# mikostrzewa/AprilSLAM

Hardware: AMD Instinct MI355X
Metric: frames/sec at 1280x720, 20 tags/frame (detection + batched PnP) (higher is better)
Workload: dtype u8/f64

## Files before the change

aprilslam_amd/csrc/aprilslam.hip:

```cpp
#include "../../include/aprilslam.h"

#include <algorithm>
#include <chrono>
#include <cmath>
#include <cstdarg>
#include <cstdio>
#include <cstring>
#include <memory>
#include <string>
#include <type_traits>
#include <vector>

#include "asl_common.h"
#include "tag_standard41h12.inc"
#include "k_wave.inc"

#include "k_threshold.inc"
#include "k_cc.inc"
#include "k_cluster.inc"
#include "k_seg.inc"
#include "k_quad.inc"
#include "k_decode.inc"
#include "k_pnp.inc"
#include "k_dedup.inc"
#include "k_graph.inc"
#include "k_render.inc"
#include "k_gn.inc"
#include "k_localize.inc"
#include "k_posecov.inc"
#include "k_rig.inc"
#include "k_calib.inc"
#include "k_map.inc"

static thread_local std::string g_err;

#include <dlfcn.h>
static struct Markers {
    int (*push)(const char *) = nullptr;
    int (*pop)() = nullptr;
    bool tried = false;
    void load()
    {
        tried = true;
        const char *e = getenv("ASL_ROCTX");
        if (!e || !*e || *e == '0') return;
        void *h = dlopen("librocprofiler-sdk-roctx.so", RTLD_NOW | RTLD_GLOBAL);
        if (!h) h = dlopen("libroctx64.so", RTLD_NOW | RTLD_GLOBAL);
        if (!h) return;
        push = reinterpret_cast<int (*)(const char *)>(dlsym(h, "roctxRangePushA"));
        pop = reinterpret_cast<int (*)()>(dlsym(h, "roctxRangePop"));
        if (!push || !pop) { push = nullptr; pop = nullptr; }
    }
} g_markers;
static inline void range_push(const char *name) { if (!g_markers.tried) g_markers.load(); if (g_markers.push) g_markers.push(name); }
static inline void range_pop() { if (g_markers.pop) g_markers.pop(); }

static int fail(int code, const char *fmt, ...)
{
    char buf[512];
    va_list ap;
    va_start(ap, fmt);
    vsnprintf(buf, sizeof buf, fmt, ap);
    va_end(ap);
    g_err = buf;
    return code;
}

#define HIPCHK(expr)                                                                                   \
    do {                                                                                               \
        hipError_t e__ = (expr);                                                                       \
        if (e__ != hipSuccess) return fail(ASL_EDEVICE, "%s failed: %s", #expr, hipGetErrorString(e__)); \
    } while (0)

#define MAX_STAGES 24

struct asl_detector {
    int device = 0;
    int maxhamming = 1;
    int decimate = 2;
    int refine = 1;
    int pnp_both_minima = 0;
    FamilyDev fam;
    DevBuf<unsigned long long> codes;
    DevBuf<unsigned short> idx_start;
    DevBuf<unsigned long long> idx_entries;

    unsigned int hash_slots_per_frame = 1024;
    unsigned int clusters_per_frame = 2048;
    unsigned int dets_per_frame = 256;
    double points_per_pixel = 0.5;

    DevBuf<uint8_t> in, dgray, tmin, tmax, tcut;
    DevBuf<uint8_t> dbg_thresh;
    DevBuf<unsigned int> dbg_labels;
    DevBuf<unsigned int> parent, sizes;
    DevBuf<unsigned long long> hkeys, points, rootmask, wmask, bmask;
    DevBuf<unsigned int> hcounts, class_lists, stage_pos, frame_cursor, dense_tiles, dense_seg, quad_list;
    DevBuf<unsigned long long> stage_rec;
    DevBuf<uint4> seg_edges;
    unsigned int stage_cap = 0;
    DevBuf<unsigned long long> slot_cluster;
    DevBuf<ClusterRec> clusters;
    DevBuf<QuadRec> quads;
    DevBuf<double> scratch, quadH, wtab, side_mom;
    DevBuf<DetRec> dets;
    DevBuf<unsigned int> frame_ndets, frame_idx, frame_nkeep, frame_off;
    DevBuf<DetOut> out_det;
    DevBuf<PoseOut> out_pose;
    DevBuf<long long> counters;
    DevBuf<float> pnp_corners;
    DevBuf<double> pnp_out;
    DevBuf<uint8_t> pnp_ok;
    DevBuf<uint8_t> gn_ws;
    DevBuf<uint8_t> loc_obs, loc_map;
    DevBuf<uint8_t> solve_out;
    DevBuf<uint8_t> rig_cams;
    DevBuf<uint8_t> cal_ws;
    DevBuf<uint8_t> map_ws, map_lm;
    hipStream_t copy_stream = nullptr, host_stream = nullptr;
    std::vector<hipEvent_t> copy_done;
    hipStream_t aux_stream = nullptr;

    Geom last{};
    unsigned int nslots = 0, max_clusters = 0, max_points = 0, max_dets = 0;
    long long last_counters[CNT__N] = {0};
    bool pending = false;
    const uint8_t *p_frames = nullptr;
    Geom p_geom{};
    hipStream_t p_stream = nullptr;
    bool p_has_cam = false;
    CamDev p_cam{};
    size_t prefetched = 0, nd_guess = 0;
    std::chrono::steady_clock::time_point t_submit, t_enqueued;
    PinnedBuf<long long> pinned_counters;
    PinnedBuf<DetOut> host_det;
    PinnedBuf<PoseOut> host_pose;
    PinnedBuf<unsigned int> host_nkeep;

    int profiling = 0;
    hipEvent_t ev[MAX_STAGES + 1] = {nullptr};
    int nev = 0;
    const char *stage_names[MAX_STAGES] = {nullptr};
    float stage_ms[MAX_STAGES] = {0};
    int nstages = 0;
    float host_ms[4] = {0, 0, 0, 0};

    size_t host_cap() const { return std::min(host_det.n, host_pose.n); }
    ~asl_detector()
    {
        for (hipStream_t s : {aux_stream, copy_stream, host_stream})
            if (s) (void)hipStreamDestroy(s);
        for (hipEvent_t e : copy_done) (void)hipEventDestroy(e);
        for (hipEvent_t e : ev)
            if (e) (void)hipEventDestroy(e);
    }
};

static const char *kVersion = "aprilslam 0.1 gfx950 (HIP, tagStandard41h12)";

extern "C" const char *asl_last_error(void) { return g_err.c_str(); }
extern "C" const char *asl_version(void) { return kVersion; }

static int build_code_index(asl_detector *d)
{
    FamilyDev &f = d->fam;
    f.idx_nch = 0; f.idx_start = nullptr; f.idx_entries = nullptr;
    const int nch = d->maxhamming + 1;
    if (f.nbits > 48 || f.ncodes > 65535 || nch > IDX_MAX_CHUNKS) return 0;
    if (getenv("ASL_NO_CODE_INDEX")) return 0;
    std::vector<unsigned short> start((size_t)nch * (IDX_BUCKETS + 1), 0);
    std::vector<unsigned long long> entries((size_t)nch * f.ncodes);
    int lo = 0;
    for (int c = 0; c < nch; c++) {
        const int w = f.nbits / nch + (c < f.nbits % nch ? 1 : 0);
        f.idx_lo[c] = lo; f.idx_w[c] = w;
        std::vector<unsigned int> bucket(f.ncodes);
        unsigned short *st = start.data() + (size_t)c * (IDX_BUCKETS + 1);
        for (int i = 0; i < f.ncodes; i++) {
            bucket[i] = idx_bucket((kTag41h12Codes[i] >> lo) & ((1ull << w) - 1ull), w);
            st[bucket[i] + 1]++;
        }
        for (int b = 0; b < IDX_BUCKETS; b++) st[b + 1] = (unsigned short)(st[b + 1] + st[b]);
        std::vector<unsigned short> fill(st, st + IDX_BUCKETS);
        for (int i = 0; i < f.ncodes; i++)
            entries[(size_t)c * f.ncodes + fill[bucket[i]]++] = ((unsigned long long)i << 48) | kTag41h12Codes[i];
        lo += w;
    }
    for (int c = nch; c < IDX_MAX_CHUNKS; c++) { f.idx_lo[c] = 0; f.idx_w[c] = 1; }
    if (d->idx_start.ensure(start.size()) || d->idx_entries.ensure((size_t)IDX_MAX_CHUNKS * kTag41h12NCodes)) return -1;
    if (hipMemcpy(d->idx_start.p, start.data(), start.size() * sizeof(unsigned short), hipMemcpyHostToDevice) != hipSuccess) return -1;
    if (hipMemcpy(d->idx_entries.p, entries.data(), entries.size() * sizeof(unsigned long long), hipMemcpyHostToDevice) != hipSuccess) return -1;
    f.idx_start = d->idx_start.p; f.idx_entries = d->idx_entries.p; f.idx_nch = nch;
    return 0;
}

extern "C" int asl_detector_create(const char *family, int nthreads, int maxhamming, float decimate, float blur,
                                   int refine_edges, int device, asl_detector **out)
{
    (void)nthreads;
    if (!out) return fail(ASL_EINVAL, "out is NULL");
    *out = nullptr;
    if (!family || strcmp(family, "tagStandard41h12") != 0)
        return fail(ASL_EINVAL, "unknown tag family '%s' (supported: tagStandard41h12)", family ? family : "(null)");
    if (!(decimate >= 1.0f) || decimate != std::floor(decimate) || decimate > 8.0f)
        return fail(ASL_EINVAL, "decimate must be an integer value in [1, 8] (got %g)", (double)decimate);
    if (blur != 0.0f) return fail(ASL_EINVAL, "blur (quad_sigma) != 0 is not supported (the reference never sets it)");
    if (maxhamming < 0 || maxhamming > 3) return fail(ASL_EINVAL, "maxhamming must be in [0, 3]");
    int ndev = 0;
    hipError_t e = hipGetDeviceCount(&ndev);
    if (e != hipSuccess || ndev <= 0) return fail(ASL_EDEVICE, "no HIP device available (%s)", hipGetErrorString(e));
    if (device < 0 || device >= ndev) return fail(ASL_EINVAL, "device %d out of range (have %d)", device, ndev);
    HIPCHK(hipSetDevice(device));
    std::unique_ptr<asl_detector> d(new asl_detector());
    d->device = device;
    d->maxhamming = maxhamming;
    d->decimate = (int)decimate;
    d->refine = refine_edges ? 1 : 0;
    memset(&d->fam, 0, sizeof d->fam);
    d->fam.nbits = kTag41h12NBits;
    d->fam.width_at_border = kTag41h12WidthAtBorder;
    d->fam.total_width = kTag41h12TotalWidth;
    d->fam.reversed_border = 1;
    d->fam.ncodes = kTag41h12PinnedIds;
    for (int i = 0; i < kTag41h12NBits; i++) { d->fam.bit_x[i] = kTag41h12BitX[i]; d->fam.bit_y[i] = kTag41h12BitY[i]; }
    if (d->codes.ensure(kTag41h12NCodes)) return fail(ASL_ENOMEM, "hipMalloc(code book) failed");
    if (hipMemcpy(d->codes.p, kTag41h12Codes, sizeof(unsigned long long) * kTag41h12NCodes, hipMemcpyHostToDevice) != hipSuccess)
        return fail(ASL_EDEVICE, "hipMemcpy(code book) failed");
    d->fam.codes = d->codes.p;
    if (build_code_index(d.get())) return fail(ASL_ENOMEM, "code-book index allocation failed");
    if (d->wtab.ensure(WEIGHT_TABLE_N)) return fail(ASL_ENOMEM, "hipMalloc(weight table) failed");
    hipLaunchKernelGGL(k_weight_table, dim3((WEIGHT_TABLE_N + 255) / 256), dim3(256), 0, 0, d->wtab.p);
    if (hipDeviceSynchronize() != hipSuccess) return fail(ASL_EDEVICE, "weight table kernel failed");
    (void)hipFuncSetAttribute(reinterpret_cast<const void *>(&k_fit_quads<256, true, CLASS3_CAP / 256>), hipFuncAttributeMaxDynamicSharedMemorySize, QUAD_LDS_BYTES(CLASS3_CAP));
    *out = d.release();
    return ASL_OK;
}

extern "C" void asl_detector_destroy(asl_detector *d)
{
    if (!d) return;
    (void)hipSetDevice(d->device);
    if (d->pending) (void)hipStreamSynchronize(d->p_stream);
    delete d;
}

extern "C" int asl_detector_set_id_limit(asl_detector *d, int n_ids)
{
    if (!d) return fail(ASL_EINVAL, "detector is NULL");
    if (n_ids > kTag41h12NCodes) return fail(ASL_EINVAL, "the code table holds %d ids (asked for %d)", kTag41h12NCodes, n_ids);
    if (d->pending) return fail(ASL_EINVAL, "a batch is in flight on this detector");
    d->fam.ncodes = n_ids <= 0 ? kTag41h12NCodes : n_ids;
    HIPCHK(hipSetDevice(d->device));
    if (build_code_index(d)) return fail(ASL_ENOMEM, "code-book index allocation failed");
    return ASL_OK;
}

extern "C" int asl_detector_set_pnp_both_minima(asl_detector *d, int enabled)
{
    if (!d) return fail(ASL_EINVAL, "detector is NULL");
    d->pnp_both_minima = enabled ? 1 : 0;
    return ASL_OK;
}

extern "C" int asl_set_profiling(asl_detector *d, int enabled)
{
    if (!d) return fail(ASL_EINVAL, "detector is NULL");
    d->profiling = enabled ? 1 : 0;
    if (enabled)
        for (int i = 0; i <= MAX_STAGES; i++)
            if (!d->ev[i]) HIPCHK(hipEventCreate(&d->ev[i]));
    return ASL_OK;
}

extern "C" int asl_stage_times(asl_detector *d, const char **names, float *ms, int max_n, int *n)
{
    if (!d || !n) return fail(ASL_EINVAL, "NULL argument");
    int k = std::min(max_n, d->nstages);
    for (int i = 0; i < k; i++) { if (names) names[i] = d->stage_names[i]; if (ms) ms[i] = d->stage_ms[i]; }
    static const char *hn[4] = {"host_enqueue", "host_wait", "host_copy", "host_post"};
    for (int i = 0; i < 4 && k < max_n; i++, k++) { if (names) names[k] = hn[i]; if (ms) ms[k] = d->host_ms[i]; }
    *n = k;
    return ASL_OK;
}

static int pnp_tpw(size_t expected)
{
    const char *e = getenv("ASL_PNP_TPW");
    if (e) { int x = atoi(e); return x < 1 ? 1 : (x > 16 ? 16 : x); }
    int v = 1;
    while (v < 16 && (size_t)v * 2 * 1024 <= expected) v <<= 1;
    return v;
}

static unsigned int next_pow2(unsigned long long v)
{
    unsigned long long p = 1;
    while (p < v) p <<= 1;
    return (unsigned int)p;
}

static int make_geom(asl_detector *d, int n_frames, int channels, int w, int h, int stride, size_t frame_pitch, Geom *g)
{
    if (n_frames <= 0 || n_frames > 65535) return fail(ASL_EINVAL, "n_frames must be in [1, 65535] (got %d)", n_frames);
    if (channels != 1 && channels != 3) return fail(ASL_EINVAL, "channels must be 1 (gray) or 3 (BGR), got %d", channels);
    if (w < 8 || h < 8 || w > 16384 || h > 16384) return fail(ASL_EINVAL, "unsupported image size %dx%d", w, h);
    if (stride < w * channels) return fail(ASL_EINVAL, "stride %d smaller than a row (%d bytes)", stride, w * channels);
    g->w = w; g->h = h; g->stride = stride; g->channels = channels; g->f = d->decimate;
    g->sw = 1 + (w - 1) / g->f; g->sh = 1 + (h - 1) / g->f;
    g->tw = g->sw / TILESZ; g->th = g->sh / TILESZ;
    g->nframes = n_frames; g->frame_pitch = frame_pitch;
    g->npix = (size_t)g->sw * g->sh;
    if (g->npix >= (1u << 24)) return fail(ASL_EINVAL, "decimated frame has %zu pixels; the cluster key holds 2^24", g->npix);
    return ASL_OK;
}

static int seg_nwx(const Geom &g) { return (g.sw + 63) / 64; }
static int seg_point_tiles_y(const Geom &g) { return std::max(1, (g.sh - 1 + SEG_PH - 1) / SEG_PH); }
static size_t count_tiles(const Geom &g) { return (size_t)seg_nwx(g) * (size_t)seg_point_tiles_y(g); }

static int ensure_workspace(asl_detector *d, const Geom &g)
{
    size_t B = (size_t)g.nframes;
    size_t total = B * g.npix;
    d->nslots = next_pow2(std::max<unsigned long long>(16384ull, (unsigned long long)B * d->hash_slots_per_frame));
    unsigned long long mc = (unsigned long long)B * d->clusters_per_frame;
    d->max_clusters = (unsigned int)std::min<unsigned long long>(mc, 0x7FFFFFFFull);
    unsigned long long mp = (unsigned long long)((double)total * d->points_per_pixel) + 65536ull;
    d->max_points = (unsigned int)std::min<unsigned long long>(mp, 0xFFFFFFF0ull);
    d->max_dets = (unsigned int)std::min<unsigned long long>((unsigned long long)B * d->dets_per_frame, 0x7FFFFFFFull);
    int bad = 0;
    bad |= d->dgray.ensure(total);
    bad |= d->tmin.ensure(B * (size_t)std::max(1, g.tw * g.th) + 8);
    bad |= d->tmax.ensure(B * (size_t)std::max(1, g.tw * g.th) + 8);
    bad |= d->tcut.ensure(B * (size_t)std::max(1, g.tw * g.th));
    bad |= d->parent.ensure(total);
    bad |= d->sizes.ensure(total);
    bad |= d->rootmask.ensure(B * (size_t)g.sh * (size_t)seg_nwx(g));
    bad |= d->wmask.ensure(B * (size_t)g.sh * (size_t)seg_nwx(g));
    bad |= d->bmask.ensure(B * (size_t)g.sh * (size_t)seg_nwx(g));
    bad |= d->hkeys.ensure(d->nslots);
    bad |= d->hcounts.ensure(d->nslots);
    bad |= d->class_lists.ensure((size_t)NCLASSES * d->max_clusters);
    bad |= d->slot_cluster.ensure(d->nslots);
    bad |= d->clusters.ensure(d->max_clusters);
    bad |= d->quads.ensure(d->max_clusters);
    bad |= d->quad_list.ensure(d->max_clusters);
    bad |= d->quadH.ensure((size_t)10 * d->max_clusters);
    bad |= d->side_mom.ensure((size_t)24 * d->max_clusters);
    bad |= d->points.ensure(d->max_points);
    d->stage_cap = (unsigned int)((double)g.npix * d->points_per_pixel) + 1024u;
    bad |= d->stage_rec.ensure((size_t)B * d->stage_cap);
    bad |= d->stage_pos.ensure((size_t)B * d->stage_cap);
    bad |= d->frame_cursor.ensure(B);
    bad |= d->dense_tiles.ensure(B * count_tiles(g));
    bad |= d->dense_seg.ensure(B * (size_t)seg_nwx(g) * (size_t)((g.sh + SEG_TH - 1) / SEG_TH));
    bad |= d->seg_edges.ensure(B * (size_t)seg_nwx(g) * (size_t)((g.sh + SEG_TH - 1) / SEG_TH));
    bad |= d->scratch.ensure((size_t)d->max_points * 8);
    bad |= d->dets.ensure(d->max_dets);
    bad |= d->frame_ndets.ensure(B);
    bad |= d->frame_nkeep.ensure(B);
    bad |= d->frame_off.ensure(B);
    bad |= d->frame_idx.ensure(B * (size_t)d->dets_per_frame);
    bad |= d->out_det.ensure(d->max_dets);
    bad |= d->out_pose.ensure(d->max_dets);
    bad |= d->counters.ensure(CNT__N);
    if (bad) return fail(ASL_ENOMEM, "device workspace allocation failed (%zu frames of %dx%d)", B, g.sw, g.sh);
    return ASL_OK;
}

#define STAGE(name)                                                        \
    do {                                                                   \
        if (d->profiling && d->nev < MAX_STAGES) {                         \
            d->stage_names[d->nev] = name;                                 \
            HIPCHK(hipEventRecord(d->ev[d->nev], st));                     \
            d->nev++;                                                      \
        }                                                                  \
    } while (0)

static int tag_width(const asl_detector *d, const Geom &g) { return std::max(3, d->fam.width_at_border / g.f); }

template <int BLOCK, int CAP>
static void launch_fit(asl_detector *d, const Geom &g, int cls, unsigned int grid, hipStream_t st)
{
    const int want_rev = d->fam.reversed_border ? 1 : 0, want_norm = d->fam.reversed_border ? 0 : 1;
    hipLaunchKernelGGL((k_fit_quads<BLOCK, (CAP > 0), CAP / BLOCK>), dim3(grid), dim3(BLOCK), CAP > 0 ? QUAD_LDS_BYTES(CAP) : 0, st, d->clusters.p,
                       d->class_lists.p + (size_t)cls * d->max_clusters, d->counters.p, cls, d->max_clusters, CAP, d->points.p, d->dgray.p, g,
                       tag_width(d, g), want_rev, want_norm, d->scratch.p, d->quads.p, d->wtab.p, d->side_mom.p);
}

static void launch_fit_class(asl_detector *d, const Geom &g, int cls, unsigned int B, hipStream_t st)
{
    const unsigned int qgrid = std::min<unsigned int>(d->max_clusters, std::max<unsigned int>(16384u, 32u * B));
    const unsigned int q2grid = std::min<unsigned int>(d->max_clusters, 2048u);
    switch (cls) {
    case 0: return launch_fit<64, CLASS0_CAP>(d, g, 0, qgrid, st);
    case 1: return launch_fit<128, CLASS1_CAP>(d, g, 1, qgrid, st);
    case 2: return launch_fit<256, CLASS2_CAP>(d, g, 2, q2grid, st);
    case 3: return launch_fit<256, CLASS3_CAP>(d, g, 3, q2grid, st);
    default: return launch_fit<256, 0>(d, g, 4, q2grid, st);
    }
}

static void launch_quad_finish(asl_detector *d, const Geom &g, hipStream_t st)
{
    hipLaunchKernelGGL(k_quad_finish, dim3(std::min<unsigned int>((d->max_clusters + 63) / 64, 4096u)), dim3(256), 0, st, d->quads.p, d->side_mom.p, d->counters.p,
                       d->max_clusters, tag_width(d, g));
}

static int enqueue_detect(asl_detector *d, const uint8_t *d_frames, const Geom &g, hipStream_t st, const CamDev *cam)
{
    dim3 blk(64, 4, 1);
    int thx = (g.sh + TILESZ - 1) / TILESZ;
    unsigned int B = (unsigned int)g.nframes;
    d->nev = 0;
    range_push("S0-S4 gray, decimate, threshold, segmentation, clusters");
    STAGE("k_hash_clear");
    hipLaunchKernelGGL(k_hash_clear, dim3((std::max<unsigned int>(d->nslots, std::max<unsigned int>(B, CNT__N)) + 255) / 256), dim3(256), 0, st, d->hkeys.p,
                       d->hcounts.p, d->nslots, d->counters.p, d->frame_cursor.p, d->frame_ndets.p, B);

    STAGE("k_decimate_minmax");
    if (g.f == 2) {
        const unsigned int ntile = (unsigned int)(g.tw * g.th);
        const unsigned int nrest = (unsigned int)(g.sw - 4 * g.tw) * (unsigned int)g.sh + (unsigned int)(g.sh - 4 * g.th) * (unsigned int)(4 * g.tw);
        if (ntile)
            hipLaunchKernelGGL((g.channels == 1 ? k_decimate2_tiles<1> : k_decimate2_tiles<3>), dim3((ntile + 255) / 256, B), dim3(256), 0, st, d_frames, g,
                               d->dgray.p, d->tmin.p, d->tmax.p);
        if (nrest)
            hipLaunchKernelGGL((g.channels == 1 ? k_decimate_rest<1> : k_decimate_rest<3>), dim3((nrest + 255) / 256, B), dim3(256), 0, st, d_frames, g,
                               d->dgray.p);
    } else
        hipLaunchKernelGGL((g.channels == 1 ? k_decimate_minmax<1> : k_decimate_minmax<3>), dim3((g.sw + 63) / 64, (thx + 3) / 4, B), blk, 0, st, d_frames, g, d->dgray.p, d->tmin.p, d->tmax.p);

    const int nwx = seg_nwx(g), pty = seg_point_tiles_y(g);
    const size_t nwords = (size_t)B * g.sh * nwx;
    STAGE("k_tile_cut");
    if (g.tw > 0 && g.th > 0)
        hipLaunchKernelGGL(k_tile_cut, dim3((((g.tw + 3) / 4) * ((g.th + 3) / 4) + 255) / 256, B), dim3(256), 0, st, d->tmin.p, d->tmax.p, g, d->tcut.p);
    STAGE("k_seg_tile");
    {
        const int ntiles = nwx * ((g.sh + SEG_TH - 1) / SEG_TH);
        hipLaunchKernelGGL(k_seg_tile, dim3((ntiles + SEG_TILE_WAVES - 1) / SEG_TILE_WAVES, 1, B), dim3(64 * SEG_TILE_WAVES), 0, st, d->dgray.p, d->tcut.p, g, nwx, ntiles,
                           d->wmask.p, d->bmask.p, d->parent.p, d->sizes.p, d->rootmask.p, d->seg_edges.p, d->dense_seg.p, d->counters.p);
        hipLaunchKernelGGL(k_seg_tile_dense, dim3(1024), dim3(64), 0, st, g, nwx, ntiles, d->wmask.p, d->bmask.p, d->parent.p, d->sizes.p,
                           d->rootmask.p, d->dense_seg.p, d->counters.p);
    }
    STAGE("k_seg_border");
    {
        const size_t nseams = nwx > 1 ? (size_t)B * g.sh * (nwx - 1) : 0;
        const unsigned int ncol_blocks = (unsigned int)((nseams + 63) / 64);
        const int nrb = (g.sh - 1) / SEG_TH;
        const unsigned int nrow_blocks = (unsigned int)nwx * (unsigned int)nrb * (unsigned int)B;
        if (ncol_blocks + nrow_blocks > 0)
            hipLaunchKernelGGL(k_seg_border, dim3(ncol_blocks + nrow_blocks), dim3(64), 0, st, d->wmask.p, d->bmask.p, d->seg_edges.p,
                               nwx * ((g.sh + SEG_TH - 1) / SEG_TH), g, nwx, d->parent.p, d->counters.p, ncol_blocks, nrb > 0 ? nrb : 1);
    }
    STAGE("k_seg_roots");
    hipLaunchKernelGGL(k_seg_roots, dim3((unsigned int)((nwords + 255) / 256)), dim3(256), 0, st, d->rootmask.p, g, nwx, d->parent.p, d->sizes.p);

    STAGE("k_seg_points");
    hipLaunchKernelGGL((k_seg_points<SEGP_PCAP, SEGP_RUNCAP, SEGP_NW, 1>), dim3(B, (nwx + SEGP_NW - 1) / SEGP_NW, pty), dim3(64 * SEGP_NW), 0, st,
                       d->wmask.p, d->bmask.p, g, nwx, d->parent.p, d->sizes.p, d->hkeys.p, d->hcounts.p, d->nslots - 1, d->stage_rec.p,
                       d->stage_pos.p, d->frame_cursor.p, d->stage_cap, d->dense_tiles.p, pty, d->counters.p);
    hipLaunchKernelGGL((k_seg_points<SEGP_PCAP_DENSE, SEGP_RUNCAP_DENSE, 1, 2>), dim3(256), dim3(64), 0, st, d->wmask.p, d->bmask.p, g, nwx,
                       d->parent.p, d->sizes.p, d->hkeys.p, d->hcounts.p, d->nslots - 1, d->stage_rec.p, d->stage_pos.p, d->frame_cursor.p,
                       d->stage_cap, d->dense_tiles.p, pty, d->counters.p);
    STAGE("k_cluster_filter");
    hipLaunchKernelGGL(k_cluster_filter, dim3((d->nslots + 1023) / 1024), dim3(1024), 0, st, d->hkeys.p, d->hcounts.p, d->nslots, g,
                       d->clusters.p, d->slot_cluster.p, d->class_lists.p, d->max_clusters, d->max_points, d->counters.p);
    STAGE("k_point_place");
    hipLaunchKernelGGL(k_point_place, dim3(16, B), dim3(256), 0, st, d->stage_rec.p, d->stage_pos.p, d->frame_cursor.p, d->stage_cap,
                       d->slot_cluster.p, d->points.p, d->counters.p);

    range_pop();
    range_push("S5 quad fit");
    for (int cls = 0; cls < NCLASSES; cls++) {
        static const char *const kFitStage[NCLASSES] = {"k_fit_quads<0>", "k_fit_quads<1>", "k_fit_quads<2>", "k_fit_quads<3>", "k_fit_quads<4>"};
        STAGE(kFitStage[cls]);
        launch_fit_class(d, g, cls, B, st);
    }

    STAGE("k_quad_finish");
    launch_quad_finish(d, g, st);
    range_pop();
    range_push("S6-S7 edge refinement, homography, decode");
    STAGE("k_quad_compact");
    hipLaunchKernelGGL(k_quad_compact, dim3((d->max_clusters + 1023) / 1024), dim3(1024), 0, st, d->quads.p, d->counters.p, d->max_clusters,
                       d->quad_list.p);
    unsigned int dgrid = std::min<unsigned int>(d->max_clusters, std::max<unsigned int>(8192u, 64u * B));
    STAGE("k_refine");
    hipLaunchKernelGGL((g.channels == 1 ? k_refine<1> : k_refine<3>), dim3(dgrid), dim3(64), 0, st, d->quads.p, d->counters.p, d->max_clusters, d_frames, g,
                       d->fam.reversed_border ? 1 : 0, d->refine, d->quadH.p, d->quad_list.p, d->side_mom.p);
    STAGE("k_homography");
    hipLaunchKernelGGL(k_homography, dim3(std::min<unsigned int>((d->max_clusters + 31) / 32, 2048u)), dim3(256), 0, st, d->quadH.p, d->counters.p, d->max_clusters,
                       d->quad_list.p, d->side_mom.p);
    STAGE("k_decode");
    hipLaunchKernelGGL((g.channels == 1 ? k_decode<1> : k_decode<3>), dim3(dgrid), dim3(64), 0, st, d->quads.p, d->quadH.p, d->counters.p, d->max_clusters, d_frames, g, d->fam,
                       d->maxhamming, d->dets.p, d->max_dets, d->counters.p, d->quad_list.p);

    range_pop();
    range_push("S9 PnP, S8 de-duplication");
    if (cam) {
        STAGE("k_pnp_dets");
        const int tpw = pnp_tpw(d->nd_guess ? d->nd_guess : (size_t)20 * B);
        hipLaunchKernelGGL(k_pnp_dets, dim3((d->max_dets + tpw - 1) / tpw), dim3(64), 0, st, d->dets.p, d->counters.p, d->max_dets, *cam, tpw);
    }
    STAGE("k_det_dedup");
    {
        const unsigned int cap_f = d->dets_per_frame;
        hipLaunchKernelGGL(k_det_bucket, dim3((d->max_dets + 255) / 256), dim3(256), 0, st, d->dets.p, d->counters.p, d->max_dets, d->frame_ndets.p,
                           d->frame_idx.p, cap_f, d->counters.p);
        hipLaunchKernelGGL(k_det_dedup, dim3(B), dim3(256), 0, st, d->dets.p, d->counters.p, d->frame_ndets.p, d->frame_idx.p, cap_f,
                           d->frame_nkeep.p, d->counters.p);
        hipLaunchKernelGGL(k_det_offsets, dim3(1), dim3(1024), 0, st, d->frame_nkeep.p, B, d->frame_off.p, d->counters.p);
        hipLaunchKernelGGL(k_det_gather, dim3((cap_f + 255) / 256, B), dim3(256), 0, st, d->dets.p, d->frame_idx.p, cap_f, d->frame_nkeep.p,
                           d->frame_off.p, d->out_det.p, d->out_pose.p, d->max_dets, cam ? 1 : 0);
    }
    range_pop();
    if (d->profiling && d->nev <= MAX_STAGES) HIPCHK(hipEventRecord(d->ev[d->nev], st));
    HIPCHK(hipGetLastError());
    return ASL_OK;
}

static CamDev make_cam(const asl_detector *d, const double *K, const double *dist, int n_dist, double tag_size)
{
    CamDev c;
    c.both_minima = d->pnp_both_minima; c.pad = 0;
    c.fx = K[0]; c.fy = K[4]; c.cx = K[2]; c.cy = K[5];
    c.k1 = c.k2 = c.p1 = c.p2 = c.k3 = 0;
    if (dist && n_dist >= 4) { c.k1 = dist[0]; c.k2 = dist[1]; c.p1 = dist[2]; c.p2 = dist[3]; }
    if (dist && n_dist >= 5) c.k3 = dist[4];
    c.half = (double)(float)(tag_size / 2);
    return c;
}

using clk = std::chrono::steady_clock;
static float msf(clk::time_point a, clk::time_point b) { return std::chrono::duration<float, std::milli>(b - a).count(); }

static int ensure_host_out(asl_detector *d, size_t want, size_t nframes)
{
    HIPCHK(d->host_nkeep.ensure(nframes, hipHostMallocDefault));
    if (want <= d->host_cap()) return ASL_OK;
    d->host_det.release(); d->host_pose.release();
    want = std::max<size_t>(want * 2, 4096);
    HIPCHK(d->host_det.ensure(want, hipHostMallocNonCoherent));
    HIPCHK(d->host_pose.ensure(want, hipHostMallocNonCoherent));
    return ASL_OK;
}

static int submit_batch(asl_detector *d, const uint8_t *d_frames, const Geom &g, hipStream_t st, const CamDev *cam)
{
    if (d->pending) return fail(ASL_EINVAL, "a batch is already in flight on this detector: collect it first");
    int rc = ensure_workspace(d, g);
    if (rc) return rc;
    d->t_submit = clk::now();
    rc = enqueue_detect(d, d_frames, g, st, cam);
    if (rc) return rc;
    HIPCHK(d->pinned_counters.ensure(CNT__N, hipHostMallocDefault));
    HIPCHK(hipMemcpyAsync(d->pinned_counters.p, d->counters.p, sizeof(long long) * CNT__N, hipMemcpyDeviceToHost, st));
    d->prefetched = 0;
    rc = ensure_host_out(d, std::min<size_t>(d->nd_guess, d->max_dets), (size_t)g.nframes);
    if (rc) return rc;
    HIPCHK(hipMemcpyAsync(d->host_nkeep.p, d->frame_nkeep.p, sizeof(unsigned int) * (size_t)g.nframes, hipMemcpyDeviceToHost, st));
    if (d->nd_guess > 0) {
        size_t guess = std::min<size_t>(d->nd_guess, d->max_dets);
        HIPCHK(hipMemcpyAsync(d->host_det.p, d->out_det.p, guess * sizeof(DetOut), hipMemcpyDeviceToHost, st));
        if (cam) HIPCHK(hipMemcpyAsync(d->host_pose.p, d->out_pose.p, guess * sizeof(PoseOut), hipMemcpyDeviceToHost, st));
        d->prefetched = guess;
    }
    d->pending = true;
    d->p_frames = d_frames; d->p_geom = g; d->p_stream = st; d->p_has_cam = cam != nullptr;
    if (cam) d->p_cam = *cam;
    d->t_enqueued = clk::now();
    return ASL_OK;
}

static int collect_batch(asl_detector *d, asl_detection *out, asl_pose *poses, int max_out, int *n_per_frame, int *n_out)
{
    if (!d->pending) return fail(ASL_EINVAL, "no batch in flight on this detector");
    const Geom g = d->p_geom;
    hipStream_t st = d->p_stream;
    const CamDev *cam = d->p_has_cam ? &d->p_cam : nullptr;
    clk::time_point t0 = d->t_submit, t1 = d->t_enqueued, t2 = t1;
    for (int attempt = 0; attempt < 4; attempt++) {
        if (attempt > 0) {
            d->pending = false;
            d->nd_guess = 0;
            int rc = submit_batch(d, d->p_frames, g, st, cam);
            if (rc) return rc;
        }
        HIPCHK(hipStreamSynchronize(st));
        t2 = clk::now();
        memcpy(d->last_counters, d->pinned_counters.p, sizeof(long long) * CNT__N);
        d->last = g;
        long long *c = d->last_counters;
        if (c[CNT_UF_GUARD]) {
            d->pending = false;
            return fail(ASL_ECAPACITY, "a union-find loop hit its iteration guard (%lld times): labels of this batch are not trustworthy", c[CNT_UF_GUARD]);
        }
        bool again = false;
        if (c[CNT_OVERFLOW_HASH]) { d->hash_slots_per_frame *= 4; again = true; }
        if (c[CNT_OVERFLOW_CLUSTERS] || c[CNT_NCLUSTERS] > (long long)d->max_clusters) { d->clusters_per_frame *= 4; again = true; }
        if (c[CNT_OVERFLOW_POINTS]) { d->points_per_pixel *= 2; again = true; }
        if (c[CNT_OVERFLOW_DETS]) { d->dets_per_frame *= 4; again = true; }
        if (again) {
            if (attempt == 3) {
                d->pending = false;
                return fail(ASL_ECAPACITY, "work buffers still overflow after growing (hash %lld clusters %lld points %lld dets %lld)",
                            c[CNT_OVERFLOW_HASH], c[CNT_OVERFLOW_CLUSTERS], c[CNT_OVERFLOW_POINTS], c[CNT_OVERFLOW_DETS]);
            }
            continue;
        }
        break;
    }
    d->pending = false;
    if (d->profiling) {
        d->nstages = d->nev;
        for (int i = 0; i < d->nev; i++) HIPCHK(hipEventElapsedTime(&d->stage_ms[i], d->ev[i], d->ev[i + 1]));
    }
    if (d->last_counters[CNT_DEDUP_LIMIT])
        return fail(ASL_ECAPACITY, "%lld frame(s) hold more than %d detections: the de-duplication does not sort that many", d->last_counters[CNT_DEDUP_LIMIT], DEDUP_MAX);
    size_t nd = (size_t)d->last_counters[CNT_NKEEP];
    if (nd > d->max_dets) nd = d->max_dets;
    if (nd > d->prefetched) {
        size_t have = d->prefetched;
        if (nd > d->host_cap()) have = 0;
        int rc = ensure_host_out(d, nd, (size_t)g.nframes);
        if (rc) return rc;
        HIPCHK(hipMemcpy(d->host_det.p + have, d->out_det.p + have, (nd - have) * sizeof(DetOut), hipMemcpyDeviceToHost));
        if (cam) HIPCHK(hipMemcpy(d->host_pose.p + have, d->out_pose.p + have, (nd - have) * sizeof(PoseOut), hipMemcpyDeviceToHost));
    }
    d->nd_guess = nd + nd / 4 + 256;
    clk::time_point t3 = clk::now();
    static_assert(sizeof(DetOut) == sizeof(asl_detection) && sizeof(PoseOut) == sizeof(asl_pose), "device results are copied verbatim");
    int total = (int)nd;
    int nw = std::min(total, max_out);
    if (out && nw > 0) memcpy(out, d->host_det.p, (size_t)nw * sizeof(asl_detection));
    if (poses && cam && nw > 0) memcpy(poses, d->host_pose.p, (size_t)nw * sizeof(asl_pose));
    if (n_per_frame) for (int f = 0; f < g.nframes; f++) n_per_frame[f] = (int)d->host_nkeep.p[f];
    if (n_out) *n_out = total;
    d->host_ms[0] = msf(t0, t1); d->host_ms[1] = msf(t1, t2); d->host_ms[2] = msf(t2, t3); d->host_ms[3] = msf(t3, clk::now());
    return ASL_OK;
}

static int check_n_dist(int n_dist)
{
    if (n_dist != 0 && n_dist != 4 && n_dist != 5) return fail(ASL_EINVAL, "n_dist must be 0, 4 or 5");
    return ASL_OK;
}

static int check_device_args(asl_detector *d, const void *d_frames, int n_frames, int channels, int w, int h, int stride, size_t frame_pitch,
                             int n_dist, Geom *g)
{
    if (!d || !d_frames) return fail(ASL_EINVAL, "NULL detector or frames");
    if (int rc = check_n_dist(n_dist)) return rc;
    HIPCHK(hipSetDevice(d->device));
    int rc = make_geom(d, n_frames, channels, w, h, stride, frame_pitch, g);
    if (rc) return rc;
    if (frame_pitch < (size_t)stride * (size_t)h) return fail(ASL_EINVAL, "frame_pitch smaller than one frame");
    return ASL_OK;
}

extern "C" int asl_submit_batch_device(asl_detector *d, const void *d_frames, int n_frames, int channels, int w, int h, int stride,
                                       size_t frame_pitch, void *stream, const double *K, const double *dist, int n_dist, double tag_size)
{
    Geom g;
    int rc = check_device_args(d, d_frames, n_frames, channels, w, h, stride, frame_pitch, n_dist, &g);
    if (rc) return rc;
    CamDev cam;
    if (K) cam = make_cam(d, K, dist, n_dist, tag_size);
    return submit_batch(d, (const uint8_t *)d_frames, g, (hipStream_t)stream, K ? &cam : nullptr);
}

extern "C" int asl_collect_batch(asl_detector *d, asl_detection *out, asl_pose *poses, int max_out, int *n_per_frame, int *n_out)
{
    if (!d) return fail(ASL_EINVAL, "NULL detector");
    if (max_out < 0 || (max_out > 0 && !out)) return fail(ASL_EINVAL, "out is NULL");
    HIPCHK(hipSetDevice(d->device));
    return collect_batch(d, out, poses, max_out, n_per_frame, n_out);
}

extern "C" int asl_collect_batch_view(asl_detector *d, const asl_detection **out, const asl_pose **poses, const uint32_t **n_per_frame, int *n_out)
{
    if (!d || !out || !n_per_frame || !n_out) return fail(ASL_EINVAL, "NULL argument");
    HIPCHK(hipSetDevice(d->device));
    const bool with_poses = d->p_has_cam;
    int rc = collect_batch(d, nullptr, nullptr, 0, nullptr, n_out);
    if (rc) return rc;
    *out = reinterpret_cast<const asl_detection *>(d->host_det.p);
    if (poses) *poses = with_poses ? reinterpret_cast<const asl_pose *>(d->host_pose.p) : nullptr;
    *n_per_frame = d->host_nkeep.p;
    return ASL_OK;
}

extern "C" int asl_detect_batch_device(asl_detector *d, const void *d_frames, int n_frames, int channels, int w, int h, int stride,
                                       size_t frame_pitch, void *stream, const double *K, const double *dist, int n_dist,
                                       double tag_size, asl_detection *out, asl_pose *poses, int max_out, int *n_per_frame, int *n_out)
{
    if (max_out < 0 || (max_out > 0 && !out)) return fail(ASL_EINVAL, "out is NULL");
    int rc = asl_submit_batch_device(d, d_frames, n_frames, channels, w, h, stride, frame_pitch, stream, K, dist, n_dist, tag_size);
    if (rc) return rc;
    return collect_batch(d, out, poses, max_out, n_per_frame, n_out);
}

#define HOST_CHUNK_FRAMES 64
static hipError_t copy_frames(asl_detector *d, const uint8_t *const *frames, int f0, int f1, size_t pitch, hipStream_t st)
{
    int i = f0;
    while (i < f1) {
        int j = i + 1;
        while (j < f1 && frames[j] == frames[j - 1] + pitch) j++;
        hipError_t e = hipMemcpyAsync(d->in.p + (size_t)i * pitch, frames[i], pitch * (size_t)(j - i), hipMemcpyHostToDevice, st);
        if (e != hipSuccess) return e;
        i = j;
    }
    return hipSuccess;
}

static int detect_host_frames(asl_detector *d, const uint8_t *const *frames, int n_frames, int channels, int w, int h, int stride,
                              const CamDev *cam, asl_detection *out, asl_pose *poses, int max_out, int *n_per_frame, int *n_out)
{
    Geom g;
    const size_t pitch = (size_t)stride * (size_t)h;
    int rc = make_geom(d, n_frames, channels, w, h, stride, pitch, &g);
    if (rc) return rc;
    if (d->in.ensure(pitch * (size_t)n_frames)) return fail(ASL_ENOMEM, "input staging allocation failed");
    for (int i = 0; i < n_frames; i++)
        if (!frames[i]) return fail(ASL_EINVAL, "frames[%d] is NULL", i);
    int chunk = HOST_CHUNK_FRAMES;
    { const char *e = getenv("ASL_HOST_CHUNK"); if (e && atoi(e) > 0) chunk = atoi(e); }
    const int nchunks = n_frames >= 2 * chunk ? (n_frames + chunk - 1) / chunk : 1;
    if (nchunks == 1) {
        HIPCHK(copy_frames(d, frames, 0, n_frames, pitch, nullptr));
        int rcs = submit_batch(d, d->in.p, g, nullptr, cam);
        if (rcs) return rcs;
        return collect_batch(d, out, poses, max_out, n_per_frame, n_out);
    }
    if (!d->copy_stream) {
        HIPCHK(hipStreamCreateWithFlags(&d->copy_stream, hipStreamNonBlocking));
        HIPCHK(hipStreamCreateWithFlags(&d->host_stream, hipStreamNonBlocking));
    }
    while ((int)d->copy_done.size() < nchunks) {
        hipEvent_t e;
        HIPCHK(hipEventCreateWithFlags(&e, hipEventDisableTiming));
        d->copy_done.push_back(e);
    }
    HIPCHK(hipStreamSynchronize(nullptr));
    for (int c = 0; c < nchunks; c++) {
        const int f0 = c * chunk, f1 = std::min(n_frames, f0 + chunk);
        HIPCHK(copy_frames(d, frames, f0, f1, pitch, d->copy_stream));
        HIPCHK(hipEventRecord(d->copy_done[c], d->copy_stream));
    }
    int total = 0;
    for (int c = 0; c < nchunks; c++) {
        const int f0 = c * chunk, f1 = std::min(n_frames, f0 + chunk);
        Geom gc = g;
        gc.nframes = f1 - f0;
        HIPCHK(hipStreamWaitEvent(d->host_stream, d->copy_done[c], 0));
        int rcs = submit_batch(d, d->in.p + (size_t)f0 * pitch, gc, d->host_stream, cam);
        if (rcs) { (void)hipStreamSynchronize(d->copy_stream); return rcs; }
        int nc = 0;
        const int room = std::max(0, max_out - total);
        rcs = collect_batch(d, out ? out + std::min(total, max_out) : nullptr, (poses && cam) ? poses + std::min(total, max_out) : nullptr, room,
                            n_per_frame ? n_per_frame + f0 : nullptr, &nc);
        if (rcs) { (void)hipStreamSynchronize(d->copy_stream); return rcs; }
        for (int k = total; k < std::min(total + nc, max_out); k++) out[k].frame += f0;
        total += nc;
    }
    if (n_out) *n_out = total;
    return ASL_OK;
}

extern "C" int asl_detect_batch_u8(asl_detector *d, const uint8_t *const *frames, int n_frames, int channels, int w, int h, int stride,
                                   asl_detection *out, int max_out, int *n_per_frame, int *n_out)
{
    if (!d || !frames) return fail(ASL_EINVAL, "NULL detector or frames");
    if (max_out < 0 || (max_out > 0 && !out)) return fail(ASL_EINVAL, "out is NULL");
    HIPCHK(hipSetDevice(d->device));
    return detect_host_frames(d, frames, n_frames, channels, w, h, stride, nullptr, out, nullptr, max_out, n_per_frame, n_out);
}

extern "C" int asl_detect_batch_pose_u8(asl_detector *d, const uint8_t *const *frames, int n_frames, int channels, int w, int h, int stride,
                                        const double *K, const double *dist, int n_dist, double tag_size, asl_detection *out, asl_pose *poses,
                                        int max_out, int *n_per_frame, int *n_out)
{
    if (!d || !frames || !K || !poses) return fail(ASL_EINVAL, "NULL detector, frames, K or poses");
    if (max_out < 0 || (max_out > 0 && !out)) return fail(ASL_EINVAL, "out is NULL");
    if (int rc = check_n_dist(n_dist)) return rc;
    if (n_dist && !dist) return fail(ASL_EINVAL, "dist is NULL but n_dist = %d", n_dist);
    HIPCHK(hipSetDevice(d->device));
    CamDev cam = make_cam(d, K, dist, n_dist, tag_size);
    return detect_host_frames(d, frames, n_frames, channels, w, h, stride, &cam, out, poses, max_out, n_per_frame, n_out);
}

extern "C" int asl_detect_gray_u8(asl_detector *d, const uint8_t *gray, int w, int h, int stride, asl_detection *out, int max_out, int *n_out)
{
    const uint8_t *fr[1] = {gray};
    return asl_detect_batch_u8(d, fr, 1, 1, w, h, stride, out, max_out, nullptr, n_out);
}

extern "C" int asl_detect_bgr_u8(asl_detector *d, const uint8_t *bgr, int w, int h, int stride, asl_detection *out, int max_out, int *n_out)
{
    const uint8_t *fr[1] = {bgr};
    return asl_detect_batch_u8(d, fr, 1, 3, w, h, stride, out, max_out, nullptr, n_out);
}

extern "C" int asl_render_frames_device(asl_detector *d, void *d_frames, int n_frames, int w, int h, int stride, size_t frame_pitch,
                                        const void *d_planes, int max_planes, const void *d_textures, int tw, int th, double half,
                                        const double *K, const double *dist, int n_dist, void *stream)
{
    if (!d || !d_frames || !d_planes || !d_textures) return fail(ASL_EINVAL, "NULL argument");
    if (n_frames <= 0 || w <= 0 || h <= 0 || max_planes <= 0 || tw <= 0 || th <= 0) return fail(ASL_EINVAL, "sizes must be positive");
    if (stride < 3 * w || frame_pitch < (size_t)stride * (size_t)h) return fail(ASL_EINVAL, "stride / frame_pitch smaller than a BGR row / frame");
    if (dist && n_dist != 4 && n_dist != 5) return fail(ASL_EINVAL, "n_dist must be 4 or 5");
    if (dist && !K) return fail(ASL_EINVAL, "lens coefficients need the camera matrix");
    static_assert(sizeof(RenderPlane) == sizeof(asl_render_plane) && sizeof(asl_render_plane) == 96, "asl_render_plane layout");
    HIPCHK(hipSetDevice(d->device));
    RenderCam cam;
    memset(&cam, 0, sizeof cam);
    cam.iters = 8;
    if (K && dist) {
        cam.fx = K[0]; cam.fy = K[4]; cam.cx = K[2]; cam.cy = K[5];
        cam.k1 = dist[0]; cam.k2 = dist[1]; cam.p1 = dist[2]; cam.p2 = dist[3]; cam.k3 = n_dist >= 5 ? dist[4] : 0.0;
        cam.distort = 1;
    }
    hipLaunchKernelGGL(k_render, dim3((w + RENDER_TW - 1) / RENDER_TW, (h + 4 * RENDER_TH - 1) / (4 * RENDER_TH), (unsigned int)n_frames), dim3(64, 4), 0, (hipStream_t)stream, (uint8_t *)d_frames, w, h,
                       stride, frame_pitch, (const RenderPlane *)d_planes, max_planes, (const uint8_t *)d_textures, tw, th, half, cam);
    HIPCHK(hipGetLastError());
    return ASL_OK;
}

extern "C" int asl_pack_observations_device(asl_detector *d, void *d_obs, int max_tags, void *stream)
{
    if (!d || !d_obs) return fail(ASL_EINVAL, "NULL detector or output");
    if (max_tags <= 0) return fail(ASL_EINVAL, "max_tags must be positive");
    if (!d->pending) return fail(ASL_EINVAL, "no batch in flight on this detector: pack between submit and the next submit");
    static_assert(sizeof(ObsRec) == sizeof(asl_obs) && sizeof(asl_obs) == 136, "asl_obs layout");
    HIPCHK(hipSetDevice(d->device));
    const int nf = d->p_geom.nframes;
    const unsigned int total = (unsigned int)nf * (unsigned int)max_tags;
    hipLaunchKernelGGL(k_obs_pack, dim3((total + 255) / 256), dim3(256), 0, (hipStream_t)stream, d->dets.p, d->frame_idx.p, d->dets_per_frame,
                       d->frame_nkeep.p, d->counters.p, (ObsRec *)d_obs, nf, max_tags);
    HIPCHK(hipGetLastError());
    return ASL_OK;
}

extern "C" int asl_graph_frames_device(asl_detector *d, const void *d_obs, int world, int n_frames, int max_tags, int coordinate_id,
                                       double *d_pose, uint8_t *d_status, uint32_t *d_last, int n_ids, void *d_picks, void *stream)
{
    if (!d || !d_obs || !d_pose || !d_status || !d_last) return fail(ASL_EINVAL, "NULL argument");
    if (world <= 0 || n_frames <= 0 || max_tags <= 0 || n_ids <= 0) return fail(ASL_EINVAL, "sizes must be positive");
    HIPCHK(hipSetDevice(d->device));
    const unsigned int total = (unsigned int)world * (unsigned int)n_frames;
    const int lds_ids = (size_t)n_ids * sizeof(unsigned int) <= 48 * 1024 ? n_ids : 0;
    hipLaunchKernelGGL(k_graph_frames, dim3((total + 255) / 256), dim3(256), sizeof(unsigned int) * (size_t)lds_ids, (hipStream_t)stream, (const ObsRec *)d_obs,
                       world, n_frames, max_tags, coordinate_id, d_pose, d_status, (unsigned int *)d_last, n_ids, lds_ids);
    if (d_picks)
        hipLaunchKernelGGL(k_graph_pick, dim3((n_ids + 255) / 256), dim3(256), 0, (hipStream_t)stream, (const ObsRec *)d_obs, world, n_frames, max_tags,
                           (const unsigned int *)d_last, n_ids, (ObsRec *)d_picks);
    HIPCHK(hipGetLastError());
    return ASL_OK;
}

extern "C" int asl_graph_picks_device(asl_detector *d, const void *d_obs, int world, int n_frames, int max_tags, const uint8_t *d_status,
                                      unsigned int order_lo, unsigned int order_hi, uint32_t *d_last, int n_ids, void *d_picks, void *stream)
{
    if (!d || !d_obs || !d_status || !d_last || !d_picks) return fail(ASL_EINVAL, "NULL argument");
    if (world <= 0 || n_frames <= 0 || max_tags <= 0 || n_ids <= 0) return fail(ASL_EINVAL, "sizes must be positive");
    if (order_lo > order_hi) return fail(ASL_EINVAL, "empty or reversed range");
    HIPCHK(hipSetDevice(d->device));
    HIPCHK(hipMemsetAsync(d_last, 0, sizeof(uint32_t) * (size_t)n_ids, (hipStream_t)stream));
    const unsigned int total = (unsigned int)world * (unsigned int)n_frames;
    const int lds_ids = (size_t)n_ids * sizeof(unsigned int) <= 48 * 1024 ? n_ids : 0;
    hipLaunchKernelGGL(k_graph_last_range, dim3((total + 255) / 256), dim3(256), sizeof(unsigned int) * (size_t)lds_ids, (hipStream_t)stream, (const ObsRec *)d_obs,
                       world, n_frames, max_tags, d_status, order_lo, order_hi, (unsigned int *)d_last, n_ids, lds_ids);
    hipLaunchKernelGGL(k_graph_pick, dim3((n_ids + 255) / 256), dim3(256), 0, (hipStream_t)stream, (const ObsRec *)d_obs, world, n_frames, max_tags,
                       (const unsigned int *)d_last, n_ids, (ObsRec *)d_picks);
    HIPCHK(hipGetLastError());
    return ASL_OK;
}

extern "C" int asl_solve_pnp_batch(asl_detector *d, const float *corners, const double *K, const double *dist, int n_dist,
                                   double tag_size, double *rvec, double *tvec, double *T, uint8_t *ok, int N)
{
    if (!d || !corners || !K || !rvec || !tvec || !T || !ok) return fail(ASL_EINVAL, "NULL argument");
    if (N < 0) return fail(ASL_EINVAL, "N < 0");
    if (int rc = check_n_dist(n_dist)) return rc;
    if (N == 0) return ASL_OK;
    HIPCHK(hipSetDevice(d->device));
    if (d->pnp_corners.ensure((size_t)N * 8) || d->pnp_out.ensure((size_t)N * 22) || d->pnp_ok.ensure((size_t)N))
        return fail(ASL_ENOMEM, "PnP workspace allocation failed");
    CamDev cam = make_cam(d, K, dist, n_dist, tag_size);
    HIPCHK(hipMemcpy(d->pnp_corners.p, corners, sizeof(float) * 8 * (size_t)N, hipMemcpyHostToDevice));
    double *dr = d->pnp_out.p, *dt = dr + 3 * (size_t)N, *dT = dt + 3 * (size_t)N;
    hipLaunchKernelGGL(k_pnp_batch, dim3((N + pnp_tpw((size_t)N) - 1) / pnp_tpw((size_t)N)), dim3(64), 0, nullptr, d->pnp_corners.p, N, cam, dr, dt, dT, d->pnp_ok.p, pnp_tpw((size_t)N));
    HIPCHK(hipGetLastError());
    HIPCHK(hipMemcpy(rvec, dr, sizeof(double) * 3 * (size_t)N, hipMemcpyDeviceToHost));
    HIPCHK(hipMemcpy(tvec, dt, sizeof(double) * 3 * (size_t)N, hipMemcpyDeviceToHost));
    HIPCHK(hipMemcpy(T, dT, sizeof(double) * 16 * (size_t)N, hipMemcpyDeviceToHost));
    HIPCHK(hipMemcpy(ok, d->pnp_ok.p, (size_t)N, hipMemcpyDeviceToHost));
    return ASL_OK;
}

#include "gn_host.inc"


static int check_obs_args(int max_tags, int n_ids, int n_dist, bool no_dist, double tag_size)
{
    if (max_tags < 1 || max_tags > 256) return fail(ASL_EINVAL, "max_tags must be in [1, 256] (got %d)", max_tags);
    if (n_ids < 1) return fail(ASL_EINVAL, "n_ids must be >= 1 (got %d)", n_ids);
    if (int rc = check_n_dist(n_dist)) return rc;
    if (n_dist && no_dist) return fail(ASL_EINVAL, "dist is NULL with n_dist = %d", n_dist);
    if (!(tag_size > 0) || !std::isfinite(tag_size)) return fail(ASL_EINVAL, "tag_size must be positive (got %g)", tag_size);
    return ASL_OK;
}

static int upload_obs(asl_detector *d, const char *what, const asl_obs *obs, int n_frames, int max_tags, const asl_map_tag *map, int n_ids)
{
    const size_t obs_bytes = sizeof(asl_obs) * (size_t)n_frames * (size_t)max_tags, map_bytes = sizeof(asl_map_tag) * (size_t)n_ids;
    if (d->loc_obs.ensure(obs_bytes) || (map && d->loc_map.ensure(map_bytes))) return fail(ASL_ENOMEM, "%s workspace allocation failed", what);
    HIPCHK(hipMemcpy(d->loc_obs.p, obs, obs_bytes, hipMemcpyHostToDevice));
    if (map) HIPCHK(hipMemcpy(d->loc_map.p, map, map_bytes, hipMemcpyHostToDevice));
    return ASL_OK;
}

static int check_localize_args(const void *obs, int n_frames, int max_tags, const void *map, int n_ids, const double *K, const double *dist,
                               int n_dist, double tag_size, double max_tag_rms_px, const void *out)
{
    if (!obs || !map || !K || !out) return fail(ASL_EINVAL, "NULL argument");
    if (n_frames < 0) return fail(ASL_EINVAL, "n_frames < 0");
    if (int rc = check_obs_args(max_tags, n_ids, n_dist, !dist, tag_size)) return rc;
    if (!(max_tag_rms_px >= 0) || !std::isfinite(max_tag_rms_px)) return fail(ASL_EINVAL, "max_tag_rms_px must be >= 0 (got %g)", max_tag_rms_px);
    return ASL_OK;
}

static void launch_localize(asl_detector *d, const void *d_obs, int n_frames, int max_tags, const void *d_map, int n_ids, const double *K,
                            const double *dist, int n_dist, double tag_size, double max_tag_rms_px, void *d_out, void *d_cov, double sigma_px,
                            hipStream_t st)
{
    CamDev cam = make_cam(d, K, dist, n_dist, tag_size);
    if (d_cov)
        hipLaunchKernelGGL(k_localize<true>, dim3((unsigned int)n_frames), dim3(ASL_WAVE), loc_lds_bytes(max_tags), st, (const ObsRec *)d_obs, max_tags,
                           (const MapTagRec *)d_map, n_ids, cam, max_tag_rms_px, (CamPoseRec *)d_out, (PoseCovRec *)d_cov, sigma_px);
    else
        hipLaunchKernelGGL(k_localize<false>, dim3((unsigned int)n_frames), dim3(ASL_WAVE), loc_lds_bytes(max_tags), st, (const ObsRec *)d_obs, max_tags,
                           (const MapTagRec *)d_map, n_ids, cam, max_tag_rms_px, (CamPoseRec *)d_out, (PoseCovRec *)nullptr, 0.0);
}

static int check_sigma_px(double sigma_px)
{
    if (!(sigma_px >= 0) || !std::isfinite(sigma_px)) return fail(ASL_EINVAL, "sigma_px must be >= 0 and finite (got %g)", sigma_px);
    return ASL_OK;
}

static int localize_frames_device(asl_detector *d, const void *d_obs, int n_frames, int max_tags, const void *d_map, int n_ids, const double *K,
                                  const double *dist, int n_dist, double tag_size, double max_tag_rms_px, double sigma_px, void *d_out,
                                  void *d_cov, void *stream)
{
    static_assert(sizeof(MapTagRec) == sizeof(asl_map_tag) && sizeof(asl_map_tag) == 104, "asl_map_tag layout");
    static_assert(sizeof(CamPoseRec) == sizeof(asl_cam_pose) && sizeof(asl_cam_pose) == 160, "asl_cam_pose layout");
    static_assert(sizeof(PoseCovRec) == sizeof(asl_pose_cov) && sizeof(asl_pose_cov) == 304, "asl_pose_cov layout");
    if (!d) return fail(ASL_EINVAL, "NULL detector");
    int rc = check_localize_args(d_obs, n_frames, max_tags, d_map, n_ids, K, dist, n_dist, tag_size, max_tag_rms_px, d_out);
    if (rc) return rc;
    if ((rc = check_sigma_px(sigma_px))) return rc;
    if (n_frames == 0) return ASL_OK;
    HIPCHK(hipSetDevice(d->device));
    launch_localize(d, d_obs, n_frames, max_tags, d_map, n_ids, K, dist, n_dist, tag_size, max_tag_rms_px, d_out, d_cov, sigma_px, (hipStream_t)stream);
    HIPCHK(hipGetLastError());
    return ASL_OK;
}

extern "C" int asl_localize_frames_device(asl_detector *d, const void *d_obs, int n_frames, int max_tags, const void *d_map, int n_ids,
                                          const double *K, const double *dist, int n_dist, double tag_size, double max_tag_rms_px,
                                          void *d_out, void *stream)
{
    return localize_frames_device(d, d_obs, n_frames, max_tags, d_map, n_ids, K, dist, n_dist, tag_size, max_tag_rms_px, 0.0, d_out, nullptr, stream);
}

extern "C" int asl_localize_cov_frames_device(asl_detector *d, const void *d_obs, int n_frames, int max_tags, const void *d_map, int n_ids,
                                              const double *K, const double *dist, int n_dist, double tag_size, double max_tag_rms_px,
                                              double sigma_px, void *d_out, void *d_cov, void *stream)
{
    if (!d_cov) return fail(ASL_EINVAL, "NULL argument");
    return localize_frames_device(d, d_obs, n_frames, max_tags, d_map, n_ids, K, dist, n_dist, tag_size, max_tag_rms_px, sigma_px, d_out, d_cov, stream);
}

static int localize_batch(asl_detector *d, const asl_obs *obs, int n_frames, int max_tags, const asl_map_tag *map, int n_ids, const double *K,
                          const double *dist, int n_dist, double tag_size, double max_tag_rms_px, double sigma_px, asl_cam_pose *out,
                          asl_pose_cov *cov)
{
    if (!d) return fail(ASL_EINVAL, "NULL detector");
    int rc = check_localize_args(obs, n_frames, max_tags, map, n_ids, K, dist, n_dist, tag_size, max_tag_rms_px, out);
    if (rc) return rc;
    if ((rc = check_sigma_px(sigma_px))) return rc;
    if (n_frames == 0) return ASL_OK;
    HIPCHK(hipSetDevice(d->device));
    asl_cam_pose *d_out = nullptr;
    asl_pose_cov *d_cov = nullptr;
    if (carve_ws(d->solve_out, [&](WsCarve &c) { d_out = c.take<asl_cam_pose>(n_frames); d_cov = c.take<asl_pose_cov>(cov ? n_frames : 0); }))
        return fail(ASL_ENOMEM, "localisation workspace allocation failed");
    if ((rc = upload_obs(d, "localisation", obs, n_frames, max_tags, map, n_ids))) return rc;
    launch_localize(d, d->loc_obs.p, n_frames, max_tags, d->loc_map.p, n_ids, K, dist, n_dist, tag_size, max_tag_rms_px, d_out, cov ? d_cov : nullptr,
                    sigma_px, nullptr);
    HIPCHK(hipGetLastError());
    HIPCHK(hipMemcpy(out, d_out, sizeof(asl_cam_pose) * (size_t)n_frames, hipMemcpyDeviceToHost));
    if (cov) HIPCHK(hipMemcpy(cov, d_cov, sizeof(asl_pose_cov) * (size_t)n_frames, hipMemcpyDeviceToHost));
    return ASL_OK;
}

extern "C" int asl_localize_batch(asl_detector *d, const asl_obs *obs, int n_frames, int max_tags, const asl_map_tag *map, int n_ids,
                                  const double *K, const double *dist, int n_dist, double tag_size, double max_tag_rms_px, asl_cam_pose *out)
{
    return localize_batch(d, obs, n_frames, max_tags, map, n_ids, K, dist, n_dist, tag_size, max_tag_rms_px, 0.0, out, nullptr);
}

extern "C" int asl_localize_cov_batch(asl_detector *d, const asl_obs *obs, int n_frames, int max_tags, const asl_map_tag *map, int n_ids,
                                      const double *K, const double *dist, int n_dist, double tag_size, double max_tag_rms_px, double sigma_px,
                                      asl_cam_pose *out, asl_pose_cov *cov)
{
    if (!cov) return fail(ASL_EINVAL, "NULL argument");
    return localize_batch(d, obs, n_frames, max_tags, map, n_ids, K, dist, n_dist, tag_size, max_tag_rms_px, sigma_px, out, cov);
}


static int check_rig_table(const asl_rig_camera *rig, int n_cams)
{
    for (int c = 0; c < n_cams; c++) {
        const asl_rig_camera &r = rig[c];
        if (check_n_dist(r.n_dist)) return fail(ASL_EINVAL, "camera %d: n_dist must be 0, 4 or 5 (got %d)", c, r.n_dist);
        for (int k = 0; k < 9; k++)
            if (!std::isfinite(r.K[k])) return fail(ASL_EINVAL, "camera %d: K is not finite", c);
        for (int k = 0; k < r.n_dist; k++)
            if (!std::isfinite(r.dist[k])) return fail(ASL_EINVAL, "camera %d: dist is not finite", c);
        for (int k = 0; k < 12; k++)
            if (!std::isfinite(r.E[k])) return fail(ASL_EINVAL, "camera %d: E is not finite", c);
        const double *E = r.E;
        double dev = 0;
        for (int i = 0; i < 3; i++)
            for (int j = 0; j < 3; j++)
                dev = std::max(dev, std::fabs(E[4 * i] * E[4 * j] + E[4 * i + 1] * E[4 * j + 1] + E[4 * i + 2] * E[4 * j + 2] - (i == j ? 1.0 : 0.0)));
        const double det = E[0] * (E[5] * E[10] - E[6] * E[9]) - E[1] * (E[4] * E[10] - E[6] * E[8]) + E[2] * (E[4] * E[9] - E[5] * E[8]);
        if (!(dev <= 1e-6) || !(det > 0))
            return fail(ASL_EINVAL, "camera %d: the rotation part of E is not a rotation (|R R^T - I| = %g, det %g)", c, dev, det);
    }
    return ASL_OK;
}

static int check_rig_args(const void *obs, int n_cams, int n_frames, int max_tags, const void *map, int n_ids, const void *rig, double tag_size,
                          double max_tag_rms_px, double sigma_px, const void *out)
{
    if (!obs || !map || !rig || !out) return fail(ASL_EINVAL, "NULL argument");
    if (n_frames < 0) return fail(ASL_EINVAL, "n_frames < 0");
    if (n_cams < 1 || n_cams > RIG_MAX_CAMS) return fail(ASL_EINVAL, "n_cams must be in [1, %d] (got %d)", RIG_MAX_CAMS, n_cams);
    if (int rc = check_obs_args(max_tags, n_ids, 0, false, tag_size)) return rc;
    if (n_cams * max_tags > RIG_MAX_SLOTS) return fail(ASL_EINVAL, "n_cams * max_tags must be <= %d (got %d x %d)", RIG_MAX_SLOTS, n_cams, max_tags);
    if (!(max_tag_rms_px >= 0) || !std::isfinite(max_tag_rms_px)) return fail(ASL_EINVAL, "max_tag_rms_px must be >= 0 (got %g)", max_tag_rms_px);
    return check_sigma_px(sigma_px);
}

static void launch_localize_rig(const void *d_obs, int n_cams, int n_frames, int max_tags, const void *d_map, int n_ids, const void *d_rig,
                                double tag_size, double max_tag_rms_px, void *d_out, void *d_cov, double sigma_px, hipStream_t st)
{
    const double half = (double)(float)(tag_size / 2);
    if (d_cov)
        hipLaunchKernelGGL(k_localize_rig<true>, dim3((unsigned int)n_frames), dim3(ASL_WAVE), rig_lds_bytes(n_cams, max_tags), st, (const ObsRec *)d_obs,
                           n_cams, max_tags, (const MapTagRec *)d_map, n_ids, (const RigCamRec *)d_rig, half, max_tag_rms_px, (CamPoseRec *)d_out,
                           (PoseCovRec *)d_cov, sigma_px);
    else
        hipLaunchKernelGGL(k_localize_rig<false>, dim3((unsigned int)n_frames), dim3(ASL_WAVE), rig_lds_bytes(n_cams, max_tags), st, (const ObsRec *)d_obs,
                           n_cams, max_tags, (const MapTagRec *)d_map, n_ids, (const RigCamRec *)d_rig, half, max_tag_rms_px, (CamPoseRec *)d_out,
                           (PoseCovRec *)nullptr, 0.0);
}

static int localize_rig_frames_device(asl_detector *d, const void *d_obs, int n_cams, int n_frames, int max_tags, const void *d_map, int n_ids,
                                      const void *d_rig, double tag_size, double max_tag_rms_px, double sigma_px, void *d_out, void *d_cov,
                                      void *stream)
{
    static_assert(sizeof(RigCamRec) == sizeof(asl_rig_camera) && sizeof(asl_rig_camera) == 216, "asl_rig_camera layout");
    if (!d) return fail(ASL_EINVAL, "NULL detector");
    if (int rc = check_rig_args(d_obs, n_cams, n_frames, max_tags, d_map, n_ids, d_rig, tag_size, max_tag_rms_px, sigma_px, d_out)) return rc;
    HIPCHK(hipSetDevice(d->device));
    asl_rig_camera tab[RIG_MAX_CAMS];
    HIPCHK(hipMemcpy(tab, d_rig, sizeof(asl_rig_camera) * (size_t)n_cams, hipMemcpyDeviceToHost));
    if (int rc = check_rig_table(tab, n_cams)) return rc;
    if (n_frames == 0) return ASL_OK;
    launch_localize_rig(d_obs, n_cams, n_frames, max_tags, d_map, n_ids, d_rig, tag_size, max_tag_rms_px, d_out, d_cov, sigma_px, (hipStream_t)stream);
    HIPCHK(hipGetLastError());
    return ASL_OK;
}

extern "C" int asl_localize_rig_frames_device(asl_detector *d, const void *d_obs, int n_cams, int n_frames, int max_tags, const void *d_map,
                                              int n_ids, const void *d_rig, double tag_size, double max_tag_rms_px, void *d_out, void *stream)
{
    return localize_rig_frames_device(d, d_obs, n_cams, n_frames, max_tags, d_map, n_ids, d_rig, tag_size, max_tag_rms_px, 0.0, d_out, nullptr, stream);
}

extern "C" int asl_localize_rig_cov_frames_device(asl_detector *d, const void *d_obs, int n_cams, int n_frames, int max_tags, const void *d_map,
                                                  int n_ids, const void *d_rig, double tag_size, double max_tag_rms_px, double sigma_px,
                                                  void *d_out, void *d_cov, void *stream)
{
    if (!d_cov) return fail(ASL_EINVAL, "NULL argument");
    return localize_rig_frames_device(d, d_obs, n_cams, n_frames, max_tags, d_map, n_ids, d_rig, tag_size, max_tag_rms_px, sigma_px, d_out, d_cov, stream);
}

static int localize_rig_batch(asl_detector *d, const asl_obs *obs, int n_cams, int n_frames, int max_tags, const asl_map_tag *map, int n_ids,
                              const asl_rig_camera *rig, double tag_size, double max_tag_rms_px, double sigma_px, asl_cam_pose *out,
                              asl_pose_cov *cov)
{
    if (!d) return fail(ASL_EINVAL, "NULL detector");
    int rc = check_rig_args(obs, n_cams, n_frames, max_tags, map, n_ids, rig, tag_size, max_tag_rms_px, sigma_px, out);
    if (rc) return rc;
    if ((rc = check_rig_table(rig, n_cams))) return rc;
    if (n_frames == 0) return ASL_OK;
    HIPCHK(hipSetDevice(d->device));
    asl_cam_pose *d_out = nullptr;
    asl_pose_cov *d_cov = nullptr;
    if (carve_ws(d->solve_out, [&](WsCarve &c) { d_out = c.take<asl_cam_pose>(n_frames); d_cov = c.take<asl_pose_cov>(cov ? n_frames : 0); }) ||
        d->rig_cams.ensure(sizeof(asl_rig_camera) * (size_t)n_cams))
        return fail(ASL_ENOMEM, "rig localisation workspace allocation failed");
    if ((rc = upload_obs(d, "rig localisation", obs, n_cams * n_frames, max_tags, map, n_ids))) return rc;
    HIPCHK(hipMemcpy(d->rig_cams.p, rig, sizeof(asl_rig_camera) * (size_t)n_cams, hipMemcpyHostToDevice));
    launch_localize_rig(d->loc_obs.p, n_cams, n_frames, max_tags, d->loc_map.p, n_ids, d->rig_cams.p, tag_size, max_tag_rms_px, d_out,
                        cov ? d_cov : nullptr, sigma_px, nullptr);
    HIPCHK(hipGetLastError());
    HIPCHK(hipMemcpy(out, d_out, sizeof(asl_cam_pose) * (size_t)n_frames, hipMemcpyDeviceToHost));
    if (cov) HIPCHK(hipMemcpy(cov, d_cov, sizeof(asl_pose_cov) * (size_t)n_frames, hipMemcpyDeviceToHost));
    return ASL_OK;
}

extern "C" int asl_localize_rig_batch(asl_detector *d, const asl_obs *obs, int n_cams, int n_frames, int max_tags, const asl_map_tag *map, int n_ids,
                                      const asl_rig_camera *rig, double tag_size, double max_tag_rms_px, asl_cam_pose *out)
{
    return localize_rig_batch(d, obs, n_cams, n_frames, max_tags, map, n_ids, rig, tag_size, max_tag_rms_px, 0.0, out, nullptr);
}

extern "C" int asl_localize_rig_cov_batch(asl_detector *d, const asl_obs *obs, int n_cams, int n_frames, int max_tags, const asl_map_tag *map,
                                          int n_ids, const asl_rig_camera *rig, double tag_size, double max_tag_rms_px, double sigma_px,
                                          asl_cam_pose *out, asl_pose_cov *cov)
{
    if (!cov) return fail(ASL_EINVAL, "NULL argument");
    return localize_rig_batch(d, obs, n_cams, n_frames, max_tags, map, n_ids, rig, tag_size, max_tag_rms_px, sigma_px, out, cov);
}


static int check_pose_cov_args(const void *in, int n, const double *K, const double *dist, int n_dist, double tag_size, double sigma_px, const void *cov)
{
    if (!in || !K || !cov) return fail(ASL_EINVAL, "NULL argument");
    if (n < 0) return fail(ASL_EINVAL, "record count < 0");
    if (int rc = check_n_dist(n_dist)) return rc;
    if (n_dist && !dist) return fail(ASL_EINVAL, "dist is NULL with n_dist = %d", n_dist);
    if (!(tag_size > 0) || !std::isfinite(tag_size)) return fail(ASL_EINVAL, "tag_size must be positive (got %g)", tag_size);
    return check_sigma_px(sigma_px);
}

static void launch_pose_cov(asl_detector *d, const void *d_obs, int n, const double *K, const double *dist, int n_dist, double tag_size,
                            double sigma_px, void *d_cov, hipStream_t st)
{
    CamDev cam = make_cam(d, K, dist, n_dist, tag_size);
    hipLaunchKernelGGL(k_pnp_cov, dim3((unsigned int)((n + PNP_TAGS_PER_WAVE - 1) / PNP_TAGS_PER_WAVE)), dim3(ASL_WAVE), 0, st, (const ObsRec *)d_obs, n, cam,
                       sigma_px, (PoseCovRec *)d_cov);
}

extern "C" int asl_pose_cov_device(asl_detector *d, const void *d_obs, int n_records, const double *K, const double *dist, int n_dist,
                                   double tag_size, double sigma_px, void *d_cov, void *stream)
{
    if (!d) return fail(ASL_EINVAL, "NULL detector");
    if (int rc = check_pose_cov_args(d_obs, n_records, K, dist, n_dist, tag_size, sigma_px, d_cov)) return rc;
    if (n_records == 0) return ASL_OK;
    HIPCHK(hipSetDevice(d->device));
    launch_pose_cov(d, d_obs, n_records, K, dist, n_dist, tag_size, sigma_px, d_cov, (hipStream_t)stream);
    HIPCHK(hipGetLastError());
    return ASL_OK;
}

extern "C" int asl_solve_pnp_cov_batch(asl_detector *d, const float *corners, const double *T, const double *K, const double *dist, int n_dist,
                                       double tag_size, double sigma_px, asl_pose_cov *cov, int N)
{
    if (!d) return fail(ASL_EINVAL, "NULL detector");
    if (!T) return fail(ASL_EINVAL, "NULL argument");
    if (int rc = check_pose_cov_args(corners, N, K, dist, n_dist, tag_size, sigma_px, cov)) return rc;
    if (N == 0) return ASL_OK;
    HIPCHK(hipSetDevice(d->device));
    std::vector<asl_obs> rec((size_t)N);
    for (int i = 0; i < N; i++) {
        bool finite = true;
        for (int k = 0; k < 12; k++) finite = finite && std::isfinite(T[16 * (size_t)i + k]);
        rec[i].id = 0;
        rec[i].flags = finite ? 3 : 1;
        memcpy(rec[i].corners, corners + 8 * (size_t)i, sizeof rec[i].corners);
        memcpy(rec[i].T, T + 16 * (size_t)i, sizeof rec[i].T);
    }
    const size_t cov_bytes = sizeof(asl_pose_cov) * (size_t)N;
    if (d->solve_out.ensure(cov_bytes)) return fail(ASL_ENOMEM, "pose covariance workspace allocation failed");
    if (int rc = upload_obs(d, "pose covariance", rec.data(), 1, N, nullptr, 0)) return rc;
    launch_pose_cov(d, d->loc_obs.p, N, K, dist, n_dist, tag_size, sigma_px, d->solve_out.p, nullptr);
    HIPCHK(hipGetLastError());
    HIPCHK(hipMemcpy(cov, d->solve_out.p, cov_bytes, hipMemcpyDeviceToHost));
    return ASL_OK;
}

static int check_calib_args(const void *obs, int n_frames, int max_tags, const void *map, int n_ids, double tag_size, int width, int height,
                            const double *K_init, int n_dist, int flags, int max_iters, const void *result, const void *poses)
{
    if (!obs || !map || !result || !poses) return fail(ASL_EINVAL, "NULL argument");
    if (n_frames < 1) return fail(ASL_EINVAL, "n_frames must be >= 1 (got %d)", n_frames);
    if (int rc = check_obs_args(max_tags, n_ids, n_dist, false, tag_size)) return rc;
    if (width < 1 || height < 1) return fail(ASL_EINVAL, "width and height must be positive (got %d x %d)", width, height);
    if (max_iters < 1) return fail(ASL_EINVAL, "max_iters must be >= 1 (got %d)", max_iters);
    if (flags & ~(ASL_CALIB_FIX_PRINCIPAL_POINT | ASL_CALIB_FIX_ASPECT_RATIO | ASL_CALIB_ZERO_TANGENT_DIST))
        return fail(ASL_EINVAL, "unknown calibration flags 0x%x", flags);
    if (K_init && !(K_init[0] > 0 && K_init[4] > 0 && std::isfinite(K_init[0]) && std::isfinite(K_init[4]) && std::isfinite(K_init[2]) &&
                    std::isfinite(K_init[5])))
        return fail(ASL_EINVAL, "K_init must have finite, positive focal lengths");
    return ASL_OK;
}

static int launch_calibrate(asl_detector *d, const void *d_obs, int n_frames, int max_tags, const void *d_map, int n_ids, double tag_size,
                            int width, int height, const double *K_init, int n_dist, int flags, int max_iters, void *d_result, void *d_poses,
                            hipStream_t st)
{
    static_assert(sizeof(CalibResultRec) == sizeof(asl_calib_result) && sizeof(asl_calib_result) == 216, "asl_calib_result layout");
    const size_t nf = (size_t)n_frames;
    CalibArgs a{};
    if (carve_ws(d->cal_ws, [&](WsCarve &c) {
            a.st = c.take<CalibState>(1); a.list = c.take<int>(nf); a.fr = c.take<int>(CAL_FR * nf);
            a.zh = c.take<double>(CAL_ZH * nf); a.seedc = c.take<double>(nf); a.pose = c.take<double>(2 * 12 * nf);
            a.H = c.take<double>(2 * CAL_HS * nf); a.SB = c.take<double>(CAL_SB * nf); a.back = c.take<double>(CAL_BK * nf);
        }))
        return fail(ASL_ENOMEM, "calibration workspace allocation failed");
    a.obs = (const ObsRec *)d_obs; a.map = (const MapTagRec *)d_map;
    a.res = (CalibResultRec *)d_result; a.out = (CamPoseRec *)d_poses;
    a.half = (double)(float)(tag_size / 2);
    a.width = width; a.height = height;
    a.has_init = K_init != nullptr;
    if (K_init) { a.Kinit[0] = K_init[0]; a.Kinit[1] = K_init[4]; a.Kinit[2] = K_init[2]; a.Kinit[3] = K_init[5]; }
    a.n_frames = n_frames; a.max_tags = max_tags; a.n_ids = n_ids; a.n_dist = n_dist; a.flags = flags; a.max_iters = max_iters;
    int np = 0;
    if (!(flags & ASL_CALIB_FIX_ASPECT_RATIO)) a.sel[np++] = 0;
    a.sel[np++] = 1;
    if (!(flags & ASL_CALIB_FIX_PRINCIPAL_POINT)) { a.sel[np++] = 2; a.sel[np++] = 3; }
    if (n_dist >= 4) {
        a.sel[np++] = 4; a.sel[np++] = 5;
        if (!(flags & ASL_CALIB_ZERO_TANGENT_DIST)) { a.sel[np++] = 6; a.sel[np++] = 7; }
    }
    if (n_dist == 5) a.sel[np++] = 8;
    a.np = np;
    const dim3 frames((unsigned int)n_frames), wave(ASL_WAVE), wg(CAL_WG);
    const size_t lds = loc_lds_bytes(max_tags);
    auto seed = n_dist == 5 ? k_calib_seed<5> : n_dist == 4 ? k_calib_seed<4> : k_calib_seed<0>;
    auto step = n_dist == 5 ? k_calib_step<5> : n_dist == 4 ? k_calib_step<4> : k_calib_step<0>;
    hipLaunchKernelGGL(k_calib_init, frames, wave, 0, st, a);
    hipLaunchKernelGGL(k_calib_k0, dim3(1), wg, 0, st, a);
    hipLaunchKernelGGL(seed, frames, wave, lds, st, a);
    hipLaunchKernelGGL(k_calib_start, dim3(1), wg, 0, st, a);
    for (int it = 0; it < max_iters; it++) {
        hipLaunchKernelGGL(k_calib_schur, frames, wave, 0, st, a, 0);
        hipLaunchKernelGGL(k_calib_solve, dim3(1), wg, 0, st, a);
        hipLaunchKernelGGL(step, frames, wave, lds, st, a);
        hipLaunchKernelGGL(k_calib_decide, dim3(1), wg, 0, st, a);
    }
    hipLaunchKernelGGL(k_calib_schur, frames, wave, 0, st, a, 1);
    hipLaunchKernelGGL(k_calib_finish, dim3(1), wg, 0, st, a);
    HIPCHK(hipGetLastError());
    return ASL_OK;
}

extern "C" int asl_calibrate_frames_device(asl_detector *d, const void *d_obs, int n_frames, int max_tags, const void *d_map, int n_ids,
                                           double tag_size, int width, int height, const double *K_init, int n_dist, int flags, int max_iters,
                                           void *d_result, void *d_poses, void *stream)
{
    if (!d) return fail(ASL_EINVAL, "NULL detector");
    int rc = check_calib_args(d_obs, n_frames, max_tags, d_map, n_ids, tag_size, width, height, K_init, n_dist, flags, max_iters, d_result, d_poses);
    if (rc) return rc;
    HIPCHK(hipSetDevice(d->device));
    return launch_calibrate(d, d_obs, n_frames, max_tags, d_map, n_ids, tag_size, width, height, K_init, n_dist, flags, max_iters, d_result,
                            d_poses, (hipStream_t)stream);
}

extern "C" int asl_calibrate_batch(asl_detector *d, const asl_obs *obs, int n_frames, int max_tags, const asl_map_tag *map, int n_ids,
                                   double tag_size, int width, int height, const double *K_init, int n_dist, int flags, int max_iters,
                                   asl_calib_result *result, asl_cam_pose *poses)
{
    if (!d) return fail(ASL_EINVAL, "NULL detector");
    int rc = check_calib_args(obs, n_frames, max_tags, map, n_ids, tag_size, width, height, K_init, n_dist, flags, max_iters, result, poses);
    if (rc) return rc;
    HIPCHK(hipSetDevice(d->device));
    asl_calib_result *d_result;
    asl_cam_pose *d_poses;
    if (carve_ws(d->solve_out, [&](WsCarve &c) { d_result = c.take<asl_calib_result>(1); d_poses = c.take<asl_cam_pose>(n_frames); }))
        return fail(ASL_ENOMEM, "calibration workspace allocation failed");
    if ((rc = upload_obs(d, "calibration", obs, n_frames, max_tags, map, n_ids))) return rc;
    rc = launch_calibrate(d, d->loc_obs.p, n_frames, max_tags, d->loc_map.p, n_ids, tag_size, width, height, K_init, n_dist, flags, max_iters,
                          d_result, d_poses, nullptr);
    if (rc) return rc;
    HIPCHK(hipMemcpy(result, d_result, sizeof(asl_calib_result), hipMemcpyDeviceToHost));
    HIPCHK(hipMemcpy(poses, d_poses, sizeof(asl_cam_pose) * (size_t)n_frames, hipMemcpyDeviceToHost));
    return ASL_OK;
}

static int check_map_args(const void *obs, int n_frames, int max_tags, int n_ids, const double *K, const double *dist, int n_dist,
                          double tag_size, int world_id, int max_iters, const void *map, const void *poses, const void *result)
{
    if (!obs || !K || !map || !poses || !result) return fail(ASL_EINVAL, "NULL argument");
    if (n_frames < 1) return fail(ASL_EINVAL, "n_frames must be >= 1 (got %d)", n_frames);
    if (int rc = check_obs_args(max_tags, n_ids, n_dist, !dist, tag_size)) return rc;
    if (world_id < -1 || world_id >= n_ids) return fail(ASL_EINVAL, "world_id must be -1 or in [0, n_ids) (got %d)", world_id);
    if (max_iters < 1 || max_iters > MAP_MAX_ITERS) return fail(ASL_EINVAL, "max_iters must be in [1, %d] (got %d)", MAP_MAX_ITERS, max_iters);
    return ASL_OK;
}

static int launch_map(asl_detector *d, const void *d_obs, int n_frames, int max_tags, int n_ids, const double *K, const double *dist, int n_dist,
                      double tag_size, int world_id, int max_iters, void *d_map, void *d_std, void *d_poses, void *d_result, hipStream_t st)
{
    static_assert(sizeof(MapResultRec) == sizeof(asl_map_result) && sizeof(asl_map_result) == 64, "asl_map_result layout");
    const size_t nf = (size_t)n_frames, ni = (size_t)n_ids, nsl = nf * (size_t)max_tags;
    MapArgs a{};
    int *per_id, *per_frame, *per_cam, *per_obs, *csr;
    if (carve_ws(d->map_ws, [&](WsCarve &c) {
            a.head = c.take<MapHead>(1); per_id = c.take<int>(4 * (ni + 1)); per_frame = c.take<int>(3 * (nf + 1));
            per_cam = c.take<int>(4 * (nf + 1)); a.tag_state = c.take<int>(ni + 1); a.slot_obs = c.take<int>(nsl); per_obs = c.take<int>(4 * nsl);
            csr = c.take<int>(2 * nsl + nf + ni + 2); a.W = c.take<double>(12 * nf); a.G = c.take<double>(12 * ni);
        }))
        return fail(ASL_ENOMEM, "map workspace allocation failed");
    a.obs = (const ObsRec *)d_obs; a.n_frames = n_frames; a.max_tags = max_tags; a.n_ids = n_ids; a.world_req = world_id;
    a.seen = per_id; a.id_tag = per_id + (ni + 1); a.tag_id = per_id + 2 * (ni + 1); a.tmp = per_id + 3 * (ni + 1);
    a.fr_npart = per_frame; a.fr_cam = per_frame + (nf + 1); a.fr_obs0 = per_frame + 2 * (nf + 1);
    a.cam_frame = per_cam; a.cam_ptr0 = per_cam + (nf + 1); a.cam_state = per_cam + 2 * (nf + 1); a.cam_seed = per_cam + 3 * (nf + 1);
    a.obs_slot = per_obs; a.obs_cam = per_obs + nsl; a.obs_tag = per_obs + 2 * nsl; a.obs_act = per_obs + 3 * nsl;
    a.cam_obs = csr; a.tag_obs = csr + nsl; a.cam_ptr = csr + 2 * nsl; a.tag_ptr = csr + 2 * nsl + nf + 1;
    const CamDev cam = make_cam(d, K, dist, n_dist, tag_size);

    hipLaunchKernelGGL(k_map_gather, dim3(1), dim3(MAP_WG), 0, st, a);
    MapHead h;
    HIPCHK(hipMemcpyAsync(&h, a.head, sizeof h, hipMemcpyDeviceToHost, st));
    HIPCHK(hipStreamSynchronize(st));
    const int NC = h.n_cams, NT = h.n_tags, NM = h.n_obs, WT = h.world_tag;
    auto finish_nothing = [&]() {
        hipLaunchKernelGGL(k_map_finish, dim3(1), dim3(MAP_WG), 0, st, a, NC, NT, NM, WT, 1, (const double *)nullptr, (const double *)nullptr,
                           (const double *)nullptr, (const double *)nullptr, (const int *)nullptr, (MapTagRec *)d_map, (double *)d_std, (CamPoseRec *)d_poses,
                           (MapResultRec *)d_result);
        HIPCHK(hipGetLastError());
        return ASL_OK;
    };
    if (NT > MAP_MAX_TAGS) return fail(ASL_EINVAL, "the frames see %d tags; the map's dense reduced system takes at most %d", NT, MAP_MAX_TAGS);
    if (WT < 0) {
        int rc = finish_nothing();
        if (rc) return rc;
        if (world_id >= 0) return fail(ASL_EINVAL, "world tag %d is not seen by any frame with 2 or more taking-part slots", world_id);
        return ASL_OK;
    }

    const int n = 6 * NT;
    const size_t nc = (size_t)NC, nt = (size_t)NT, nm = (size_t)NM;
    GnSystem sys = {nullptr, nullptr, a.cam_obs, nullptr, a.tag_obs, a.obs_cam, a.obs_tag, nullptr, NC, NT, WT};
    GnLmBufs b;
    double *seed_obs, *var;
    if (carve_ws(d->map_lm, [&](WsCarve &c) {
            b = gn_lm_carve(c, sys, NM, 2 * MAP_LM__N);
            seed_obs = c.take<double>(nm); var = c.take<double>(n); sys.cam_ptr = c.take<int>(nc + 1); sys.tag_ptr = c.take<int>(nt + 1);
        }))
        return fail(ASL_ENOMEM, "map workspace allocation failed");
    a.obs_of = sys.obs_of;
    double *lm = b.lm, *lm0 = lm + MAP_LM__N;
    const dim3 wg(MAP_WG);

    range_push("map: seed");
    HIPCHK(hipMemsetAsync(a.obs_of, 0xff, 4 * nc * nt, st));
    hipLaunchKernelGGL(k_map_table, dim3((NM + 255) / 256), dim3(256), 0, st, a, NM, NT);
    hipLaunchKernelGGL(k_map_csr, dim3(1), wg, 0, st, a, NC, NT);
    hipLaunchKernelGGL(k_map_chain, dim3(1), wg, 0, st, a, NC, NT, NM, WT);
    hipLaunchKernelGGL(k_map_csr, dim3(1), wg, 0, st, a, NC, NT);
    for (int sw = 0; sw < 2; sw++) {
        hipLaunchKernelGGL(k_map_sweep_cam, dim3(NC), dim3(ASL_WAVE), loc_lds_bytes(max_tags), st, a, cam);
        hipLaunchKernelGGL(k_map_sweep_tag, dim3(NT), dim3(ASL_WAVE), 0, st, a, cam);
    }
    hipLaunchKernelGGL(k_map_gauge, dim3(1), wg, 0, st, a, NC, NT, WT);
    hipLaunchKernelGGL(k_map_flip, dim3(NT), dim3(ASL_WAVE), 0, st, a, cam, WT);
    hipLaunchKernelGGL(k_map_behind, dim3((NC + 63) / 64), dim3(64), 0, st, a, NC, cam.half);
    hipLaunchKernelGGL(k_map_csr, dim3(1), wg, 0, st, a, NC, NT);
    hipLaunchKernelGGL(k_map_lm_init, dim3(1), dim3(1), 0, st, (const MapHead *)a.head, lm, lm0);
    HIPCHK(hipMemsetAsync(b.flag, 0, 8, st));
    range_pop();

    range_push("map: LM");
    auto lin = [&](const double *W, const double *G, double *D, int force) {
        hipLaunchKernelGGL(k_map_linearize, dim3((NM + 3) / 4), dim3(256), 0, st, a, W, G, NM, cam, D, b.cost_obs, lm, force);
    };
    auto decide = [&]() { hipLaunchKernelGGL(k_map_decide, dim3(1), dim3(1), 0, st, lm, b.flag); };
    auto park = [&]() {
        hipLaunchKernelGGL(k_map_park, dim3((NC + NT + 2 + 255) / 256), dim3(256), 0, st, lm, sys.cam_ptr, NC, sys.tag_ptr, NT);
    };
    HIPCHK(hipMemcpyAsync(sys.cam_ptr, a.cam_ptr, 4 * (nc + 1), hipMemcpyDeviceToDevice, st));
    HIPCHK(hipMemcpyAsync(sys.tag_ptr, a.tag_ptr, 4 * (nt + 1), hipMemcpyDeviceToDevice, st));
    int rc = gn_lm_run(sys, b, a.W, a.G, NM, max_iters, seed_obs, lin, decide, park, st);
    if (rc) return rc;
    lin(a.W, a.G, sys.D, 1);
    range_pop();
    if (d_std) {
        GnSystem full = sys;
        full.cam_ptr = a.cam_ptr;
        full.tag_ptr = a.tag_ptr;
        rc = gn_factor_step(full, lm0, b.flag + 1, st);
        if (rc) return rc;
        hipLaunchKernelGGL(k_map_std, dim3(n), dim3(256), (size_t)n * sizeof(double), st, sys.S, sys.Linv, n, var);
    }
    hipLaunchKernelGGL(k_map_finish, dim3(1), wg, 0, st, a, NC, NT, NM, WT, 0, lm, b.cost_obs, seed_obs, d_std ? var : nullptr, b.flag + 1,
                       (MapTagRec *)d_map, (double *)d_std, (CamPoseRec *)d_poses, (MapResultRec *)d_result);
    HIPCHK(hipGetLastError());
    return ASL_OK;
}

extern "C" int asl_map_frames_device(asl_detector *d, const void *d_obs, int n_frames, int max_tags, int n_ids, const double *K, const double *dist,
                                     int n_dist, double tag_size, int world_id, int max_iters, void *d_map, void *d_tag_std, void *d_poses,
                                     void *d_result, void *stream)
{
    if (!d) return fail(ASL_EINVAL, "NULL detector");
    int rc = check_map_args(d_obs, n_frames, max_tags, n_ids, K, dist, n_dist, tag_size, world_id, max_iters, d_map, d_poses, d_result);
    if (rc) return rc;
    HIPCHK(hipSetDevice(d->device));
    return launch_map(d, d_obs, n_frames, max_tags, n_ids, K, dist, n_dist, tag_size, world_id, max_iters, d_map, d_tag_std, d_poses, d_result,
                      (hipStream_t)stream);
}

extern "C" int asl_map_batch(asl_detector *d, const asl_obs *obs, int n_frames, int max_tags, int n_ids, const double *K, const double *dist,
                             int n_dist, double tag_size, int world_id, int max_iters, asl_map_tag *map, double *tag_std, asl_cam_pose *poses,
                             asl_map_result *result)
{
    if (!d) return fail(ASL_EINVAL, "NULL detector");
    int rc = check_map_args(obs, n_frames, max_tags, n_ids, K, dist, n_dist, tag_size, world_id, max_iters, map, poses, result);
    if (rc) return rc;
    HIPCHK(hipSetDevice(d->device));
    asl_map_result *d_result;
    asl_map_tag *d_map;
    double *d_std;
    asl_cam_pose *d_poses;
    if (carve_ws(d->solve_out, [&](WsCarve &c) {
            d_result = c.take<asl_map_result>(1); d_map = c.take<asl_map_tag>(n_ids); d_std = c.take<double>(6 * (size_t)n_ids);
            d_poses = c.take<asl_cam_pose>(n_frames);
        }))
        return fail(ASL_ENOMEM, "map workspace allocation failed");
    if ((rc = upload_obs(d, "map", obs, n_frames, max_tags, nullptr, n_ids))) return rc;
    rc = launch_map(d, d->loc_obs.p, n_frames, max_tags, n_ids, K, dist, n_dist, tag_size, world_id, max_iters, d_map, tag_std ? d_std : nullptr,
                    d_poses, d_result, nullptr);
    if (rc) return rc;
    HIPCHK(hipMemcpy(result, d_result, sizeof(asl_map_result), hipMemcpyDeviceToHost));
    HIPCHK(hipMemcpy(map, d_map, sizeof(asl_map_tag) * (size_t)n_ids, hipMemcpyDeviceToHost));
    if (tag_std) HIPCHK(hipMemcpy(tag_std, d_std, sizeof(double) * 6 * (size_t)n_ids, hipMemcpyDeviceToHost));
    HIPCHK(hipMemcpy(poses, d_poses, sizeof(asl_cam_pose) * (size_t)n_frames, hipMemcpyDeviceToHost));
    return ASL_OK;
}

#include "debug_host.inc"
```

aprilslam_amd/csrc/asl_common.h:

```cpp
#pragma once
#include <hip/hip_runtime.h>
#include <stdint.h>

#define ASL_WAVE 64
#define TILESZ 4
#define MIN_WHITE_BLACK_DIFF 5
#define MIN_COMPONENT 25u
#define MAX_NMAXIMA 10
#define MAX_LINE_FIT_MSE 10.0
#define COS_CRITICAL_RAD 0.984807753012208
#define HASH_EMPTY 0xFFFFFFFFFFFFFFFFull
#define HASH_MAX_PROBE 512
#define NCLASSES 5
#define CLASS0_CAP 128
#define CLASS1_CAP 256
#define CLASS2_CAP 512
#define CLASS3_CAP 1024

template <typename T>
struct DevBuf {
    T *p = nullptr;
    size_t n = 0;
    DevBuf() = default;
    DevBuf(const DevBuf &) = delete;
    DevBuf &operator=(const DevBuf &) = delete;
    ~DevBuf() { release(); }
    int ensure(size_t want)
    {
        if (want <= n) return 0;
        release();
        hipError_t e = hipMalloc((void **)&p, want * sizeof(T));
        if (e != hipSuccess) { p = nullptr; return -1; }
        n = want;
        return 0;
    }
    void release() { if (p) (void)hipFree(p); p = nullptr; n = 0; }
};

template <typename T>
struct PinnedBuf {
    T *p = nullptr;
    size_t n = 0;
    PinnedBuf() = default;
    PinnedBuf(const PinnedBuf &) = delete;
    PinnedBuf &operator=(const PinnedBuf &) = delete;
    ~PinnedBuf() { release(); }
    hipError_t ensure(size_t want, unsigned int flags)
    {
        if (want <= n) return hipSuccess;
        release();
        hipError_t e = hipHostMalloc((void **)&p, want * sizeof(T), flags);
        if (e != hipSuccess) { p = nullptr; return e; }
        n = want;
        return hipSuccess;
    }
    void release() { if (p) (void)hipHostFree(p); p = nullptr; n = 0; }
};

struct WsCarve {
    uintptr_t base = 0;
    size_t off = 0;
    size_t take(size_t bytes) { const size_t o = off; off += (bytes + 255) & ~(size_t)255; return o; }
    template <typename T>
    T *take(size_t n) { return (T *)(base + take(sizeof(T) * n)); }
};

template <class Carve>
static int carve_ws(DevBuf<uint8_t> &buf, Carve carve)
{
    WsCarve c;
    carve(c);
    if (buf.ensure(c.off)) return -1;
    c = WsCarve{(uintptr_t)buf.p};
    carve(c);
    return 0;
}

struct Geom {
    int w, h;
    int stride;
    int channels;
    int f;
    int sw, sh;
    int tw, th;
    int nframes;
    size_t frame_pitch;
    size_t npix;
};

struct ClusterRec {
    uint64_t key;
    unsigned int offset;
    unsigned int count;
    unsigned int fill;
    unsigned int pad;
};

struct QuadRec {
    double p[4][2];
    uint64_t key;
    int valid;
    int reversed_border;
};

struct DetRec {
    int32_t id, hamming;
    float margin;
    int32_t frame;
    double center[2];
    double corners[4][2];
    uint64_t key;
    double rvec[3], tvec[3], T[16];
    int32_t pose_ok, pad;
};

#define IDX_BUCKET_BITS 12
#define IDX_BUCKETS (1 << IDX_BUCKET_BITS)
#define IDX_MAX_CHUNKS 4
struct FamilyDev {
    int nbits, width_at_border, total_width, reversed_border, ncodes;
    int bit_x[64], bit_y[64];
    const unsigned long long *codes;
    int idx_nch;
    int idx_lo[IDX_MAX_CHUNKS], idx_w[IDX_MAX_CHUNKS];
    const unsigned short *idx_start;
    const unsigned long long *idx_entries;
};
__host__ __device__ __forceinline__ unsigned int idx_bucket(unsigned long long chunk_value, int width)
{
    return width <= IDX_BUCKET_BITS ? (unsigned int)chunk_value : (unsigned int)((chunk_value * 0x9E3779B97F4A7C15ull) >> (64 - IDX_BUCKET_BITS));
}

struct CamDev {
    double fx, fy, cx, cy, k1, k2, p1, p2, k3;
    double half;
    int both_minima;
    int pad;
};

enum {
    CNT_NCLUSTERS = 0,
    CNT_OVERFLOW_HASH = 1,
    CNT_OVERFLOW_POINTS = 2,
    CNT_OVERFLOW_CLUSTERS = 3,
    CNT_OVERFLOW_DETS = 4,
    CNT_UF_GUARD = 5,
    CNT_DEDUP_LIMIT = 6,
    CNT_NPOINTS = 16,
    CNT_CLASS0 = 32,
    CNT_NDETS = 112,
    CNT_NQUADS = 128,
    CNT_NKEEP = 144,
    CNT_DENSE_TILES = 160,
    CNT_DENSE_SEG = 161,
    CNT__N = 176
};
#define CNT_CLASS(c) (CNT_CLASS0 + 16 * (c))

struct Recip {
    double d, r;
};
__device__ __forceinline__ Recip recip_of(double d)
{
    double r = __builtin_amdgcn_rcp(d);
    double e = __builtin_fma(-d, r, 1.0);
    r = __builtin_fma(r, e, r);
    e = __builtin_fma(-d, r, 1.0);
    r = __builtin_fma(r, e, r);
    return Recip{d, r};
}
__device__ __forceinline__ double div_by(double a, const Recip &k)
{
    const double q = a * k.r;
    const double rem = __builtin_fma(-k.d, q, a);
    return __builtin_fma(rem, k.r, q);
}

__device__ __forceinline__ bool batch_poisoned(const long long *counters)
{
    return (counters[CNT_OVERFLOW_HASH] | counters[CNT_OVERFLOW_POINTS] | counters[CNT_OVERFLOW_CLUSTERS] | counters[CNT_OVERFLOW_DETS]) != 0;
}

#define PHASE_SPREAD 512
__device__ unsigned long long g_phase_cycles[64 * PHASE_SPREAD];
#ifdef ASL_PHASE_TIMING
#define PHASE_DECL()                                                                  \
    __shared__ unsigned long long ph_s__[16];                                         \
    long long ph_t__ = 0;                                                             \
    if (threadIdx.x == 0 && threadIdx.y == 0)                                         \
        for (int ph_i__ = 0; ph_i__ < 16; ph_i__++) ph_s__[ph_i__] = 0
#define PHASE_INIT() ph_t__ = clock64()
#define PHASE(k)                                                                      \
    do {                                                                              \
        if (threadIdx.x == 0 && threadIdx.y == 0) {                                   \
            long long now__ = clock64();                                              \
            ph_s__[(k) & 15] += (unsigned long long)(now__ - ph_t__);                 \
            ph_t__ = now__;                                                           \
        }                                                                             \
    } while (0)
#define PHASE_COUNT(k, v) do { if (threadIdx.x == 0 && threadIdx.y == 0) ph_s__[(k) & 15] += (unsigned long long)(v); } while (0)
#define PHASE_FLUSH(base)                                                             \
    do {                                                                              \
        if (threadIdx.x == 0 && threadIdx.y == 0)                                     \
            for (int ph_i__ = 0; ph_i__ < 16; ph_i__++)                               \
                if (ph_s__[ph_i__]) atomicAdd(&g_phase_cycles[((base) + ph_i__) * PHASE_SPREAD + ((blockIdx.x + 7u * blockIdx.y + 13u * blockIdx.z) & (PHASE_SPREAD - 1))], ph_s__[ph_i__]); \
    } while (0)
#else
#define PHASE_DECL() do {} while (0)
#define PHASE_INIT() do {} while (0)
#define PHASE(k) do {} while (0)
#define PHASE_COUNT(k, v) do {} while (0)
#define PHASE_FLUSH(base) do {} while (0)
#endif

template <int CH>
__device__ __forceinline__ unsigned int pixel_fetch(const uint8_t *frame, const Geom &g, int x, int y, unsigned int *shift)
{
    if (CH == 1) { *shift = 0; return frame[(unsigned int)y * (unsigned int)g.stride + (unsigned int)x]; }
    const unsigned int sh = (x + 1 < g.w) ? 0u : 1u;
    unsigned int u;
    __builtin_memcpy(&u, frame + ((unsigned int)y * (unsigned int)g.stride + 3u * (unsigned int)x - sh), 4);
    *shift = 8u * sh;
    return u;
}

__device__ __forceinline__ int bgr_gray(unsigned int u)
{
    const unsigned int hi = __builtin_amdgcn_udot4(u, 0x00264B0Eu, 0u, false), lo = __builtin_amdgcn_udot4(u, 0x00462397u, 16384u, false);
    return (int)(((hi << 8) + lo) >> 15);
}

template <int CH>
__device__ __forceinline__ int pixel_gray(unsigned int u, unsigned int shift)
{
    if (CH == 1) return (int)u;
    return bgr_gray(u >> shift);
}

template <int CH>
__device__ __forceinline__ int gray_at(const uint8_t *frame, const Geom &g, int x, int y)
{
    unsigned int sh;
    unsigned int u = pixel_fetch<CH>(frame, g, x, y, &sh);
    return pixel_gray<CH>(u, sh);
}
```

aprilslam_amd/csrc/debug_host.inc:

```

__global__ void __launch_bounds__(256) k_div_check(unsigned long long seed, int per_thread, int lim, unsigned long long *bad)
{
    unsigned long long s = seed + 0x9E3779B97F4A7C15ull * (blockIdx.x * (unsigned long long)blockDim.x + threadIdx.x + 1);
    auto rng = [&]() { s ^= s << 13; s ^= s >> 7; s ^= s << 17; return s; };
    for (int i = 0; i < 8; i++) rng();
    unsigned long long nbad = 0;
    for (int i = 0; i < per_thread; i++) {
        const unsigned long long u = rng(), v = rng(), w = rng();
        const int ea = (int)(u % (unsigned)(2 * lim + 1)) - lim, ed = (int)((u >> 20) % (unsigned)(2 * lim + 1)) - lim;
        double a = ldexp(1.0 + (double)(v & 0xFFFFFFFFFFFFFull) * 0x1p-52, ea);
        double dd = ldexp(1.0 + (double)(w & 0xFFFFFFFFFFFFFull) * 0x1p-52, ed);
        if (u & (1ull << 60)) a = -a;
        if (u & (1ull << 61)) dd = -dd;
        if ((u >> 40) % 257 == 0) a = 0.0;
        const double want = a / dd, got = div_by(a, recip_of(dd));
        if (__double_as_longlong(want) != __double_as_longlong(got)) nbad++;
    }
    if (nbad) atomicAdd(bad, nbad);
}

static int expand_thresh(asl_detector *d, const Geom &g, size_t total)
{
    if (d->dbg_thresh.ensure(total)) return fail(ASL_ENOMEM, "debug buffer allocation failed");
    hipLaunchKernelGGL(k_seg_debug_thresh, dim3((g.sw + 63) / 64, (g.sh + 3) / 4, (unsigned int)g.nframes), dim3(64, 4), 0, nullptr,
                       d->wmask.p, d->bmask.p, g, seg_nwx(g), d->dbg_thresh.p);
    HIPCHK(hipGetLastError());
    return ASL_OK;
}

extern "C" int asl_debug_fetch(asl_detector *d, int what, void *dst, size_t bytes, size_t *n_items)
{
    if (!d || !dst || !n_items) return fail(ASL_EINVAL, "NULL argument");
    HIPCHK(hipSetDevice(d->device));
    const Geom &g = d->last;
    size_t total = (size_t)g.nframes * g.npix;
    if (what >= 0 && what <= 3 && total == 0) return fail(ASL_EINVAL, "no batch has run yet");
    switch (what) {
    case 0: {
        if (bytes < total) return fail(ASL_EINVAL, "dst too small: need %zu bytes", total);
        HIPCHK(hipMemcpy(dst, d->dgray.p, total, hipMemcpyDeviceToHost));
        *n_items = total;
        return ASL_OK;
    }
    case 1: {
        if (bytes < total) return fail(ASL_EINVAL, "dst too small: need %zu bytes", total);
        if (int rc = expand_thresh(d, g, total)) return rc;
        HIPCHK(hipMemcpy(dst, d->dbg_thresh.p, total, hipMemcpyDeviceToHost));
        *n_items = total;
        return ASL_OK;
    }
    case 2: {
        if (bytes < total * 4) return fail(ASL_EINVAL, "dst too small: need %zu bytes", total * 4);
        if (d->dbg_labels.ensure(total)) return fail(ASL_ENOMEM, "debug buffer allocation failed");
        hipLaunchKernelGGL(k_seg_debug_labels, dim3((g.sw + 63) / 64, (g.sh + 3) / 4, (unsigned int)g.nframes), dim3(64, 4), 0, nullptr,
                           d->wmask.p, d->bmask.p, g, seg_nwx(g), d->parent.p, d->dbg_labels.p);
        HIPCHK(hipGetLastError());
        HIPCHK(hipMemcpy(dst, d->dbg_labels.p, total * 4, hipMemcpyDeviceToHost));
        *n_items = total;
        return ASL_OK;
    }
    case 3: {
        if (bytes < total * 4) return fail(ASL_EINVAL, "dst too small: need %zu bytes", total * 4);
        if (int rc = expand_thresh(d, g, total)) return rc;
        std::vector<uint8_t> th(total);
        HIPCHK(hipMemcpy(th.data(), d->dbg_thresh.p, total, hipMemcpyDeviceToHost));
        HIPCHK(hipMemcpy(dst, d->sizes.p, total * 4, hipMemcpyDeviceToHost));
        unsigned int *o = (unsigned int *)dst;
        for (size_t i = 0; i < total; i++)
            if (th[i] == 127) o[i] = 1u;
        *n_items = total;
        return ASL_OK;
    }
    case 4: {
        size_t ncl = (size_t)std::min<long long>(d->last_counters[CNT_NCLUSTERS], (long long)d->max_clusters);
        std::vector<QuadRec> q(ncl);
        if (ncl) HIPCHK(hipMemcpy(q.data(), d->quads.p, ncl * sizeof(QuadRec), hipMemcpyDeviceToHost));
        const size_t nvalid = (size_t)std::count_if(q.begin(), q.end(), [](const QuadRec &r) { return r.valid != 0; });
        if (bytes < nvalid * sizeof(asl_debug_quad))
            return fail(ASL_EINVAL, "dst too small: need %zu bytes for %zu quads", nvalid * sizeof(asl_debug_quad), nvalid);
        std::sort(q.begin(), q.end(), [](const QuadRec &a, const QuadRec &b) { return a.key < b.key; });
        asl_debug_quad *o = (asl_debug_quad *)dst;
        size_t k = 0;
        for (size_t i = 0; i < ncl; i++) {
            if (!q[i].valid) continue;
            for (int a = 0; a < 4; a++) { o[k].p[a][0] = q[i].p[a][0]; o[k].p[a][1] = q[i].p[a][1]; }
            unsigned long long key = q[i].key;
            o[k].frame = (int)(key >> 48);
            o[k].cluster = (((key >> 24) & 0xFFFFFFull) << 32) + (key & 0xFFFFFFull);
            o[k].reversed_border = q[i].reversed_border;
            k++;
        }
        *n_items = k;
        return ASL_OK;
    }
    case 5: {
        if (bytes < sizeof(long long) * 18) return fail(ASL_EINVAL, "dst too small: need %zu bytes", sizeof(long long) * 18);
        long long *o = (long long *)dst;
        o[0] = g.nframes; o[1] = g.sw; o[2] = g.sh;
        o[3] = d->last_counters[CNT_NCLUSTERS]; o[4] = d->last_counters[CNT_NPOINTS]; o[5] = d->last_counters[CNT_NQUADS];
        o[6] = d->last_counters[CNT_NDETS]; o[7] = d->nslots; o[8] = d->max_clusters; o[9] = d->max_points; o[10] = d->max_dets;
        o[11] = d->last_counters[CNT_OVERFLOW_HASH]; o[12] = d->last_counters[CNT_OVERFLOW_CLUSTERS];
        o[13] = d->last_counters[CNT_OVERFLOW_POINTS]; o[14] = d->last_counters[CNT_OVERFLOW_DETS]; o[15] = d->last_counters[CNT_CLASS0];
        o[16] = d->last_counters[CNT_DENSE_TILES]; o[17] = d->last_counters[CNT_DENSE_SEG];
        *n_items = 18;
        return ASL_OK;
    }
    case 6: {
        size_t ncl = (size_t)std::min<long long>(d->last_counters[CNT_NCLUSTERS], (long long)d->max_clusters);
        size_t npts = (size_t)std::min<long long>(d->last_counters[CNT_NPOINTS], (long long)d->max_points);
        if (bytes < ncl * 24) return fail(ASL_EINVAL, "dst too small: need %zu bytes", ncl * 24);
        std::vector<ClusterRec> cl(ncl);
        std::vector<unsigned long long> pts(npts);
        if (ncl) HIPCHK(hipMemcpy(cl.data(), d->clusters.p, ncl * sizeof(ClusterRec), hipMemcpyDeviceToHost));
        if (npts) HIPCHK(hipMemcpy(pts.data(), d->points.p, npts * sizeof(unsigned long long), hipMemcpyDeviceToHost));
        std::sort(cl.begin(), cl.end(), [](const ClusterRec &a, const ClusterRec &b) { return a.key < b.key; });
        unsigned long long *o = (unsigned long long *)dst;
        for (size_t i = 0; i < ncl; i++) {
            unsigned long long h = 0xcbf29ce484222325ull;
            if ((size_t)cl[i].offset + cl[i].count <= npts) {
                std::sort(pts.begin() + cl[i].offset, pts.begin() + cl[i].offset + cl[i].count);
                for (unsigned int k = 0; k < cl[i].count; k++) { h ^= pts[(size_t)cl[i].offset + k]; h *= 0x100000001b3ull; }
            }
            o[3 * i] = cl[i].key; o[3 * i + 1] = cl[i].count; o[3 * i + 2] = h;
        }
        *n_items = ncl;
        return ASL_OK;
    }
    default:
        return fail(ASL_EINVAL, "unknown debug item %d", what);
    }
}

extern "C" int asl_debug_refit(asl_detector *d, int reps, int64_t *out, size_t n_out)
{
    if (!d || !out) return fail(ASL_EINVAL, "NULL argument");
    if (reps < 1) return fail(ASL_EINVAL, "reps must be >= 1 (got %d)", reps);
    if (n_out < 2 + NCLASSES) return fail(ASL_EINVAL, "out too small: need %d values (got %zu)", 2 + NCLASSES, n_out);
    if (d->pending) return fail(ASL_EINVAL, "a batch is in flight on this detector");
    size_t ncl = (size_t)std::min<long long>(d->last_counters[CNT_NCLUSTERS], (long long)d->max_clusters);
    if (!ncl) return fail(ASL_EINVAL, "no clusters in the last batch");
    HIPCHK(hipSetDevice(d->device));
    const Geom &g = d->last;
    std::vector<QuadRec> ref(ncl), cur(ncl);
    std::vector<ClusterRec> cl(ncl);
    HIPCHK(hipMemcpy(cl.data(), d->clusters.p, ncl * sizeof(ClusterRec), hipMemcpyDeviceToHost));
    for (int k = 0; k < 2 + NCLASSES; k++) out[k] = 0;
    for (int r = 0; r < reps; r++) {
        for (int cls = 0; cls < NCLASSES - 1; cls++) launch_fit_class(d, g, cls, (unsigned int)g.nframes, nullptr);
        launch_quad_finish(d, g, nullptr);
        HIPCHK(hipGetLastError());
        HIPCHK(hipMemcpy((r ? cur : ref).data(), d->quads.p, ncl * sizeof(QuadRec), hipMemcpyDeviceToHost));
        if (!r) continue;
        for (size_t i = 0; i < ncl; i++) {
            const bool same = cur[i].valid == ref[i].valid && (!ref[i].valid || memcmp(cur[i].p, ref[i].p, sizeof ref[i].p) == 0);
            if (same) continue;
            const unsigned int cnt = cl[i].count;
            if (cnt > CLASS3_CAP) continue;
            out[1]++;
            out[2 + (cnt <= CLASS0_CAP ? 0 : (cnt <= CLASS1_CAP ? 1 : (cnt <= CLASS2_CAP ? 2 : (cnt <= CLASS3_CAP ? 3 : 4))))]++;
        }
    }
    out[0] = reps;
    return ASL_OK;
}

extern "C" int asl_debug_division_check(asl_detector *d, int exponent_limit, int64_t *out, size_t n_out)
{
    if (!d || !out) return fail(ASL_EINVAL, "NULL argument");
    if (exponent_limit < 1 || exponent_limit > 900) return fail(ASL_EINVAL, "exponent_limit must be in [1, 900] (got %d)", exponent_limit);
    if (n_out < 2) return fail(ASL_EINVAL, "out too small: need 2 values (got %zu)", n_out);
    HIPCHK(hipSetDevice(d->device));
    const int blocks = 2048, per = 1024;
    DevBuf<unsigned long long> d_bad;
    if (d_bad.ensure(1)) return fail(ASL_ENOMEM, "debug buffer allocation failed");
    HIPCHK(hipMemset(d_bad.p, 0, sizeof(unsigned long long)));
    hipLaunchKernelGGL(k_div_check, dim3(blocks), dim3(256), 0, nullptr, 20260301ull, per, exponent_limit, d_bad.p);
    HIPCHK(hipGetLastError());
    unsigned long long h_bad = 0;
    HIPCHK(hipMemcpy(&h_bad, d_bad.p, sizeof h_bad, hipMemcpyDeviceToHost));
    out[0] = (int64_t)blocks * 256 * per;
    out[1] = (int64_t)h_bad;
    return ASL_OK;
}

extern "C" int asl_debug_phase_cycles(asl_detector *d, unsigned long long *out, size_t n_out, int reset)
{
    if (!d || !out) return fail(ASL_EINVAL, "NULL argument");
    if (n_out < 64) return fail(ASL_EINVAL, "out too small: need 64 values (got %zu)", n_out);
    HIPCHK(hipSetDevice(d->device));
    std::vector<unsigned long long> all((size_t)64 * PHASE_SPREAD);
    HIPCHK(hipMemcpyFromSymbol(all.data(), HIP_SYMBOL(g_phase_cycles), sizeof(unsigned long long) * all.size()));
    for (int i = 0; i < 64; i++) {
        out[i] = 0;
        for (int k = 0; k < PHASE_SPREAD; k++) out[i] += all[(size_t)i * PHASE_SPREAD + k];
    }
    if (reset) {
        std::fill(all.begin(), all.end(), 0ull);
        HIPCHK(hipMemcpyToSymbol(HIP_SYMBOL(g_phase_cycles), all.data(), sizeof(unsigned long long) * all.size()));
    }
    return ASL_OK;
}
```

aprilslam_amd/csrc/k_seg.inc:

```

#define SEG_TH 32
#define SEG_PH 63

__device__ __forceinline__ unsigned long long seg_join_mask(int x0, int sw)
{
    unsigned long long m = ~0ull;
    if (x0 == 0) m &= ~1ull;
    const int last = sw - 2 - x0;
    if (last < 0) return 0ull;
    if (last < 63) m &= (2ull << last) - 1ull;
    return m;
}

__device__ __forceinline__ unsigned long long seg_exist_mask(int x0, int sw)
{
    const int n = sw - x0;
    return n >= 64 ? ~0ull : ((1ull << n) - 1ull);
}

__device__ __forceinline__ unsigned long long seg_starts(unsigned long long M, unsigned long long J) { return M & ~((M << 1) & J); }

__device__ __forceinline__ int seg_start_of(unsigned long long S, int x)
{
    return 63 - __clzll((long long)(S & (~0ull >> (63 - x))));
}

__device__ __forceinline__ int seg_run_len(unsigned long long M, unsigned long long J, int sx)
{
    const unsigned long long cont = (M >> 1) & (J >> 1);
    return 1 + __ffsll((long long)~(cont >> sx)) - 1;
}

__device__ __forceinline__ unsigned int seg_writelane(unsigned int old, unsigned int val, int lane)
{
#if __HIP_DEVICE_COMPILE__
    asm("v_writelane_b32 %0, %1, %2" : "+v"(old) : "s"(val), "i"(lane));
    return old;
#else
    (void)val; (void)lane;
    return old;
#endif
}

__device__ __forceinline__ void seg_wave_sync()
{
    __builtin_amdgcn_fence(__ATOMIC_SEQ_CST, "wavefront");
    __builtin_amdgcn_wave_barrier();
}

#define SEG_LW 65
#define SEG_LN (SEG_TH * SEG_LW)
__device__ __forceinline__ unsigned int seg_lrow(unsigned int i) { return (i * 2017u) >> 17; }

__device__ __forceinline__ unsigned int seg_lds_load(const unsigned int *L, unsigned int a)
{
    return __hip_atomic_load(&L[a], __ATOMIC_RELAXED, __HIP_MEMORY_SCOPE_WORKGROUP) & 0xFFFFu;
}

__device__ __forceinline__ void seg_lds_find2(const unsigned int *L, unsigned int &a, unsigned int &b)
{
    unsigned int pa = seg_lds_load(L, a), pb = seg_lds_load(L, b);
    int guard = 0;
    while ((pa != a || pb != b) && guard++ < 4096) {
        a = pa; b = pb;
        pa = seg_lds_load(L, a); pb = seg_lds_load(L, b);
    }
}

__device__ __forceinline__ bool seg_lds_union(unsigned int *L, unsigned int a, unsigned int b)
{
    for (int guard = 0; guard < 4096; guard++) {
        seg_lds_find2(L, a, b);
        if (a == b) return true;
        if (a < b) { unsigned int t = a; a = b; b = t; }
        unsigned int old = atomicMin(&L[a], b);
        if (old == a) return true;
        a = old;
    }
    return false;
}

__global__ void __launch_bounds__(256) k_tile_cut(const uint8_t *__restrict__ tmin, const uint8_t *__restrict__ tmax, Geom g,
                                                  uint8_t *__restrict__ tcut)
{
    const int tw = g.tw, th = g.th, gx = (tw + 3) >> 2, gy = (th + 3) >> 2;
    const int i = blockIdx.x * 256 + threadIdx.x, fr = blockIdx.y;
    if (i >= gx * gy) return;
    const int by = i / gx, t0 = (i - by * gx) * 4, y0 = by * 4;
    const uint8_t *pmin = tmin + (size_t)fr * tw * th, *pmax = tmax + (size_t)fr * tw * th;
    uint8_t *out = tcut + (size_t)fr * tw * th + t0;
    if (t0 + 4 <= tw) {
        const bool first = t0 == 0, last = t0 + 4 >= tw;
        unsigned int hmn[6], hmx[6];
#pragma unroll
        for (int r = 0; r < 6; r++) {
            const unsigned int row = (unsigned int)min(max(y0 - 1 + r, 0), th - 1) * (unsigned int)tw;
            unsigned long long a, b;
            __builtin_memcpy(&a, pmin + row + t0 - (first ? 0 : 1), 8);
            __builtin_memcpy(&b, pmax + row + t0 - (first ? 0 : 1), 8);
            if (first) { a = (a << 8) | (a & 255ull); b = (b << 8) | (b & 255ull); }
            if (last) { a = (a & ~(255ull << 40)) | (((a >> 32) & 255ull) << 40); b = (b & ~(255ull << 40)) | (((b >> 32) & 255ull) << 40); }
            unsigned int pn = 0, px = 0;
#pragma unroll
            for (int k = 0; k < 4; k++) {
                const unsigned int n0 = (unsigned int)(a >> (8 * k)) & 255u, n1 = (unsigned int)(a >> (8 * k + 8)) & 255u, n2 = (unsigned int)(a >> (8 * k + 16)) & 255u;
                const unsigned int x0 = (unsigned int)(b >> (8 * k)) & 255u, x1 = (unsigned int)(b >> (8 * k + 8)) & 255u, x2 = (unsigned int)(b >> (8 * k + 16)) & 255u;
                pn |= min(min(n0, n1), n2) << (8 * k);
                px |= max(max(x0, x1), x2) << (8 * k);
            }
            hmn[r] = pn; hmx[r] = px;
        }
#pragma unroll
        for (int r = 0; r < 4; r++) {
            if (y0 + r >= th) break;
            unsigned int packed = 0;
#pragma unroll
            for (int k = 0; k < 4; k++) {
                const unsigned int mn = min(min((hmn[r] >> (8 * k)) & 255u, (hmn[r + 1] >> (8 * k)) & 255u), (hmn[r + 2] >> (8 * k)) & 255u);
                const unsigned int mx = max(max((hmx[r] >> (8 * k)) & 255u, (hmx[r + 1] >> (8 * k)) & 255u), (hmx[r + 2] >> (8 * k)) & 255u);
                packed |= (mx - mn < (unsigned int)MIN_WHITE_BLACK_DIFF ? 255u : mn + (mx - mn) / 2u) << (8 * k);
            }
            __builtin_memcpy(out + (size_t)(y0 + r) * tw, &packed, 4);
        }
        return;
    }
    for (int ty = y0; ty < min(y0 + 4, th); ty++)
        for (int tx = t0; tx < tw; tx++) {
            int mn = 255, mx = 0;
            for (int dy = -1; dy <= 1; dy++) {
                const int yy = min(max(ty + dy, 0), th - 1);
                for (int dx = -1; dx <= 1; dx++) {
                    const int xx = min(max(tx + dx, 0), tw - 1);
                    mn = min(mn, (int)pmin[yy * tw + xx]);
                    mx = max(mx, (int)pmax[yy * tw + xx]);
                }
            }
            out[(size_t)ty * tw + tx - t0] = (uint8_t)(mx - mn < MIN_WHITE_BLACK_DIFF ? 255 : mn + (mx - mn) / 2);
        }
}

#ifndef SEG_TILE_WAVES
#define SEG_TILE_WAVES 4
#endif
#define SEG_CAP 512

__device__ __forceinline__ unsigned long long seg_upto(int x) { return ~0ull >> (63 - x); }

__device__ __forceinline__ unsigned long long seg_threshold_tile(const uint8_t *__restrict__ dg, const uint8_t *__restrict__ tc, const Geom &g, int x0, int y0, int lane)
{
    const int sw = g.sw, sh = g.sh;
    const int seg = lane & 3, rq = lane >> 2;
    const int xs = x0 + 16 * seg;
    const bool whole = xs + 16 <= sw;
    uint4 px[2];
    unsigned int cut[2][4];
#pragma unroll
    for (int hf = 0; hf < 2; hf++) {
        const unsigned int yy = (unsigned int)min(y0 + 16 * hf + rq, sh - 1);
        const unsigned int trow = (unsigned int)min((int)yy / TILESZ, g.th - 1) * (unsigned int)g.tw;
#pragma unroll
        for (int q = 0; q < 4; q++) cut[hf][q] = tc[trow + (unsigned int)min((xs >> 2) + q, g.tw - 1)];
    }
#pragma unroll
    for (int hf = 0; hf < 2; hf++) {
        const unsigned int yy = (unsigned int)min(y0 + 16 * hf + rq, sh - 1);
        const uint8_t *row = dg + (size_t)yy * (unsigned int)sw;
        if (whole) {
            px[hf] = *reinterpret_cast<const uint4 *>(row + xs);
        } else {
            unsigned int d[4] = {0, 0, 0, 0};
            for (int k = 0; k < 16; k++) d[k >> 2] |= (unsigned int)row[min(xs + k, sw - 1)] << (8 * (k & 3));
            px[hf] = make_uint4(d[0], d[1], d[2], d[3]);
        }
    }
    const unsigned int cmin = min(min(min(cut[0][0], cut[0][1]), min(cut[0][2], cut[0][3])), min(min(cut[1][0], cut[1][1]), min(cut[1][2], cut[1][3])));
    if (__ballot(cmin != 255u) == 0ull) return 0ull;
    unsigned int xlo[2], xhi[2];
#pragma unroll
    for (int hf = 0; hf < 2; hf++) {
        const unsigned int d[4] = {px[hf].x, px[hf].y, px[hf].z, px[hf].w};
        unsigned int wbits = 0, cbits = 0;
#pragma unroll
        for (int q = 0; q < 4; q++) {
            const unsigned int c = cut[hf][q];
            if (c != 255u) cbits |= 0xFu << (4 * q);
#pragma unroll
            for (int k = 0; k < 4; k++) wbits |= (((d[q] >> (8 * k)) & 255u) > c ? 1u : 0u) << (4 * q + k);
        }
        const int left = sw - xs;
        cbits &= left >= 16 ? 0xFFFFu : (left <= 0 ? 0u : (1u << left) - 1u);
        wbits &= cbits;
        const unsigned int pk = wbits | ((cbits & ~wbits) << 16);
        const unsigned int q0 = quad_bcast<0>(pk), q1 = quad_bcast<1>(pk), q2 = quad_bcast<2>(pk), q3 = quad_bcast<3>(pk);
        const bool blk = (seg & 1) != 0;
        xlo[hf] = blk ? ((q0 >> 16) | (q1 & 0xFFFF0000u)) : ((q0 & 0xFFFFu) | (q1 << 16));
        xhi[hf] = blk ? ((q2 >> 16) | (q3 & 0xFFFF0000u)) : ((q2 & 0xFFFFu) | (q3 << 16));
    }
    const int src = 4 * (lane & 15) + (lane >> 5);
    const bool second = (lane & 16) != 0;
    const unsigned int lo0 = (unsigned int)__shfl((int)xlo[0], src), hi0 = (unsigned int)__shfl((int)xhi[0], src);
    const unsigned int lo1 = (unsigned int)__shfl((int)xlo[1], src), hi1 = (unsigned int)__shfl((int)xhi[1], src);
    return ((unsigned long long)(second ? hi1 : hi0) << 32) | (second ? lo1 : lo0);
}

__global__ void __launch_bounds__(64 * SEG_TILE_WAVES) k_seg_tile(const uint8_t *__restrict__ dgray, const uint8_t *__restrict__ tcut, Geom g, int nwx, int ntiles,
                                                 unsigned long long *__restrict__ wmask, unsigned long long *__restrict__ bmask,
                                                 unsigned int *__restrict__ parent, unsigned int *__restrict__ sizes,
                                                 unsigned long long *__restrict__ rootmask, uint4 *__restrict__ edges, unsigned int *__restrict__ dense_list,
                                                 long long *counters)
{
    __shared__ unsigned int Ls[SEG_TILE_WAVES][SEG_CAP];
    __shared__ unsigned int WLs[SEG_TILE_WAVES][SEG_CAP];
    __shared__ unsigned long long RMKs[SEG_TILE_WAVES][SEG_TH];
    const int lane = threadIdx.x & 63, wave = threadIdx.x >> 6;
    unsigned int *const L = Ls[wave], *const WL = WLs[wave];
    unsigned long long *const RMK = RMKs[wave];
    const int tile = blockIdx.x * SEG_TILE_WAVES + wave, fr = blockIdx.z;
    if (tile >= ntiles) return;
    const int wx = tile % nwx, x0 = wx * 64, y0 = (tile / nwx) * SEG_TH;
    const int sw = g.sw, sh = g.sh;
    PHASE_DECL();
    PHASE_INIT();
    unsigned long long M = 0;
    if (g.tw > 0 && g.th > 0)
        M = seg_threshold_tile(dgray + (size_t)fr * g.npix, tcut + (size_t)fr * g.tw * g.th, g, x0, y0, lane);
    PHASE(2);
    const int r = lane & 31;
    const bool isw = lane < 32;
    const int y = y0 + r;
    if (y >= sh) M = 0;
    const size_t mi = ((size_t)fr * nwx + wx) * sh + y;
    if (y < sh) { if (isw) wmask[mi] = M; else bmask[mi] = M; }
    {
        const unsigned long long el = __ballot((M & 1ull) != 0ull), er = __ballot((M >> 63) != 0ull);
        if (lane == 0) edges[(size_t)fr * ntiles + tile] = make_uint4((unsigned int)el, (unsigned int)(el >> 32), (unsigned int)er, (unsigned int)(er >> 32));
    }
    PHASE(8);
    if (__ballot(M != 0) == 0ull) {
        if (isw && y < sh) rootmask[mi] = 0ull;
        PHASE_FLUSH(48);
        return;
    }
    const unsigned long long J = seg_join_mask(x0, sw);
    const unsigned long long S = seg_starts(M, J);
    unsigned long long Mp = __shfl_up(M, 1), Sp = __shfl_up(S, 1);
    if (r == 0) { Mp = 0; Sp = 0; }
    const unsigned long long U = M & Mp & J;
    unsigned long long link[3];
    link[0] = U & ~(U << 1);
    link[1] = isw ? (M & J & (Mp << 1) & ~Mp) : 0ull;
    link[2] = isw ? (M & J & (Mp >> 1) & ~(Mp & (J >> 1))) : 0ull;
    const unsigned int nlinks_lane = (unsigned int)(__popcll(link[0]) + __popcll(link[1]) + __popcll(link[2])), nruns_lane = (unsigned int)__popcll(S);
    const unsigned int incl = wave_scan<false>(nlinks_lane | (nruns_lane << 16), 0u, [](unsigned int a, unsigned int b) { return a + b; });
    const unsigned int tot = readlane(incl, 63);
    const int nlinks = (int)(tot & 0xFFFFu), nruns = (int)(tot >> 16);
    PHASE_COUNT(12, nlinks); PHASE_COUNT(13, nruns); PHASE_COUNT(14, 1);
    if (nlinks > SEG_CAP || nruns > SEG_CAP) {
        if (lane == 0) dense_list[atomicAdd((unsigned long long *)&counters[CNT_DENSE_SEG], 1ull)] = (unsigned int)fr * (unsigned int)ntiles + (unsigned int)tile;
        PHASE_FLUSH(48);
        return;
    }
    const unsigned int rb = (incl >> 16) - nruns_lane;
    const unsigned int rbp = (unsigned int)__shfl_up((int)rb, 1);
    for (int i = lane; i < nruns; i += 64) L[i] = (unsigned int)i;
    if (lane < SEG_TH) RMK[lane] = 0ull;
    {
        unsigned int j = (incl & 0xFFFFu) - nlinks_lane;
#pragma unroll
        for (int t = 0; t < 3; t++) {
            unsigned long long m = link[t];
            const int dx = t == 0 ? 0 : (t == 1 ? -1 : 1);
            while (m) {
                const int bx = __ffsll((long long)m) - 1;
                m &= m - 1;
                const unsigned int a = rb + (unsigned int)__popcll(S & seg_upto(bx)) - 1u;
                const unsigned int b = rbp + (unsigned int)__popcll(Sp & seg_upto(bx + dx)) - 1u;
                WL[j++] = a | (b << 16);
            }
        }
    }
    seg_wave_sync();
    PHASE(3);
    {
        bool bad = false;
        for (int i = lane; i < nlinks; i += 64) {
            const unsigned int e = WL[i];
            bad |= !seg_lds_union(L, e & 0xFFFFu, e >> 16);
        }
        if (bad) atomicAdd((unsigned long long *)&counters[CNT_UF_GUARD], 1ull);
    }
    seg_wave_sync();
    PHASE(9);
    {
        unsigned int j = rb;
        unsigned long long m = S;
        while (m) {
            const int sx = __ffsll((long long)m) - 1;
            m &= m - 1;
            WL[j++] = (unsigned int)r | ((unsigned int)sx << 5) | ((unsigned int)(seg_run_len(M, J, sx) - 1) << 11);
        }
    }
    seg_wave_sync();
    unsigned int *P = parent + (size_t)fr * g.npix;
    for (int i = lane; i < nruns; i += 128) {
        const bool two = i + 64 < nruns;
        const unsigned int i0 = (unsigned int)i, i1 = two ? i0 + 64u : i0;
        const unsigned int e0 = WL[i0], e1 = WL[i1];
        unsigned int r0 = i0, r1 = i1;
        seg_lds_find2(L, r0, r1);
        const unsigned int f0 = WL[r0], f1 = WL[r1];
        atomicAdd(&L[r0], ((e0 >> 11) + 1u) << 16);
        if (two) atomicAdd(&L[r1], ((e1 >> 11) + 1u) << 16);
        if (r0 != i0) L[i0] = r0; else atomicOr(&RMK[e0 & 31u], 1ull << ((e0 >> 5) & 63u));
        if (two) { if (r1 != i1) L[i1] = r1; else atomicOr(&RMK[e1 & 31u], 1ull << ((e1 >> 5) & 63u)); }
        P[(size_t)(y0 + (int)(e0 & 31u)) * sw + x0 + (int)((e0 >> 5) & 63u)] = (unsigned int)((y0 + (int)(f0 & 31u)) * sw + x0 + (int)((f0 >> 5) & 63u));
        if (two) P[(size_t)(y0 + (int)(e1 & 31u)) * sw + x0 + (int)((e1 >> 5) & 63u)] = (unsigned int)((y0 + (int)(f1 & 31u)) * sw + x0 + (int)((f1 >> 5) & 63u));
    }
    seg_wave_sync();
    PHASE(10);
    const unsigned long long rm = RMK[r];
    {
        unsigned int *SZ = sizes + (size_t)fr * g.npix;
        unsigned long long m = rm & S;
        while (m) {
            const int sx = __ffsll((long long)m) - 1;
            m &= m - 1;
            SZ[(size_t)y * sw + x0 + sx] = L[rb + (unsigned int)__popcll(S & seg_upto(sx)) - 1u] >> 16;
        }
    }
    if (isw && y < sh) rootmask[mi] = rm;
    PHASE(11);
    PHASE_FLUSH(48);
}

__global__ void __launch_bounds__(64) k_seg_tile_dense(Geom g, int nwx, int ntiles, const unsigned long long *__restrict__ wmask,
                                                       const unsigned long long *__restrict__ bmask, unsigned int *__restrict__ parent,
                                                       unsigned int *__restrict__ sizes, unsigned long long *__restrict__ rootmask,
                                                       const unsigned int *__restrict__ dense_list, long long *counters)
{
    __shared__ __attribute__((aligned(16))) unsigned int L[SEG_LN];
    const int lane = threadIdx.x & 63, r = lane & 31;
    const bool isw = lane < 32;
    const int sw = g.sw, sh = g.sh;
    const long long n = counters[CNT_DENSE_SEG];
    for (long long w = blockIdx.x; w < n; w += gridDim.x) {
        const unsigned int id = dense_list[w];
        const int fr = (int)(id / (unsigned int)ntiles), tile = (int)(id % (unsigned int)ntiles);
        const int wx = tile % nwx, x0 = wx * 64, y0 = (tile / nwx) * SEG_TH;
        const int y = y0 + r;
        const size_t mi = ((size_t)fr * nwx + wx) * sh + y;
        const unsigned long long M = y < sh ? (isw ? wmask[mi] : bmask[mi]) : 0ull;
        const unsigned long long J = seg_join_mask(x0, sw);
        const unsigned long long S = seg_starts(M, J);
        unsigned long long Mp = __shfl_up(M, 1), Sp = __shfl_up(S, 1);
        if (r == 0) { Mp = 0; Sp = 0; }
        seg_wave_sync();
#pragma unroll
        for (int k = 0; k < (SEG_LN + 255) / 256; k++) {
            const unsigned int i = (unsigned int)(k * 256 + 4 * lane);
            if (i < (unsigned int)SEG_LN) *reinterpret_cast<uint4 *>(&L[i]) = make_uint4(i, i + 1, i + 2, i + 3);
        }
        seg_wave_sync();
        const unsigned int rbase = (unsigned int)(r * SEG_LW);
        {
            const unsigned long long U = M & Mp & J;
            unsigned long long link[3];
            link[0] = U & ~(U << 1);
            link[1] = isw ? (M & J & (Mp << 1) & ~Mp) : 0ull;
            link[2] = isw ? (M & J & (Mp >> 1) & ~(Mp & (J >> 1))) : 0ull;
            bool bad = false;
#pragma unroll
            for (int t = 0; t < 3; t++) {
                unsigned long long m = link[t];
                const int dx = t == 0 ? 0 : (t == 1 ? -1 : 1);
                while (m) {
                    const int bx = __ffsll((long long)m) - 1;
                    m &= m - 1;
                    bad |= !seg_lds_union(L, rbase + (unsigned int)seg_start_of(S, bx), rbase - (unsigned int)SEG_LW + (unsigned int)seg_start_of(Sp, bx + dx));
                }
            }
            if (bad) atomicAdd((unsigned long long *)&counters[CNT_UF_GUARD], 1ull);
        }
        seg_wave_sync();
        unsigned int *P = parent + (size_t)fr * g.npix;
        unsigned long long rm = 0;
        {
            unsigned long long m = S;
            while (m) {
                const int sx0 = __ffsll((long long)m) - 1;
                m &= m - 1;
                const bool two = m != 0ull;
                const int sx1 = two ? __ffsll((long long)m) - 1 : sx0;
                if (two) m &= m - 1;
                const unsigned int i0 = rbase + (unsigned int)sx0, i1 = rbase + (unsigned int)sx1;
                unsigned int r0 = i0, r1 = i1;
                seg_lds_find2(L, r0, r1);
                atomicAdd(&L[r0], (unsigned int)seg_run_len(M, J, sx0) << 16);
                if (two) atomicAdd(&L[r1], (unsigned int)seg_run_len(M, J, sx1) << 16);
                if (r0 != i0) L[i0] = r0; else rm |= 1ull << sx0;
                if (two) { if (r1 != i1) L[i1] = r1; else rm |= 1ull << sx1; }
                const unsigned int q0 = seg_lrow(r0), q1 = seg_lrow(r1);
                P[(size_t)y * sw + x0 + sx0] = (unsigned int)((y0 + (int)q0) * sw + x0 + (int)(r0 - q0 * SEG_LW));
                if (two) P[(size_t)y * sw + x0 + sx1] = (unsigned int)((y0 + (int)q1) * sw + x0 + (int)(r1 - q1 * SEG_LW));
            }
        }
        seg_wave_sync();
        {
            unsigned int *SZ = sizes + (size_t)fr * g.npix;
            unsigned long long m = rm;
            while (m) {
                const int sx = __ffsll((long long)m) - 1;
                m &= m - 1;
                SZ[(size_t)y * sw + x0 + sx] = L[rbase + (unsigned int)sx] >> 16;
            }
        }
        rm |= __shfl_down(rm, 32);
        if (isw && y < sh) rootmask[mi] = rm;
    }
}

__device__ __forceinline__ bool seg_global_join(unsigned int *P, unsigned int a, unsigned int b)
{
    for (int guard = 0; guard < (1 << 16); guard++) {
        unsigned int pa = __hip_atomic_load(&P[a], __ATOMIC_RELAXED, __HIP_MEMORY_SCOPE_AGENT);
        unsigned int pb = __hip_atomic_load(&P[b], __ATOMIC_RELAXED, __HIP_MEMORY_SCOPE_AGENT);
        int hops = 0;
        while ((pa != a || pb != b) && hops++ < (1 << 22)) {
            a = pa; b = pb;
            pa = __hip_atomic_load(&P[a], __ATOMIC_RELAXED, __HIP_MEMORY_SCOPE_AGENT);
            pb = __hip_atomic_load(&P[b], __ATOMIC_RELAXED, __HIP_MEMORY_SCOPE_AGENT);
        }
        if (a == b) return true;
        if (a < b) { unsigned int t = a; a = b; b = t; }
        unsigned int old = atomicMin(&P[a], b);
        if (old == a) return true;
        a = old;
    }
    return false;
}

__device__ __forceinline__ void seg_border_cols_body(const unsigned long long *__restrict__ wmask, const unsigned long long *__restrict__ bmask,
                                                     const uint4 *__restrict__ edges, int ntiles, const Geom &g, int nwx,
                                                     unsigned int *__restrict__ parent, long long *counters, unsigned int blk)
{
    const int sw = g.sw, sh = g.sh;
    const size_t per_frame = (size_t)nwx * sh, seams = (size_t)(nwx - 1) * sh;
    const size_t i0 = (size_t)blk * 64 + threadIdx.x;
    const bool inrange = i0 < seams * g.nframes;
    const size_t i = inrange ? i0 : 0;
    const int fr = (int)(i / seams);
    const int rem = (int)(i - (size_t)fr * seams);
    const int wx = 1 + rem / sh, y = rem % sh, x0 = wx * 64;
    const unsigned long long *wm = wmask + (size_t)fr * per_frame, *bm = bmask + (size_t)fr * per_frame;
    const size_t m0 = (size_t)wx * sh + y;
    const size_t et = (size_t)fr * ntiles + (size_t)(y / SEG_TH) * nwx + wx;
    const uint4 ec = edges[et], el = edges[et - 1];
    const bool seam = inrange && ((((ec.x | ec.y) | (el.z | el.w)) >> (y % SEG_TH)) & 1u) != 0u;
    if (__ballot(seam) == 0ull) return;
    const bool diag = seam && y > 0 && (y % SEG_TH) != 0;
    const unsigned long long W = seam ? wm[m0] : 0ull, B = seam ? bm[m0] : 0ull, Wl = seam ? wm[m0 - sh] : 0ull, Bl = seam ? bm[m0 - sh] : 0ull;
    const unsigned long long Wp = diag ? wm[m0 - 1] : 0ull, Wlp = diag ? wm[m0 - sh - 1] : 0ull;
    unsigned int *P = parent + (size_t)fr * g.npix;
    const unsigned long long J = seam ? seg_join_mask(x0, sw) : 0ull, Jl = seam ? seg_join_mask(x0 - 64, sw) : 0ull;
    auto gidx = [&](int word, int yy, int bit) { return (unsigned int)(yy * sw + word * 64 + bit); };
    unsigned int ja[4], jb[4];
    bool jv[4] = {false, false, false, false};
    if (J & 1ull) {
        if ((W & 1ull) && (Wl >> 63)) { jv[0] = true; ja[0] = gidx(wx, y, 0); jb[0] = gidx(wx - 1, y, seg_start_of(seg_starts(Wl, Jl), 63)); }
        if ((B & 1ull) && (Bl >> 63)) { jv[1] = true; ja[1] = gidx(wx, y, 0); jb[1] = gidx(wx - 1, y, seg_start_of(seg_starts(Bl, Jl), 63)); }
        if ((W & 1ull) && (Wlp >> 63)) { jv[2] = true; ja[2] = gidx(wx, y, 0); jb[2] = gidx(wx - 1, y - 1, seg_start_of(seg_starts(Wlp, Jl), 63)); }
    }
    if ((Jl >> 63) && (Wl >> 63) && (Wp & 1ull)) { jv[3] = true; ja[3] = gidx(wx - 1, y, seg_start_of(seg_starts(Wl, Jl), 63)); jb[3] = gidx(wx, y - 1, 0); }
    bool ok = true;
#pragma unroll
    for (int t = 0; t < 4; t++) {
        if (jv[t]) {
            ja[t] = __hip_atomic_load(&P[ja[t]], __ATOMIC_RELAXED, __HIP_MEMORY_SCOPE_AGENT);
            jb[t] = __hip_atomic_load(&P[jb[t]], __ATOMIC_RELAXED, __HIP_MEMORY_SCOPE_AGENT);
        }
    }
#pragma unroll
    for (int t = 0; t < 4; t++) {
        const unsigned long long key = jv[t] ? (((unsigned long long)ja[t] << 32) | jb[t]) : ~0ull;
        const unsigned long long up = __shfl_up(key, 1);
        const bool dup = jv[t] && threadIdx.x > 0 && y > 0 && up == key;
        if (jv[t] && !dup) ok &= seg_global_join(P, ja[t], jb[t]);
    }
    if (!ok) atomicAdd((unsigned long long *)&counters[CNT_UF_GUARD], 1ull);
}

__device__ __forceinline__ void seg_border_rows_body(const unsigned long long *__restrict__ wmask, const unsigned long long *__restrict__ bmask,
                                                     const Geom &g, int nwx, unsigned int *__restrict__ parent, long long *counters, int wx, int rb, int fr)
{
    const int sw = g.sw, sh = g.sh;
    const int y = (rb + 1) * SEG_TH, x0 = wx * 64;
    const int bx = threadIdx.x;
    const size_t per_frame = (size_t)nwx * sh;
    const unsigned long long *wm = wmask + (size_t)fr * per_frame, *bm = bmask + (size_t)fr * per_frame;
    const size_t m0 = (size_t)wx * sh + y;
    const unsigned long long W = wm[m0], B = bm[m0], Wp = wm[m0 - 1], Bp = bm[m0 - 1];
    if ((W | B) == 0ull || (Wp | Bp) == 0ull) return;
    unsigned int *P = parent + (size_t)fr * g.npix;
    const unsigned long long J = seg_join_mask(x0, sw);
    const unsigned long long bit = 1ull << bx;
    auto gidx = [&](int word, int yy, int b) { return (unsigned int)(yy * sw + word * 64 + b); };
    bool ok = true;
    {
        const unsigned long long UW = W & Wp & J, UB = B & Bp & J;
        if (UW & ~(UW << 1) & bit) ok &= seg_global_join(P, gidx(wx, y, seg_start_of(seg_starts(W, J), bx)), gidx(wx, y - 1, seg_start_of(seg_starts(Wp, J), bx)));
        if (UB & ~(UB << 1) & bit) ok &= seg_global_join(P, gidx(wx, y, seg_start_of(seg_starts(B, J), bx)), gidx(wx, y - 1, seg_start_of(seg_starts(Bp, J), bx)));
    }
    if (W & J & bit) {
        const unsigned int me = gidx(wx, y, seg_start_of(seg_starts(W, J), bx));
        if (!((Wp >> bx) & 1ull)) {
            if (bx > 0) {
                if ((Wp >> (bx - 1)) & 1ull) ok &= seg_global_join(P, me, gidx(wx, y - 1, seg_start_of(seg_starts(Wp, J), bx - 1)));
            } else if (wx > 0) {
                const unsigned long long Wlp = wm[m0 - sh - 1];
                if (Wlp >> 63) ok &= seg_global_join(P, me, gidx(wx - 1, y - 1, seg_start_of(seg_starts(Wlp, seg_join_mask(x0 - 64, sw)), 63)));
            }
        }
        if (bx < 63) {
            if (((Wp >> (bx + 1)) & 1ull) && !(((Wp >> bx) & 1ull) && ((J >> (bx + 1)) & 1ull)))
                ok &= seg_global_join(P, me, gidx(wx, y - 1, seg_start_of(seg_starts(Wp, J), bx + 1)));
        } else if (wx + 1 < nwx) {
            const unsigned long long Wrp = wm[m0 + sh - 1];
            if ((Wrp & 1ull) && !((Wp >> 63) && (seg_join_mask(x0 + 64, sw) & 1ull))) ok &= seg_global_join(P, me, gidx(wx + 1, y - 1, 0));
        }
    }
    if (!ok) atomicAdd((unsigned long long *)&counters[CNT_UF_GUARD], 1ull);
}

__global__ void __launch_bounds__(64) k_seg_border(const unsigned long long *__restrict__ wmask, const unsigned long long *__restrict__ bmask,
                                                   const uint4 *__restrict__ edges, int ntiles, Geom g, int nwx, unsigned int *__restrict__ parent,
                                                   long long *counters, unsigned int ncol_blocks, int nrb)
{
    if (blockIdx.x < ncol_blocks) {
        seg_border_cols_body(wmask, bmask, edges, ntiles, g, nwx, parent, counters, blockIdx.x);
    } else {
        const unsigned int r = blockIdx.x - ncol_blocks;
        const unsigned int t = r / (unsigned int)nwx;
        seg_border_rows_body(wmask, bmask, g, nwx, parent, counters, (int)(r - t * (unsigned int)nwx), (int)(t % (unsigned int)nrb), (int)(t / (unsigned int)nrb));
    }
}

__global__ void __launch_bounds__(256) k_seg_roots(const unsigned long long *__restrict__ rootmask, Geom g, int nwx,
                                                   unsigned int *__restrict__ parent, unsigned int *__restrict__ sizes)
{
    const size_t per_frame = (size_t)nwx * g.sh;
    const size_t i = (size_t)blockIdx.x * blockDim.x + threadIdx.x;
    if (i >= per_frame * g.nframes) return;
    unsigned long long w = rootmask[i];
    if (!w) return;
    const int fr = (int)(i / per_frame);
    const int rem = (int)(i - (size_t)fr * per_frame);
    const int wx = rem / g.sh, y = rem - wx * g.sh;
    unsigned int *P = parent + (size_t)fr * g.npix;
    unsigned int *S = sizes + (size_t)fr * g.npix;
    while (w) {
        const int b = __ffsll((long long)w) - 1;
        w &= w - 1;
        const unsigned int p = (unsigned int)(y * g.sw + wx * 64 + b);
        const unsigned int sp = S[p];
        const unsigned int root = uf_find(P, p);
        if (root != p) {
            atomicAdd(&S[root], sp);
            P[p] = root;
        }
    }
}

#define SEGP_NSLOT 256
#define SEGP_NW 4
#define SEGP_RUNCAP 2048
#define SEGP_RUNCAP_DENSE 4352
#define SEGP_PCAP 4096
#define SEGP_PCAP_DENSE 8192

template <int PCAP, int RUNCAP, int NW, int NHALF>
__global__ void __launch_bounds__(64 * NW) k_seg_points(const unsigned long long *__restrict__ wmask, const unsigned long long *__restrict__ bmask,
                                                        Geom g, int nwx, const unsigned int *__restrict__ labels, const unsigned int *__restrict__ sizes,
                                                        unsigned long long *keys, unsigned int *counts, unsigned int hmask,
                                                        unsigned long long *stage_rec, unsigned int *stage_pos, unsigned int *frame_cursor,
                                                        unsigned int stage_cap, unsigned int *dense_tiles, int tiles_y, long long *counters)
{
    constexpr bool DENSE = NHALF > 1;
    constexpr int NSLOT = SEGP_NSLOT, NT = 64 * NW;
    __shared__ unsigned int RT[RUNCAP];
    __shared__ unsigned long long ROWS[NT];
    __shared__ unsigned int ROWB[NT];
    __shared__ unsigned long long BK[NSLOT];
    __shared__ unsigned int BC[NSLOT];
    __shared__ __attribute__((aligned(8))) unsigned int PT[PCAP];
    static_assert(PCAP >= 3 * NT, "the small-run masks borrow the parking space");
    unsigned long long *const SML = reinterpret_cast<unsigned long long *>(PT);
    unsigned int *const EFL = PT + 2 * NT;
    __shared__ unsigned int s_npts, s_base, s_wtot[NW];
    const int tid = threadIdx.x, lane = tid & 63, wid = tid >> 6;
    const int sw = g.sw, sh = g.sh;
    const size_t per_frame = (size_t)nwx * sh;
    PHASE_DECL();
    const long long ndense = DENSE ? counters[CNT_DENSE_TILES] : 1;
  for (long long work = DENSE ? blockIdx.x : 0; work < ndense; work += DENSE ? gridDim.x : 1) {
    int wx, ty, fr;
    if (DENSE) {
        __syncthreads();
        const unsigned int tile_id = dense_tiles[work];
        wx = (int)(tile_id % (unsigned int)nwx);
        ty = (int)((tile_id / (unsigned int)nwx) % (unsigned int)tiles_y);
        fr = (int)(tile_id / (unsigned int)(nwx * tiles_y));
    } else {
        fr = blockIdx.x; ty = blockIdx.z; wx = (int)blockIdx.y * NW + wid;
    }
    const unsigned int my_tile_id = (unsigned int)((fr * tiles_y + ty) * nwx + wx);
    const int x0 = wx * 64, y0 = ty * SEG_PH;
    const int y = y0 + lane;
    const bool rowok = y < sh && wx < nwx;
    const unsigned long long *wm = wmask + (size_t)fr * per_frame, *bm = bmask + (size_t)fr * per_frame;
    const unsigned int *lab = labels + (size_t)fr * g.npix, *siz = sizes + (size_t)fr * g.npix;
    PHASE_INIT();
    const size_t m0 = (size_t)wx * sh + y;
    unsigned long long W = 0, B = 0;
    bool wl = false, bl = false, wr = false, br = false;
    unsigned long long SL = 0;
    if (rowok) {
        W = wm[m0]; B = bm[m0];
        if (wx > 0) {
            const unsigned long long Wl = wm[m0 - sh], Bl = bm[m0 - sh];
            wl = Wl >> 63; bl = Bl >> 63;
            if (wl || bl) SL = seg_starts(wl ? Wl : Bl, seg_join_mask(x0 - 64, sw));
        }
        if (wx + 1 < nwx) { wr = wm[m0 + sh] & 1ull; br = bm[m0 + sh] & 1ull; }
    }
    const bool tile_live = __ballot((W | B) != 0ull) != 0ull;
    if (!DENSE) {
        if (!__syncthreads_or(tile_live ? 1 : 0)) return;
    }
    const unsigned long long J = seg_join_mask(x0, sw);
    const unsigned long long Sall = seg_starts(W, J) | seg_starts(B, J);
    const bool havel = wl || bl, haver = wr || br;
    const int nown = __popcll(Sall);
    const int cnt = tile_live ? nown + (havel ? 1 : 0) + (haver ? 1 : 0) : 0;
    int incl = cnt;
#pragma unroll
    for (int off = 1; off < 64; off <<= 1) {
        int o = __shfl_up(incl, off);
        if (lane >= off) incl += o;
    }
    if (lane == 63) s_wtot[wid] = (unsigned int)incl;
    __syncthreads();
    int base = incl - cnt, total = 0;
#pragma unroll
    for (int w = 0; w < NW; w++) {
        if (w < wid) base += (int)s_wtot[w];
        total += (int)s_wtot[w];
    }
    SML[tid] = 0ull;
    EFL[tid] = 0u;
    ROWS[tid] = Sall;
    ROWB[tid] = (unsigned int)base | ((unsigned int)nown << 13) | (havel ? 1u << 20 : 0u);
    if (total > RUNCAP) {
        if (lane == 0 && tile_live) dense_tiles[atomicAdd((unsigned long long *)&counters[CNT_DENSE_TILES], 1ull)] = my_tile_id;
        return;
    }
    if (tile_live) {
        unsigned long long m = Sall;
        int j = base;
        const unsigned int tag = (unsigned int)(lane << 6) | ((unsigned int)wid << 14);
        while (m) {
            const int sx = __ffsll((long long)m) - 1;
            m &= m - 1;
            RT[j++] = tag | (unsigned int)sx;
        }
        if (havel) RT[j++] = tag | (unsigned int)seg_start_of(SL, 63) | (1u << 12);
        if (haver) RT[j++] = tag | (2u << 12);
    }
    __syncthreads();
    PHASE(32);
    for (int i0 = 0; i0 < total; i0 += 4 * NT) {
        unsigned int e[4], l[4], s[4];
#pragma unroll
        for (int u = 0; u < 4; u++) {
            const int i = i0 + u * NT + tid;
            e[u] = i < total ? RT[i] : 0xFFFFFFFFu;
            const int kind = (int)((e[u] >> 12) & 3u), ew = DENSE ? 0 : (int)((e[u] >> 14) & 3u);
            const int ex0 = DENSE ? x0 : ((int)blockIdx.y * NW + ew) * 64;
            const unsigned int p = (unsigned int)((y0 + (int)((e[u] >> 6) & 63u)) * sw + ex0 + (kind == 1 ? -64 : (kind == 2 ? 64 : 0)) + (int)(e[u] & 63u));
            l[u] = e[u] != 0xFFFFFFFFu ? lab[p] : 0u;
        }
#pragma unroll
        for (int u = 0; u < 4; u++) l[u] = e[u] != 0xFFFFFFFFu ? lab[l[u]] : 0u;
#pragma unroll
        for (int u = 0; u < 4; u++) s[u] = e[u] != 0xFFFFFFFFu ? siz[l[u]] : MIN_COMPONENT;
#pragma unroll
        for (int u = 0; u < 4; u++) {
            const int i = i0 + u * NT + tid;
            if (e[u] == 0xFFFFFFFFu) continue;
            const bool small = s[u] < MIN_COMPONENT;
            RT[i] = l[u] | (small ? 0x80000000u : 0u);
            if (small) {
                const int row = (int)((e[u] >> 6) & 63u) + 64 * (int)((e[u] >> 14) & 3u), kind = (int)((e[u] >> 12) & 3u);
                if (kind == 0) {
                    const int sx = (int)(e[u] & 63u);
                    atomicOr(reinterpret_cast<unsigned int *>(&SML[row]) + (sx >> 5), 1u << (sx & 31));
                } else
                    atomicOr(&EFL[row], (unsigned int)kind);
            }
        }
    }
    __syncthreads();
    PHASE(33);
    {
        unsigned long long m = SML[tid];
        while (m) {
            const int sx = __ffsll((long long)m) - 1;
            m &= m - 1;
            const bool white = (W >> sx) & 1ull;
            const int len = seg_run_len(white ? W : B, J, sx);
            const unsigned long long bits = (len >= 64 ? ~0ull : ((1ull << len) - 1ull)) << sx;
            if (white) W &= ~bits; else B &= ~bits;
        }
        const unsigned int ef = EFL[tid];
        if (ef & 1u) { wl = false; bl = false; }
        if (ef & 2u) { wr = false; br = false; }
    }
    const unsigned long long Wn = __shfl_down(W, 1), Bn = __shfl_down(B, 1);
    const int fl = (wl ? 1 : 0) | (bl ? 2 : 0) | (wr ? 4 : 0) | (br ? 8 : 0);
    const int fln = __shfl_down(fl, 1);
    const bool wln = fln & 1, bln = fln & 2, wrn = fln & 4, brn = fln & 8;
    auto label_at = [&](int trow, int xx) -> unsigned int {
        const unsigned int rb = ROWB[trow];
        const int b = (int)(rb & 0x1FFFu), no = (int)((rb >> 13) & 0x7Fu);
        int j;
        if (xx < 0) j = b + no;
        else if (xx > 63) j = b + no + (int)((rb >> 20) & 1u);
        else j = b + __popcll(ROWS[trow] & (~0ull >> (63 - xx))) - 1;
        return RT[j] & 0x7FFFFFFFu;
    };
    const unsigned long long Wsr = (W >> 1) | ((unsigned long long)wr << 63), Bsr = (B >> 1) | ((unsigned long long)br << 63);
    const unsigned long long Wnsr = (Wn >> 1) | ((unsigned long long)wrn << 63), Bnsr = (Bn >> 1) | ((unsigned long long)brn << 63);
    const unsigned long long Wnsl = (Wn << 1) | (unsigned long long)wln, Bnsl = (Bn << 1) | (unsigned long long)bln;
#pragma unroll 1
  for (int half = 0; half < NHALF; half++) {
    const int rlo = NHALF == 1 ? 0 : half * 32, rhi = NHALF == 1 ? SEG_PH - 1 : min(half * 32 + 31, SEG_PH - 1);
    if (half > 0) __syncthreads();
    if (tid == 0) s_npts = 0;
    for (int i = tid; i < NSLOT; i += NT) { BK[i] = HASH_EMPTY; BC[i] = 0; }
    __syncthreads();
    const unsigned long long V = (lane >= rlo && lane <= rhi && y >= 1 && y <= sh - 2) ? J : 0ull;
    const unsigned long long E0 = ((W & Bsr) | (B & Wsr)) & V;
    const unsigned long long E1 = ((W & Bn) | (B & Wn)) & V;
    const unsigned long long E3 = ((W & Bnsr) | (B & Wnsr)) & V;
    unsigned long long E2 = ((W & Bnsl) | (B & Wnsl)) & V;
    {
        unsigned long long cl = E3 << 1;
        if (x0 >= 64 && ((wl && (Bn & 1ull)) || (bl && (Wn & 1ull)))) cl |= 1ull;
        E2 &= ~cl;
    }
    unsigned long long any = E0 | E1 | E2 | E3;
    const unsigned int npts_lane = (unsigned int)(__popcll(E0) + __popcll(E1) + __popcll(E2) + __popcll(E3));
    {
        const unsigned int nitems_lane = (unsigned int)__popcll(any);
        unsigned int ib = 0, pi = 0;
        if (nitems_lane) {
            const unsigned int old = atomicAdd(&s_npts, nitems_lane | (npts_lane << 16));
            ib = old & 0xFFFFu; pi = old >> 16;
        }
        const unsigned int rowtag = ((unsigned int)lane << 6) | ((unsigned int)wid << 12);
#pragma unroll
        for (int hf = 0; hf < 2; hf++) {
            unsigned int a = (unsigned int)(any >> (32 * hf));
            const unsigned int e0 = (unsigned int)(E0 >> (32 * hf)), e1 = (unsigned int)(E1 >> (32 * hf)), e2 = (unsigned int)(E2 >> (32 * hf)),
                               e3 = (unsigned int)(E3 >> (32 * hf)), bb = (unsigned int)(B >> (32 * hf));
            while (a) {
                const int b = __ffs((int)a) - 1;
                a &= a - 1;
                const unsigned int m = ((e0 >> b) & 1u) | (((e1 >> b) & 1u) << 1) | (((e2 >> b) & 1u) << 2) | (((e3 >> b) & 1u) << 3);
                if (pi < (unsigned int)PCAP) PT[ib] = (unsigned int)(b + 32 * hf) | rowtag | (m << 14) | (((bb >> b) & 1u) << 18) | (pi << 19);
                ib++;
                pi += (unsigned int)__popc(m);
            }
        }
    }
    __syncthreads();
    PHASE(37);
    const unsigned int packed = s_npts;
    const unsigned int nitems = packed & 0xFFFFu, npts = packed >> 16;
    if (npts <= (unsigned int)PCAP && nitems > 0) {
#pragma unroll 1
        for (int rd = (int)((nitems - 1u) / (unsigned int)NT); rd >= 0; rd--) {
            const unsigned int i = (unsigned int)rd * (unsigned int)NT + (unsigned int)tid;
            const bool have = i < nitems;
            const unsigned int e = have ? PT[i] : 0u;
            __syncthreads();
            if (!have) continue;
            const int lx = (int)(e & 63u), trow = (int)((e >> 6) & 255u);
            unsigned int m = (e >> 14) & 15u, pidx = e >> 19;
            const unsigned int rb0 = ROWB[trow], rb1 = ROWB[trow + 1];
            const unsigned long long S0 = ROWS[trow], S1 = ROWS[trow + 1];
            const int b0 = (int)(rb0 & 0x1FFFu), n0 = (int)((rb0 >> 13) & 0x7Fu), b1 = (int)(rb1 & 0x1FFFu), n1 = (int)((rb1 >> 13) & 0x7Fu);
            const unsigned long long upto = ~0ull >> (63 - lx);
            const int j0 = b0 + __popcll(S0 & upto) - 1;
            const int j00 = lx == 63 ? b0 + n0 + (int)((rb0 >> 20) & 1u) : b0 + __popcll(S0 & ((upto << 1) | 1ull)) - 1;
            const int j10 = b1 + __popcll(S1 & upto) - 1;
            const int j11 = lx == 0 ? b1 + n1 : b1 + __popcll(S1 & (upto >> 1)) - 1;
            const int j12 = lx == 63 ? b1 + n1 + (int)((rb1 >> 20) & 1u) : b1 + __popcll(S1 & ((upto << 1) | 1ull)) - 1;
            const unsigned int rep0 = RT[j0] & 0x7FFFFFFFu;
            unsigned int rep1[4];
            rep1[0] = RT[(m & 1u) ? j00 : j0] & 0x7FFFFFFFu;
            rep1[1] = RT[(m & 2u) ? j10 : j0] & 0x7FFFFFFFu;
            rep1[2] = RT[(m & 4u) ? j11 : j0] & 0x7FFFFFFFu;
            rep1[3] = RT[(m & 8u) ? j12 : j0] & 0x7FFFFFFFu;
            const unsigned int where = (e & 0xFFFu) | (((e >> 18) & 1u) << 14) | (((e >> 12) & 3u) << 15);
            while (m) {
                const unsigned int rr = (m & 1u) ? rep1[0] : ((m & 2u) ? rep1[1] : ((m & 4u) ? rep1[2] : rep1[3]));
                const unsigned int grp = m & ((rep1[0] == rr ? 1u : 0u) | (rep1[1] == rr ? 2u : 0u) | (rep1[2] == rr ? 4u : 0u) | (rep1[3] == rr ? 8u : 0u));
                m &= ~grp;
                const unsigned int hi = rep0 > rr ? rep0 : rr, lo = rep0 > rr ? rr : rep0;
                const unsigned long long key = ((unsigned long long)fr << 48) | ((unsigned long long)hi << 24) | lo;
                unsigned int h = hi ^ ((lo << 11) | (lo >> 21));
                h ^= h >> 15;
                h ^= h >> 7;
                h &= (unsigned int)(NSLOT - 1);
                if (h == (unsigned int)(NSLOT - 1)) h = (unsigned int)(NSLOT / 2 - 1);
                unsigned int slot = NSLOT - 1;
#pragma unroll 1
                for (int probe = 0; probe < NSLOT - 1; probe++) {
                    unsigned long long cur = __hip_atomic_load(&BK[h], __ATOMIC_RELAXED, __HIP_MEMORY_SCOPE_WORKGROUP);
                    if (cur == key) { slot = h; break; }
                    if (cur == HASH_EMPTY) {
                        unsigned long long old = atomicCAS(&BK[h], HASH_EMPTY, key);
                        if (old == HASH_EMPTY || old == key) { slot = h; break; }
                    }
                    h = h + 1 == (unsigned int)(NSLOT - 1) ? 0u : h + 1;
                }
                if (slot != (unsigned int)(NSLOT - 1)) atomicAdd(&BC[slot], (unsigned int)__popc(grp));
                const unsigned int word = where | (slot << 17);
#pragma unroll
                for (int k = 0; k < 4; k++)
                    if (grp & (1u << k)) PT[pidx++] = word | ((unsigned int)k << 12);
            }
        }
    }
    __syncthreads();
    PHASE(34);
    if (npts > (unsigned int)PCAP) {
        if (!DENSE) {
            if (lane == 0 && tile_live) dense_tiles[atomicAdd((unsigned long long *)&counters[CNT_DENSE_TILES], 1ull)] = my_tile_id;
            return;
        }
        if (tid == 0) atomicAdd((unsigned long long *)&counters[CNT_OVERFLOW_POINTS], 1ull);
        continue;
    }
    if (npts == 0) continue;
    for (int i = tid; i < NSLOT - 1; i += NT) {
        const unsigned int c = BC[i];
        if (c) {
            int gslot = hash_insert(keys, hmask, BK[i]);
            unsigned int bg = 0xFFFFFFFFu, bb = 0u;
            if (gslot < 0) atomicAdd((unsigned long long *)&counters[CNT_OVERFLOW_HASH], 1ull);
            else { bg = (unsigned int)gslot; bb = atomicAdd(&counts[gslot], c); }
            BK[i] = (unsigned long long)bg | ((unsigned long long)bb << 32);
            BC[i] = 0u;
        }
    }
    if (tid == NT - 1) {
        unsigned int b = atomicAdd(&frame_cursor[fr], npts);
        if (b + npts > stage_cap) { atomicAdd((unsigned long long *)&counters[CNT_OVERFLOW_POINTS], 1ull); b = 0xFFFFFFFFu; }
        s_base = b;
    }
    __syncthreads();
    PHASE(35);
    const unsigned int tbase = s_base;
    if (tbase == 0xFFFFFFFFu) continue;
    uint2 *const srec = reinterpret_cast<uint2 *>(stage_rec) + ((size_t)fr * stage_cap + tbase);
    unsigned int *const spos = stage_pos + ((size_t)fr * stage_cap + tbase);
    for (unsigned int i = tid; i < npts; i += NT) {
        const unsigned int w = PT[i];
        const int lx = (int)(w & 63u), ly = (int)((w >> 6) & 63u), k = (int)((w >> 12) & 3u), pw = (int)((w >> 15) & 3u);
        const bool black = (w >> 14) & 1u;
        const unsigned int slot = w >> 17;
        const int dx = k == 0 ? 1 : (k == 1 ? 0 : (k == 2 ? -1 : 1)), dy = k == 0 ? 0 : 1;
        const int px0 = DENSE ? x0 : ((int)blockIdx.y * NW + pw) * 64;
        unsigned int gslot, pos;
        if (slot == (unsigned int)(NSLOT - 1)) {
            int gs = hash_insert(keys, hmask, cluster_key(fr, label_at(pw * 64 + ly, lx), label_at(pw * 64 + ly + dy, lx + dx)));
            gslot = gs < 0 ? 0xFFFFFFFFu : (unsigned int)gs;
            pos = gs < 0 ? 0u : atomicAdd(&counts[gs], 1u);
            if (gs < 0) atomicAdd((unsigned long long *)&counters[CNT_OVERFLOW_HASH], 1ull);
        } else {
            const unsigned long long gb = BK[slot];
            gslot = (unsigned int)gb;
            pos = (unsigned int)(gb >> 32) + atomicAdd(&BC[slot], 1u);
        }
        const bool good = gslot != 0xFFFFFFFFu;
        const unsigned int cpos = black ? 1u : 2u, cneg = 3u - cpos;
        const unsigned int cgx = dx == 0 ? 0u : (dx > 0 ? cpos : cneg), cgy = dy == 0 ? 0u : cpos;
        uint2 rec;
        rec.x = good ? ((unsigned int)(2 * (px0 + lx) + dx) | ((unsigned int)(2 * (y0 + ly) + dy) << 16)) : 0xFFFFFFFFu;
        rec.y = good ? (cgx | (cgy << 2) | (gslot << (POINT_BITS - 32))) : 0xFFFFFFFFu;
        srec[i] = rec;
        spos[i] = good ? pos : 0u;
    }
    PHASE(36);
  }
  }
    PHASE_FLUSH(32);
}

__global__ void __launch_bounds__(256) k_seg_debug_thresh(const unsigned long long *__restrict__ wmask, const unsigned long long *__restrict__ bmask,
                                                          Geom g, int nwx, uint8_t *__restrict__ thresh)
{
    const int x = blockIdx.x * 64 + threadIdx.x, y = blockIdx.y * 4 + threadIdx.y, fr = blockIdx.z;
    if (x >= g.sw || y >= g.sh) return;
    const size_t mi = ((size_t)fr * nwx + (x >> 6)) * g.sh + y;
    const unsigned long long W = wmask[mi], B = bmask[mi];
    thresh[(size_t)fr * g.npix + (size_t)y * g.sw + x] = ((W >> (x & 63)) & 1ull) ? 255 : (((B >> (x & 63)) & 1ull) ? 0 : 127);
}

__global__ void __launch_bounds__(256) k_seg_debug_labels(const unsigned long long *__restrict__ wmask, const unsigned long long *__restrict__ bmask,
                                                          Geom g, int nwx, const unsigned int *__restrict__ parent, unsigned int *__restrict__ out)
{
    const int x = blockIdx.x * 64 + threadIdx.x, y = blockIdx.y * 4 + threadIdx.y, fr = blockIdx.z;
    if (x >= g.sw || y >= g.sh) return;
    const int wx = x >> 6, b = x & 63;
    const size_t mi = ((size_t)fr * nwx + wx) * g.sh + y;
    const unsigned long long W = wmask[mi], B = bmask[mi];
    const unsigned int p = (unsigned int)(y * g.sw + x);
    unsigned int l = p;
    if (((W | B) >> b) & 1ull) {
        const unsigned long long J = seg_join_mask(wx * 64, g.sw);
        const unsigned long long S = seg_starts(((W >> b) & 1ull) ? W : B, J);
        l = uf_find(parent + (size_t)fr * g.npix, (unsigned int)(y * g.sw + wx * 64 + seg_start_of(S, b)));
    }
    out[(size_t)fr * g.npix + p] = l;
}
```

Baseline: 382,000.

## Compact active segmentation tiles into work lists and launch persistent loops over them

Adds a pre-pass that marks labelling tiles whose threshold cuts are not all flat and compacts them, and the point-group units touching them, into device lists with atomic counters. The seg_tile, seg_roots and seg_points kernels become grid-stride loops over these lists instead of covering the full grid, and they skip reads of inactive neighbour masks. Grid sizes come from the previous frame's active counts plus headroom. This trades two extra small kernels and list indirection for skipping uniform background tiles. The grid may be undersized if activity jumps between calls, though the loops still stride over the full count.

Result: no change. 379,700, median of 2 (-0.6%).

```diff
diff --git a/aprilslam_amd/csrc/aprilslam.hip b/aprilslam_amd/csrc/aprilslam.hip
--- a/aprilslam_amd/csrc/aprilslam.hip
+++ b/aprilslam_amd/csrc/aprilslam.hip
@@ -98,6 +98,8 @@
     DevBuf<unsigned int> hcounts, class_lists, stage_pos, frame_cursor, dense_tiles, dense_seg, quad_list;
     DevBuf<unsigned long long> stage_rec;
     DevBuf<uint4> seg_edges;
+    DevBuf<uint8_t> seg_active;
+    DevBuf<unsigned int> seg_list, pts_list;
     unsigned int stage_cap = 0;
     DevBuf<unsigned long long> slot_cluster;
     DevBuf<ClusterRec> clusters;
@@ -131,6 +133,7 @@
     bool p_has_cam = false;
     CamDev p_cam{};
     size_t prefetched = 0, nd_guess = 0;
+    size_t seg_guess = 0, pts_guess = 0;
     std::chrono::steady_clock::time_point t_submit, t_enqueued;
     PinnedBuf<long long> pinned_counters;
     PinnedBuf<DetOut> host_det;
@@ -315,6 +318,8 @@
 }
 
 static int seg_nwx(const Geom &g) { return (g.sw + 63) / 64; }
+static int seg_ntiles(const Geom &g) { return seg_nwx(g) * ((g.sh + SEG_TH - 1) / SEG_TH); }
+static int seg_point_groups_x(const Geom &g) { return (seg_nwx(g) + SEGP_NW - 1) / SEGP_NW; }
 static int seg_point_tiles_y(const Geom &g) { return std::max(1, (g.sh - 1 + SEG_PH - 1) / SEG_PH); }
 static size_t count_tiles(const Geom &g) { return (size_t)seg_nwx(g) * (size_t)seg_point_tiles_y(g); }
 
@@ -353,8 +358,11 @@
     bad |= d->stage_pos.ensure((size_t)B * d->stage_cap);
     bad |= d->frame_cursor.ensure(B);
     bad |= d->dense_tiles.ensure(B * count_tiles(g));
-    bad |= d->dense_seg.ensure(B * (size_t)seg_nwx(g) * (size_t)((g.sh + SEG_TH - 1) / SEG_TH));
-    bad |= d->seg_edges.ensure(B * (size_t)seg_nwx(g) * (size_t)((g.sh + SEG_TH - 1) / SEG_TH));
+    bad |= d->dense_seg.ensure(B * (size_t)seg_ntiles(g));
+    bad |= d->seg_edges.ensure(B * (size_t)seg_ntiles(g));
+    bad |= d->seg_active.ensure(B * (size_t)seg_ntiles(g));
+    bad |= d->seg_list.ensure(B * (size_t)seg_ntiles(g));
+    bad |= d->pts_list.ensure(B * (size_t)seg_point_groups_x(g) * (size_t)seg_point_tiles_y(g));
     bad |= d->scratch.ensure((size_t)d->max_points * 8);
     bad |= d->dets.ensure(d->max_dets);
     bad |= d->frame_ndets.ensure(B);
@@ -431,16 +439,20 @@
     } else
         hipLaunchKernelGGL((g.channels == 1 ? k_decimate_minmax<1> : k_decimate_minmax<3>), dim3((g.sw + 63) / 64, (thx + 3) / 4, B), blk, 0, st, d_frames, g, d->dgray.p, d->tmin.p, d->tmax.p);
 
-    const int nwx = seg_nwx(g), pty = seg_point_tiles_y(g);
-    const size_t nwords = (size_t)B * g.sh * nwx;
+    const int nwx = seg_nwx(g), pty = seg_point_tiles_y(g), ngx = seg_point_groups_x(g), ntiles = seg_ntiles(g);
+    const size_t all_seg = (size_t)B * ntiles, all_pts = (size_t)B * ngx * pty;
+    const size_t nseg = d->seg_guess ? std::min(d->seg_guess, all_seg) : all_seg, npts = d->pts_guess ? std::min(d->pts_guess, all_pts) : all_pts;
     STAGE("k_tile_cut");
     if (g.tw > 0 && g.th > 0)
         hipLaunchKernelGGL(k_tile_cut, dim3((((g.tw + 3) / 4) * ((g.th + 3) / 4) + 255) / 256, B), dim3(256), 0, st, d->tmin.p, d->tmax.p, g, d->tcut.p);
+    hipLaunchKernelGGL(k_seg_active, dim3((unsigned int)((all_seg + 255) / 256)), dim3(256), 0, st, d->tcut.p, g, nwx, ntiles, d->seg_active.p, d->seg_list.p,
+                       d->counters.p);
+    hipLaunchKernelGGL(k_seg_active_points, dim3((unsigned int)((all_pts + 255) / 256)), dim3(256), 0, st, d->seg_active.p, g, nwx, ntiles, pty, ngx,
+                       d->pts_list.p, d->counters.p);
     STAGE("k_seg_tile");
     {
-        const int ntiles = nwx * ((g.sh + SEG_TH - 1) / SEG_TH);
-        hipLaunchKernelGGL(k_seg_tile, dim3((ntiles + SEG_TILE_WAVES - 1) / SEG_TILE_WAVES, 1, B), dim3(64 * SEG_TILE_WAVES), 0, st, d->dgray.p, d->tcut.p, g, nwx, ntiles,
-                           d->wmask.p, d->bmask.p, d->parent.p, d->sizes.p, d->rootmask.p, d->seg_edges.p, d->dense_seg.p, d->counters.p);
+        hipLaunchKernelGGL(k_seg_tile, dim3((unsigned int)((nseg + SEG_TILE_WAVES - 1) / SEG_TILE_WAVES)), dim3(64 * SEG_TILE_WAVES), 0, st, d->dgray.p, d->tcut.p, g, nwx,
+                           ntiles, d->seg_list.p, d->wmask.p, d->bmask.p, d->parent.p, d->sizes.p, d->rootmask.p, d->seg_edges.p, d->dense_seg.p, d->counters.p);
         hipLaunchKernelGGL(k_seg_tile_dense, dim3(1024), dim3(64), 0, st, g, nwx, ntiles, d->wmask.p, d->bmask.p, d->parent.p, d->sizes.p,
                            d->rootmask.p, d->dense_seg.p, d->counters.p);
     }
@@ -451,17 +463,19 @@
         const int nrb = (g.sh - 1) / SEG_TH;
         const unsigned int nrow_blocks = (unsigned int)nwx * (unsigned int)nrb * (unsigned int)B;
         if (ncol_blocks + nrow_blocks > 0)
-            hipLaunchKernelGGL(k_seg_border, dim3(ncol_blocks + nrow_blocks), dim3(64), 0, st, d->wmask.p, d->bmask.p, d->seg_edges.p,
-                               nwx * ((g.sh + SEG_TH - 1) / SEG_TH), g, nwx, d->parent.p, d->counters.p, ncol_blocks, nrb > 0 ? nrb : 1);
+            hipLaunchKernelGGL(k_seg_border, dim3(ncol_blocks + nrow_blocks), dim3(64), 0, st, d->wmask.p, d->bmask.p, d->seg_edges.p, d->seg_active.p,
+                               ntiles, g, nwx, d->parent.p, d->counters.p, ncol_blocks, nrb > 0 ? nrb : 1);
     }
     STAGE("k_seg_roots");
-    hipLaunchKernelGGL(k_seg_roots, dim3((unsigned int)((nwords + 255) / 256)), dim3(256), 0, st, d->rootmask.p, g, nwx, d->parent.p, d->sizes.p);
+    hipLaunchKernelGGL(k_seg_roots, dim3((unsigned int)((nseg + 7) / 8)), dim3(256), 0, st, d->rootmask.p, g, nwx, ntiles, d->seg_list.p, d->counters.p,
+                       d->parent.p, d->sizes.p);
 
     STAGE("k_seg_points");
-    hipLaunchKernelGGL((k_seg_points<SEGP_PCAP, SEGP_RUNCAP, SEGP_NW, 1>), dim3(B, (nwx + SEGP_NW - 1) / SEGP_NW, pty), dim3(64 * SEGP_NW), 0, st,
-                       d->wmask.p, d->bmask.p, g, nwx, d->parent.p, d->sizes.p, d->hkeys.p, d->hcounts.p, d->nslots - 1, d->stage_rec.p,
+    hipLaunchKernelGGL((k_seg_points<SEGP_PCAP, SEGP_RUNCAP, SEGP_NW, 1>), dim3((unsigned int)npts), dim3(64 * SEGP_NW), 0, st,
+                       d->wmask.p, d->bmask.p, d->seg_active.p, ntiles, d->pts_list.p, ngx, g, nwx, d->parent.p, d->sizes.p, d->hkeys.p, d->hcounts.p, d->nslots - 1, d->stage_rec.p,
                        d->stage_pos.p, d->frame_cursor.p, d->stage_cap, d->dense_tiles.p, pty, d->counters.p);
-    hipLaunchKernelGGL((k_seg_points<SEGP_PCAP_DENSE, SEGP_RUNCAP_DENSE, 1, 2>), dim3(256), dim3(64), 0, st, d->wmask.p, d->bmask.p, g, nwx,
+    hipLaunchKernelGGL((k_seg_points<SEGP_PCAP_DENSE, SEGP_RUNCAP_DENSE, 1, 2>), dim3(256), dim3(64), 0, st, d->wmask.p, d->bmask.p,
+                       d->seg_active.p, ntiles, d->pts_list.p, ngx, g, nwx,
                        d->parent.p, d->sizes.p, d->hkeys.p, d->hcounts.p, d->nslots - 1, d->stage_rec.p, d->stage_pos.p, d->frame_cursor.p,
                        d->stage_cap, d->dense_tiles.p, pty, d->counters.p);
     STAGE("k_cluster_filter");
@@ -532,6 +546,8 @@
     c.half = (double)(float)(tag_size / 2);
     return c;
 }
+
+static long long c_active(long long n) { return n + n / 4 + 16; }
 
 using clk = std::chrono::steady_clock;
 static float msf(clk::time_point a, clk::time_point b) { return std::chrono::duration<float, std::milli>(b - a).count(); }
@@ -630,6 +646,8 @@
         if (cam) HIPCHK(hipMemcpy(d->host_pose.p + have, d->out_pose.p + have, (nd - have) * sizeof(PoseOut), hipMemcpyDeviceToHost));
     }
     d->nd_guess = nd + nd / 4 + 256;
+    d->seg_guess = (size_t)c_active(d->last_counters[CNT_ACTIVE_SEG]);
+    d->pts_guess = (size_t)c_active(d->last_counters[CNT_ACTIVE_PTS]);
     clk::time_point t3 = clk::now();
     static_assert(sizeof(DetOut) == sizeof(asl_detection) && sizeof(PoseOut) == sizeof(asl_pose), "device results are copied verbatim");
     int total = (int)nd;
diff --git a/aprilslam_amd/csrc/asl_common.h b/aprilslam_amd/csrc/asl_common.h
--- a/aprilslam_amd/csrc/asl_common.h
+++ b/aprilslam_amd/csrc/asl_common.h
@@ -153,7 +153,9 @@
     CNT_NKEEP = 144,
     CNT_DENSE_TILES = 160,
     CNT_DENSE_SEG = 161,
-    CNT__N = 176
+    CNT_ACTIVE_SEG = 176,
+    CNT_ACTIVE_PTS = 192,
+    CNT__N = 208
 };
 #define CNT_CLASS(c) (CNT_CLASS0 + 16 * (c))
 
diff --git a/aprilslam_amd/csrc/debug_host.inc b/aprilslam_amd/csrc/debug_host.inc
--- a/aprilslam_amd/csrc/debug_host.inc
+++ b/aprilslam_amd/csrc/debug_host.inc
@@ -23,7 +23,7 @@
 {
     if (d->dbg_thresh.ensure(total)) return fail(ASL_ENOMEM, "debug buffer allocation failed");
     hipLaunchKernelGGL(k_seg_debug_thresh, dim3((g.sw + 63) / 64, (g.sh + 3) / 4, (unsigned int)g.nframes), dim3(64, 4), 0, nullptr,
-                       d->wmask.p, d->bmask.p, g, seg_nwx(g), d->dbg_thresh.p);
+                       d->wmask.p, d->bmask.p, d->seg_active.p, seg_ntiles(g), g, seg_nwx(g), d->dbg_thresh.p);
     HIPCHK(hipGetLastError());
     return ASL_OK;
 }
@@ -53,7 +53,7 @@
         if (bytes < total * 4) return fail(ASL_EINVAL, "dst too small: need %zu bytes", total * 4);
         if (d->dbg_labels.ensure(total)) return fail(ASL_ENOMEM, "debug buffer allocation failed");
         hipLaunchKernelGGL(k_seg_debug_labels, dim3((g.sw + 63) / 64, (g.sh + 3) / 4, (unsigned int)g.nframes), dim3(64, 4), 0, nullptr,
-                           d->wmask.p, d->bmask.p, g, seg_nwx(g), d->parent.p, d->dbg_labels.p);
+                           d->wmask.p, d->bmask.p, d->seg_active.p, seg_ntiles(g), g, seg_nwx(g), d->parent.p, d->dbg_labels.p);
         HIPCHK(hipGetLastError());
         HIPCHK(hipMemcpy(dst, d->dbg_labels.p, total * 4, hipMemcpyDeviceToHost));
         *n_items = total;
diff --git a/aprilslam_amd/csrc/k_seg.inc b/aprilslam_amd/csrc/k_seg.inc
--- a/aprilslam_amd/csrc/k_seg.inc
+++ b/aprilslam_amd/csrc/k_seg.inc
@@ -1,6 +1,7 @@
 
 #define SEG_TH 32
 #define SEG_PH 63
+#define SEGP_NW 4
 
 __device__ __forceinline__ unsigned long long seg_join_mask(int x0, int sw)
 {
@@ -139,6 +140,82 @@
         }
 }
 
+template <int NT>
+__device__ __forceinline__ void seg_list_append(bool keep, unsigned int item, unsigned int *__restrict__ list, long long *counter)
+{
+    __shared__ unsigned int s_cnt[NT / 64];
+    __shared__ unsigned long long s_base;
+    const int lane = threadIdx.x & 63, wid = threadIdx.x >> 6;
+    const unsigned long long m = __ballot(keep);
+    if (lane == 0) s_cnt[wid] = (unsigned int)__popcll(m);
+    __syncthreads();
+    if (threadIdx.x == 0) {
+        unsigned int t = 0;
+        for (int w = 0; w < NT / 64; w++) t += s_cnt[w];
+        s_base = t ? atomicAdd((unsigned long long *)counter, (unsigned long long)t) : 0ull;
+    }
+    __syncthreads();
+    if (!keep) return;
+    unsigned long long at = s_base + __popcll(m & ((1ull << lane) - 1ull));
+    for (int w = 0; w < wid; w++) at += s_cnt[w];
+    list[at] = item;
+}
+
+__global__ void __launch_bounds__(256) k_seg_active(const uint8_t *__restrict__ tcut, Geom g, int nwx, int ntiles, uint8_t *__restrict__ active,
+                                                    unsigned int *__restrict__ seg_list, long long *counters)
+{
+    const unsigned int i = blockIdx.x * 256u + threadIdx.x;
+    const bool exists = i < (unsigned int)ntiles * (unsigned int)g.nframes;
+    bool act = false;
+    if (exists) {
+#ifdef ASL_SEG_ALL_TILES
+        act = true;
+#else
+        const int tw = g.tw, th = g.th;
+        if (tw > 0 && th > 0) {
+            const unsigned int fr = i / (unsigned int)ntiles, tile = i - fr * (unsigned int)ntiles;
+            const int wx = (int)(tile % (unsigned int)nwx), y0 = (int)(tile / (unsigned int)nwx) * SEG_TH;
+            const int c0 = min(16 * wx, tw - 1), c1 = min(16 * wx + 15, tw - 1);
+            const int r0 = min(y0 / TILESZ, th - 1), r1 = min(min(y0 + SEG_TH - 1, g.sh - 1) / TILESZ, th - 1);
+            const uint8_t *tc = tcut + (size_t)fr * tw * th;
+            static_assert(SEG_TH / TILESZ == 8, "eight rows of cuts per labelling tile");
+            if (c1 - c0 == 15) {
+                uint4 v[8];
+#pragma unroll
+                for (int k = 0; k < 8; k++) __builtin_memcpy(&v[k], tc + (size_t)min(r0 + k, r1) * tw + c0, 16);
+                unsigned int all = 0xFFFFFFFFu;
+#pragma unroll
+                for (int k = 0; k < 8; k++) all &= v[k].x & v[k].y & v[k].z & v[k].w;
+                act = all != 0xFFFFFFFFu;
+            } else {
+                for (int r = r0; r <= r1; r++)
+                    for (int c = c0; c <= c1; c++) act |= tc[(size_t)r * tw + c] != 255;
+            }
+        }
+#endif
+        active[i] = act ? 1 : 0;
+    }
+    seg_list_append<256>(act, i, seg_list, &counters[CNT_ACTIVE_SEG]);
+}
+
+__global__ void __launch_bounds__(256) k_seg_active_points(const uint8_t *__restrict__ active, Geom g, int nwx, int ntiles, int tiles_y, int ngx,
+                                                           unsigned int *__restrict__ pts_list, long long *counters)
+{
+    const unsigned int j = blockIdx.x * 256u + threadIdx.x, B = (unsigned int)g.nframes;
+    const unsigned int unit = j / B, fr = j - unit * B;
+    const int ty = (int)(unit / (unsigned int)ngx), gx = (int)(unit - (unsigned int)ty * (unsigned int)ngx);
+    bool act = false;
+    if (ty < tiles_y) {
+        const int y0 = ty * SEG_PH;
+        const int r0 = y0 / SEG_TH, r1 = min(y0 + SEG_PH, g.sh - 1) / SEG_TH;
+        const int c0 = max(gx * SEGP_NW - 1, 0), c1 = min(gx * SEGP_NW + SEGP_NW, nwx - 1);
+        const uint8_t *a = active + (size_t)fr * ntiles;
+        for (int r = r0; r <= r1; r++)
+            for (int c = c0; c <= c1; c++) act |= a[r * nwx + c] != 0;
+    }
+    seg_list_append<256>(act, (fr * (unsigned int)tiles_y + (unsigned int)ty) * (unsigned int)ngx + (unsigned int)gx, pts_list, &counters[CNT_ACTIVE_PTS]);
+}
+
 #ifndef SEG_TILE_WAVES
 #define SEG_TILE_WAVES 4
 #endif
@@ -173,8 +250,10 @@
             px[hf] = make_uint4(d[0], d[1], d[2], d[3]);
         }
     }
+#ifdef ASL_SEG_ALL_TILES
     const unsigned int cmin = min(min(min(cut[0][0], cut[0][1]), min(cut[0][2], cut[0][3])), min(min(cut[1][0], cut[1][1]), min(cut[1][2], cut[1][3])));
     if (__ballot(cmin != 255u) == 0ull) return 0ull;
+#endif
     unsigned int xlo[2], xhi[2];
 #pragma unroll
     for (int hf = 0; hf < 2; hf++) {
@@ -204,6 +283,7 @@
 }
 
 __global__ void __launch_bounds__(64 * SEG_TILE_WAVES) k_seg_tile(const uint8_t *__restrict__ dgray, const uint8_t *__restrict__ tcut, Geom g, int nwx, int ntiles,
+                                                 const unsigned int *__restrict__ seg_list,
                                                  unsigned long long *__restrict__ wmask, unsigned long long *__restrict__ bmask,
                                                  unsigned int *__restrict__ parent, unsigned int *__restrict__ sizes,
                                                  unsigned long long *__restrict__ rootmask, uint4 *__restrict__ edges, unsigned int *__restrict__ dense_list,
@@ -212,14 +292,17 @@
     __shared__ unsigned int Ls[SEG_TILE_WAVES][SEG_CAP];
     __shared__ unsigned int WLs[SEG_TILE_WAVES][SEG_CAP];
     __shared__ unsigned long long RMKs[SEG_TILE_WAVES][SEG_TH];
-    const int lane = threadIdx.x & 63, wave = threadIdx.x >> 6;
+    const int lane = threadIdx.x & 63, wave = __builtin_amdgcn_readfirstlane((int)(threadIdx.x >> 6));
     unsigned int *const L = Ls[wave], *const WL = WLs[wave];
     unsigned long long *const RMK = RMKs[wave];
-    const int tile = blockIdx.x * SEG_TILE_WAVES + wave, fr = blockIdx.z;
-    if (tile >= ntiles) return;
+    const int sw = g.sw, sh = g.sh;
+    const long long nactive = counters[CNT_ACTIVE_SEG];
+    PHASE_DECL();
+  for (long long work = (long long)blockIdx.x * SEG_TILE_WAVES + wave; work < nactive; work += (long long)gridDim.x * SEG_TILE_WAVES) {
+    seg_wave_sync();
+    const unsigned int id = __builtin_amdgcn_readfirstlane(seg_list[work]);
+    const int fr = (int)(id / (unsigned int)ntiles), tile = (int)(id % (unsigned int)ntiles);
     const int wx = tile % nwx, x0 = wx * 64, y0 = (tile / nwx) * SEG_TH;
-    const int sw = g.sw, sh = g.sh;
-    PHASE_DECL();
     PHASE_INIT();
     unsigned long long M = 0;
     if (g.tw > 0 && g.th > 0)
@@ -236,11 +319,12 @@
         if (lane == 0) edges[(size_t)fr * ntiles + tile] = make_uint4((unsigned int)el, (unsigned int)(el >> 32), (unsigned int)er, (unsigned int)(er >> 32));
     }
     PHASE(8);
+#ifdef ASL_SEG_ALL_TILES
     if (__ballot(M != 0) == 0ull) {
         if (isw && y < sh) rootmask[mi] = 0ull;
-        PHASE_FLUSH(48);
-        return;
-    }
+        continue;
+    }
+#endif
     const unsigned long long J = seg_join_mask(x0, sw);
     const unsigned long long S = seg_starts(M, J);
     unsigned long long Mp = __shfl_up(M, 1), Sp = __shfl_up(S, 1);
@@ -256,9 +340,8 @@
     const int nlinks = (int)(tot & 0xFFFFu), nruns = (int)(tot >> 16);
     PHASE_COUNT(12, nlinks); PHASE_COUNT(13, nruns); PHASE_COUNT(14, 1);
     if (nlinks > SEG_CAP || nruns > SEG_CAP) {
-        if (lane == 0) dense_list[atomicAdd((unsigned long long *)&counters[CNT_DENSE_SEG], 1ull)] = (unsigned int)fr * (unsigned int)ntiles + (unsigned int)tile;
-        PHASE_FLUSH(48);
-        return;
+        if (lane == 0) dense_list[atomicAdd((unsigned long long *)&counters[CNT_DENSE_SEG], 1ull)] = id;
+        continue;
     }
     const unsigned int rb = (incl >> 16) - nruns_lane;
     const unsigned int rbp = (unsigned int)__shfl_up((int)rb, 1);
@@ -330,6 +413,7 @@
     }
     if (isw && y < sh) rootmask[mi] = rm;
     PHASE(11);
+  }
     PHASE_FLUSH(48);
 }
 
@@ -440,7 +524,7 @@
 }
 
 __device__ __forceinline__ void seg_border_cols_body(const unsigned long long *__restrict__ wmask, const unsigned long long *__restrict__ bmask,
-                                                     const uint4 *__restrict__ edges, int ntiles, const Geom &g, int nwx,
+                                                     const uint4 *__restrict__ edges, const uint8_t *__restrict__ active, int ntiles, const Geom &g, int nwx,
                                                      unsigned int *__restrict__ parent, long long *counters, unsigned int blk)
 {
     const int sw = g.sw, sh = g.sh;
@@ -454,8 +538,11 @@
     const unsigned long long *wm = wmask + (size_t)fr * per_frame, *bm = bmask + (size_t)fr * per_frame;
     const size_t m0 = (size_t)wx * sh + y;
     const size_t et = (size_t)fr * ntiles + (size_t)(y / SEG_TH) * nwx + wx;
-    const uint4 ec = edges[et], el = edges[et - 1];
-    const bool seam = inrange && ((((ec.x | ec.y) | (el.z | el.w)) >> (y % SEG_TH)) & 1u) != 0u;
+    const bool both = inrange && active[et] != 0 && active[et - 1] != 0;
+    if (__ballot(both) == 0ull) return;
+    const uint4 none = make_uint4(0u, 0u, 0u, 0u);
+    const uint4 ec = both ? edges[et] : none, el = both ? edges[et - 1] : none;
+    const bool seam = both && ((((ec.x | ec.y) | (el.z | el.w)) >> (y % SEG_TH)) & 1u) != 0u;
     if (__ballot(seam) == 0ull) return;
     const bool diag = seam && y > 0 && (y % SEG_TH) != 0;
     const unsigned long long W = seam ? wm[m0] : 0ull, B = seam ? bm[m0] : 0ull, Wl = seam ? wm[m0 - sh] : 0ull, Bl = seam ? bm[m0 - sh] : 0ull;
@@ -490,7 +577,8 @@
 }
 
 __device__ __forceinline__ void seg_border_rows_body(const unsigned long long *__restrict__ wmask, const unsigned long long *__restrict__ bmask,
-                                                     const Geom &g, int nwx, unsigned int *__restrict__ parent, long long *counters, int wx, int rb, int fr)
+                                                     const uint8_t *__restrict__ active, int ntiles, const Geom &g, int nwx,
+                                                     unsigned int *__restrict__ parent, long long *counters, int wx, int rb, int fr)
 {
     const int sw = g.sw, sh = g.sh;
     const int y = (rb + 1) * SEG_TH, x0 = wx * 64;
@@ -498,6 +586,8 @@
     const size_t per_frame = (size_t)nwx * sh;
     const unsigned long long *wm = wmask + (size_t)fr * per_frame, *bm = bmask + (size_t)fr * per_frame;
     const size_t m0 = (size_t)wx * sh + y;
+    const uint8_t *const above = active + (size_t)fr * ntiles + (size_t)rb * nwx + wx;
+    if (above[0] == 0 || above[nwx] == 0) return;
     const unsigned long long W = wm[m0], B = bm[m0], Wp = wm[m0 - 1], Bp = bm[m0 - 1];
     if ((W | B) == 0ull || (Wp | Bp) == 0ull) return;
     unsigned int *P = parent + (size_t)fr * g.npix;
@@ -516,7 +606,7 @@
             if (bx > 0) {
                 if ((Wp >> (bx - 1)) & 1ull) ok &= seg_global_join(P, me, gidx(wx, y - 1, seg_start_of(seg_starts(Wp, J), bx - 1)));
             } else if (wx > 0) {
-                const unsigned long long Wlp = wm[m0 - sh - 1];
+                const unsigned long long Wlp = above[-1] != 0 ? wm[m0 - sh - 1] : 0ull;
                 if (Wlp >> 63) ok &= seg_global_join(P, me, gidx(wx - 1, y - 1, seg_start_of(seg_starts(Wlp, seg_join_mask(x0 - 64, sw)), 63)));
             }
         }
@@ -524,7 +614,7 @@
             if (((Wp >> (bx + 1)) & 1ull) && !(((Wp >> bx) & 1ull) && ((J >> (bx + 1)) & 1ull)))
                 ok &= seg_global_join(P, me, gidx(wx, y - 1, seg_start_of(seg_starts(Wp, J), bx + 1)));
         } else if (wx + 1 < nwx) {
-            const unsigned long long Wrp = wm[m0 + sh - 1];
+            const unsigned long long Wrp = above[1] != 0 ? wm[m0 + sh - 1] : 0ull;
             if ((Wrp & 1ull) && !((Wp >> 63) && (seg_join_mask(x0 + 64, sw) & 1ull))) ok &= seg_global_join(P, me, gidx(wx + 1, y - 1, 0));
         }
     }
@@ -532,29 +622,30 @@
 }
 
 __global__ void __launch_bounds__(64) k_seg_border(const unsigned long long *__restrict__ wmask, const unsigned long long *__restrict__ bmask,
-                                                   const uint4 *__restrict__ edges, int ntiles, Geom g, int nwx, unsigned int *__restrict__ parent,
-                                                   long long *counters, unsigned int ncol_blocks, int nrb)
+                                                   const uint4 *__restrict__ edges, const uint8_t *__restrict__ active, int ntiles, Geom g, int nwx,
+                                                   unsigned int *__restrict__ parent, long long *counters, unsigned int ncol_blocks, int nrb)
 {
     if (blockIdx.x < ncol_blocks) {
-        seg_border_cols_body(wmask, bmask, edges, ntiles, g, nwx, parent, counters, blockIdx.x);
+        seg_border_cols_body(wmask, bmask, edges, active, ntiles, g, nwx, parent, counters, blockIdx.x);
     } else {
         const unsigned int r = blockIdx.x - ncol_blocks;
         const unsigned int t = r / (unsigned int)nwx;
-        seg_border_rows_body(wmask, bmask, g, nwx, parent, counters, (int)(r - t * (unsigned int)nwx), (int)(t % (unsigned int)nrb), (int)(t / (unsigned int)nrb));
-    }
-}
-
-__global__ void __launch_bounds__(256) k_seg_roots(const unsigned long long *__restrict__ rootmask, Geom g, int nwx,
+        seg_border_rows_body(wmask, bmask, active, ntiles, g, nwx, parent, counters, (int)(r - t * (unsigned int)nwx), (int)(t % (unsigned int)nrb), (int)(t / (unsigned int)nrb));
+    }
+}
+
+__global__ void __launch_bounds__(256) k_seg_roots(const unsigned long long *__restrict__ rootmask, Geom g, int nwx, int ntiles,
+                                                   const unsigned int *__restrict__ seg_list, const long long *__restrict__ counters,
                                                    unsigned int *__restrict__ parent, unsigned int *__restrict__ sizes)
 {
-    const size_t per_frame = (size_t)nwx * g.sh;
-    const size_t i = (size_t)blockIdx.x * blockDim.x + threadIdx.x;
-    if (i >= per_frame * g.nframes) return;
-    unsigned long long w = rootmask[i];
-    if (!w) return;
-    const int fr = (int)(i / per_frame);
-    const int rem = (int)(i - (size_t)fr * per_frame);
-    const int wx = rem / g.sh, y = rem - wx * g.sh;
+    static_assert(SEG_TH == 32, "a lane per row, eight tiles per 256 threads");
+    const long long nactive = counters[CNT_ACTIVE_SEG];
+  for (long long work = (long long)blockIdx.x * 8 + (threadIdx.x >> 5); work < nactive; work += (long long)gridDim.x * 8) {
+    const unsigned int id = seg_list[work];
+    const int fr = (int)(id / (unsigned int)ntiles), tile = (int)(id % (unsigned int)ntiles);
+    const int wx = tile % nwx, y = (tile / nwx) * SEG_TH + (int)(threadIdx.x & 31u);
+    if (y >= g.sh) continue;
+    unsigned long long w = rootmask[((size_t)fr * nwx + wx) * g.sh + y];
     unsigned int *P = parent + (size_t)fr * g.npix;
     unsigned int *S = sizes + (size_t)fr * g.npix;
     while (w) {
@@ -568,10 +659,10 @@
             P[p] = root;
         }
     }
+  }
 }
 
 #define SEGP_NSLOT 256
-#define SEGP_NW 4
 #define SEGP_RUNCAP 2048
 #define SEGP_RUNCAP_DENSE 4352
 #define SEGP_PCAP 4096
@@ -579,6 +670,7 @@
 
 template <int PCAP, int RUNCAP, int NW, int NHALF>
 __global__ void __launch_bounds__(64 * NW) k_seg_points(const unsigned long long *__restrict__ wmask, const unsigned long long *__restrict__ bmask,
+                                                        const uint8_t *__restrict__ active, int ntiles, const unsigned int *__restrict__ pts_list, int ngx,
                                                         Geom g, int nwx, const unsigned int *__restrict__ labels, const unsigned int *__restrict__ sizes,
                                                         unsigned long long *keys, unsigned int *counts, unsigned int hmask,
                                                         unsigned long long *stage_rec, unsigned int *stage_pos, unsigned int *frame_cursor,
@@ -600,17 +692,21 @@
     const int sw = g.sw, sh = g.sh;
     const size_t per_frame = (size_t)nwx * sh;
     PHASE_DECL();
-    const long long ndense = DENSE ? counters[CNT_DENSE_TILES] : 1;
-  for (long long work = DENSE ? blockIdx.x : 0; work < ndense; work += DENSE ? gridDim.x : 1) {
-    int wx, ty, fr;
+    const long long nwork = counters[DENSE ? CNT_DENSE_TILES : CNT_ACTIVE_PTS];
+  for (long long work = blockIdx.x; work < nwork; work += gridDim.x) {
+    int wx, ty, fr, gx = 0;
+    __syncthreads();
     if (DENSE) {
-        __syncthreads();
         const unsigned int tile_id = dense_tiles[work];
         wx = (int)(tile_id % (unsigned int)nwx);
         ty = (int)((tile_id / (unsigned int)nwx) % (unsigned int)tiles_y);
         fr = (int)(tile_id / (unsigned int)(nwx * tiles_y));
     } else {
-        fr = blockIdx.x; ty = blockIdx.z; wx = (int)blockIdx.y * NW + wid;
+        const unsigned int unit = pts_list[work];
+        gx = (int)(unit % (unsigned int)ngx);
+        ty = (int)((unit / (unsigned int)ngx) % (unsigned int)tiles_y);
+        fr = (int)(unit / (unsigned int)(ngx * tiles_y));
+        wx = gx * NW + wid;
     }
     const unsigned int my_tile_id = (unsigned int)((fr * tiles_y + ty) * nwx + wx);
     const int x0 = wx * 64, y0 = ty * SEG_PH;
@@ -624,17 +720,19 @@
     bool wl = false, bl = false, wr = false, br = false;
     unsigned long long SL = 0;
     if (rowok) {
-        W = wm[m0]; B = bm[m0];
-        if (wx > 0) {
+        const uint8_t *const act = active + (size_t)fr * ntiles + (size_t)(y / SEG_TH) * nwx + wx;
+        const bool ac = act[0] != 0, al = wx > 0 && act[-1] != 0, ar = wx + 1 < nwx && act[1] != 0;
+        if (ac) { W = wm[m0]; B = bm[m0]; }
+        if (al) {
             const unsigned long long Wl = wm[m0 - sh], Bl = bm[m0 - sh];
             wl = Wl >> 63; bl = Bl >> 63;
             if (wl || bl) SL = seg_starts(wl ? Wl : Bl, seg_join_mask(x0 - 64, sw));
         }
-        if (wx + 1 < nwx) { wr = wm[m0 + sh] & 1ull; br = bm[m0 + sh] & 1ull; }
+        if (ar) { wr = wm[m0 + sh] & 1ull; br = bm[m0 + sh] & 1ull; }
     }
     const bool tile_live = __ballot((W | B) != 0ull) != 0ull;
     if (!DENSE) {
-        if (!__syncthreads_or(tile_live ? 1 : 0)) return;
+        if (!__syncthreads_or(tile_live ? 1 : 0)) continue;
     }
     const unsigned long long J = seg_join_mask(x0, sw);
     const unsigned long long Sall = seg_starts(W, J) | seg_starts(B, J);
@@ -661,7 +759,7 @@
     ROWB[tid] = (unsigned int)base | ((unsigned int)nown << 13) | (havel ? 1u << 20 : 0u);
     if (total > RUNCAP) {
         if (lane == 0 && tile_live) dense_tiles[atomicAdd((unsigned long long *)&counters[CNT_DENSE_TILES], 1ull)] = my_tile_id;
-        return;
+        continue;
     }
     if (tile_live) {
         unsigned long long m = Sall;
@@ -684,7 +782,7 @@
             const int i = i0 + u * NT + tid;
             e[u] = i < total ? RT[i] : 0xFFFFFFFFu;
             const int kind = (int)((e[u] >> 12) & 3u), ew = DENSE ? 0 : (int)((e[u] >> 14) & 3u);
-            const int ex0 = DENSE ? x0 : ((int)blockIdx.y * NW + ew) * 64;
+            const int ex0 = DENSE ? x0 : (gx * NW + ew) * 64;
             const unsigned int p = (unsigned int)((y0 + (int)((e[u] >> 6) & 63u)) * sw + ex0 + (kind == 1 ? -64 : (kind == 2 ? 64 : 0)) + (int)(e[u] & 63u));
             l[u] = e[u] != 0xFFFFFFFFu ? lab[p] : 0u;
         }
@@ -847,7 +945,7 @@
     if (npts > (unsigned int)PCAP) {
         if (!DENSE) {
             if (lane == 0 && tile_live) dense_tiles[atomicAdd((unsigned long long *)&counters[CNT_DENSE_TILES], 1ull)] = my_tile_id;
-            return;
+            break;
         }
         if (tid == 0) atomicAdd((unsigned long long *)&counters[CNT_OVERFLOW_POINTS], 1ull);
         continue;
@@ -881,7 +979,7 @@
         const bool black = (w >> 14) & 1u;
         const unsigned int slot = w >> 17;
         const int dx = k == 0 ? 1 : (k == 1 ? 0 : (k == 2 ? -1 : 1)), dy = k == 0 ? 0 : 1;
-        const int px0 = DENSE ? x0 : ((int)blockIdx.y * NW + pw) * 64;
+        const int px0 = DENSE ? x0 : (gx * NW + pw) * 64;
         unsigned int gslot, pos;
         if (slot == (unsigned int)(NSLOT - 1)) {
             int gs = hash_insert(keys, hmask, cluster_key(fr, label_at(pw * 64 + ly, lx), label_at(pw * 64 + ly + dy, lx + dx)));
@@ -909,23 +1007,26 @@
 }
 
 __global__ void __launch_bounds__(256) k_seg_debug_thresh(const unsigned long long *__restrict__ wmask, const unsigned long long *__restrict__ bmask,
-                                                          Geom g, int nwx, uint8_t *__restrict__ thresh)
+                                                          const uint8_t *__restrict__ active, int ntiles, Geom g, int nwx, uint8_t *__restrict__ thresh)
 {
     const int x = blockIdx.x * 64 + threadIdx.x, y = blockIdx.y * 4 + threadIdx.y, fr = blockIdx.z;
     if (x >= g.sw || y >= g.sh) return;
     const size_t mi = ((size_t)fr * nwx + (x >> 6)) * g.sh + y;
-    const unsigned long long W = wmask[mi], B = bmask[mi];
+    const bool act = active[(size_t)fr * ntiles + (size_t)(y / SEG_TH) * nwx + (x >> 6)] != 0;
+    const unsigned long long W = act ? wmask[mi] : 0ull, B = act ? bmask[mi] : 0ull;
     thresh[(size_t)fr * g.npix + (size_t)y * g.sw + x] = ((W >> (x & 63)) & 1ull) ? 255 : (((B >> (x & 63)) & 1ull) ? 0 : 127);
 }
 
 __global__ void __launch_bounds__(256) k_seg_debug_labels(const unsigned long long *__restrict__ wmask, const unsigned long long *__restrict__ bmask,
-                                                          Geom g, int nwx, const unsigned int *__restrict__ parent, unsigned int *__restrict__ out)
+                                                          const uint8_t *__restrict__ active, int ntiles, Geom g, int nwx,
+                                                          const unsigned int *__restrict__ parent, unsigned int *__restrict__ out)
 {
     const int x = blockIdx.x * 64 + threadIdx.x, y = blockIdx.y * 4 + threadIdx.y, fr = blockIdx.z;
     if (x >= g.sw || y >= g.sh) return;
     const int wx = x >> 6, b = x & 63;
     const size_t mi = ((size_t)fr * nwx + wx) * g.sh + y;
-    const unsigned long long W = wmask[mi], B = bmask[mi];
+    const bool act = active[(size_t)fr * ntiles + (size_t)(y / SEG_TH) * nwx + wx] != 0;
+    const unsigned long long W = act ? wmask[mi] : 0ull, B = act ? bmask[mi] : 0ull;
     const unsigned int p = (unsigned int)(y * g.sw + x);
     unsigned int l = p;
     if (((W | B) >> b) & 1ull) {
```
